# seungjunlee96/lightning-generative-models

Hardware: AMD Instinct MI355X
Metric: training images/sec (DDPM UNet 32x32, bs=128) (higher is better)
Workload: dtype f32; 1 GPU; configs/diffusion/ddpm.json UNet dim=64, 3x32x32 synthetic NCHW fp32, training_step+backward+Adam+EMA; global_batch=128, per_gpu_batch=128, parallelism=dp1, launch=hipGraph replay (1 graph/step)

## Files before the change

include/lgm_hip.h:

```cpp
#ifndef LGM_HIP_H
#define LGM_HIP_H

#include <stdint.h>

#ifdef __cplusplus
extern "C" {
#endif

#define LGM_ABI_VERSION 7
#define LGM_OK 0
#define LGM_ERR_INVALID (-1)
#define LGM_ERR_UNSUPPORTED (-2)

int lgm_abi_version(void);
const char* lgm_last_error(void);
const char* lgm_last_kernel(void);
int lgm_kernel_name_count(void);
const char* lgm_kernel_name(int i);

typedef struct {
  int32_t B, H, W, Cw;
  int32_t Ho, Wo, Nw;
  int32_t KH, KW, stride, pad;
} LgmConvGeom;
// ... 306 lines not shown
                float beta_acc, float* m_out, void* stream);
int lgm_bn_reduce3_coef(int modes, const float* v1, int64_t v1_pitch, const float* v2, int64_t v2_pitch,
                        const float* a, int64_t a_pitch, const float* mean, const float* rstd,
                        const float* gamma, const float* saved_m, int64_t rows, int C, float* coef8,
                        float* ggamma0, float* gbeta0, float beta_acc0, float* m_out, float* ggamma1,
                        float beta_acc1, float* sums3, void* workspace, void* stream);
int lgm_bn_reduce3_coef_tiles(int modes, const float* partial, int tiles, const float* gamma, const float* rstd,
                              const float* saved_m, int64_t rows, int C, float* coef8, float* ggamma0, float* gbeta0,
                              float beta_acc0, float* m_out, float* ggamma1, float beta_acc1, float* sums3, void* stream);
int lgm_bn_affine3x2(const float* v1, int64_t v1_pitch, const float* v2, int64_t v2_pitch, const float* a,
                     int64_t a_pitch, const float* mean, const float* rstd, const float* coef8, float* out0,
                     int64_t out0_pitch, float* out1, int64_t out1_pitch, int64_t rows, int C, void* stream);
int lgm_bn_affine3(const float* v1, int64_t v1_pitch, const float* v2, int64_t v2_pitch,
                   const float* a, int64_t a_pitch, const float* mean, const float* rstd,
                   const float* A1, const float* A2, const float* A3, const float* A4, float* out,
                   int64_t out_pitch, int accumulate, int act, float slope, int64_t rows, int C,
                   void* stream);
int lgm_image_transform(const unsigned char* src, int64_t B, int H, int W, int C, const unsigned char* flip,
                        float* dst, int S, void* stream);
int lgm_lerp_rows(const float* x, const float* y, const float* alpha, float* out, int64_t B,
                  int64_t rowlen, void* stream);
int64_t lgm_gp_penalty_workspace(int64_t npix);
int lgm_gp_penalty(const float* g, int64_t npix, int C, float lambda, const float* gscale,
                   float* loss_out, float* gbar, void* workspace, void* stream);
int lgm_r1_penalty(const float* g, int64_t npix, int64_t B, const float* gscale, float* loss_out,
                   float* gbar, void* workspace, void* stream);
int lgm_mean_col(const float* v, int64_t pitch, int64_t n, float scale, float* out, void* stream);
int lgm_fill_col(float* out, int64_t pitch, int64_t n, int ncols, int col, float scale,
                 const float* vptr, void* stream);
int lgm_wgan_dloss(float* vals4, void* stream);
int lgm_vqvae_loss(const float* recon, const float* out3, float w_recon, float w_vq, float* vals4, void* stream);
int lgm_vqvae_loss_samples(const float* per_sample, int n, const float* out3, float w_recon, float w_vq, float* vals4,
                           void* stream);
int lgm_tanh_mse_fwd(const float* pre, const float* target, int64_t pitch, int B, int C, int HW, int Cpad, float* xh,
                     float* per_sample, void* stream);
int lgm_tanh_mse_bwd(const float* xh, const float* target, int64_t pitch, const float* gloss, float w_recon, float w_vq,
                     int B, int C, int HW, int Cpad, float* gpre, float* g2, void* stream);

int64_t lgm_resstack_fwd_supported(int H, int W, int Cin, int hidden, int Rh, int layers);
int lgm_resstack_fwd(const float* x, int64_t x_pitch, int B, int H, int W, int Cin, int hidden, int Rh, int layers,
                     const float* const* w3, const float* const* w1, float* const* y, float* const* z, void* stream);
int lgm_scale_pair(const float* g, float w0, float w1, float* out2, void* stream);

int64_t lgm_conv3x3_bf16x3_supported(const LgmConvGeom* g, int mode, int64_t a_pitch);
int lgm_split_bf16x3(const float* src, uint16_t* dst, const int32_t* table, int n_slots, int64_t total_chunks,
                     int64_t plane_elems, void* stream);
int lgm_conv3x3_bf16x3(int mode, const LgmConvGeom* g, const float* a, int64_t a_pitch,
                       const uint16_t* w_planes, int64_t plane_elems, const float* bias, const float* res,
                       int64_t res_pitch, float* out, int64_t out_pitch, void* workspace,
                       int64_t workspace_bytes, void* stream);

int64_t lgm_conv3x3_wino_supported(const LgmConvGeom* g, int yx);
int64_t lgm_conv3x3_wino_fits(const LgmConvGeom* g, int64_t a_pitch, int64_t out_pitch, int64_t res_pitch);
int64_t lgm_conv3x3_wino_workspace_partial(const LgmConvGeom* g, int yx);
int64_t lgm_conv3x3_wino_bwd_supported(const LgmConvGeom* g, int64_t gy_pitch, int64_t x_pitch, int64_t gx_pitch,
                                       int64_t res_pitch);
int lgm_conv3x3_wino_bwd_workspaces(const LgmConvGeom* g, int partial, int64_t* out);
int lgm_conv3x3_wino_bwd(const LgmConvGeom* g, const float* gy, int64_t gy_pitch, const float* x, int64_t x_pitch,
                         const float* u_b, const float* res, int64_t res_pitch, float* gx, int64_t gx_pitch,
                         void* dgrad_ws, int64_t dgrad_ws_bytes, int64_t* partial, float* gw, float* gbias, float beta,
                         void* wgrad_ws, int64_t wgrad_ws_bytes, int64_t* desc, void* stream);
int64_t lgm_conv3x3_wino_wgrad2_supported(const LgmConvGeom* ga, const LgmConvGeom* gb);
typedef struct {
  const LgmConvGeom* g;
  const float* y;
  int64_t y_pitch;
  const float* x;
  int64_t x_pitch;
  float* gw;
  float* gbias;
  float beta;
  void* ws;
  int64_t ws_bytes;
  int64_t* desc;
} LgmWgradItem;
int64_t lgm_wgrad1x1_group_supported(int n, const LgmConvGeom* const* geoms);
int lgm_wgrad_queue_enable(int on);
int lgm_wgrad_queue_flush(void);
int lgm_wgrad1x1_group_workspaces(int n, const LgmConvGeom* const* geoms, int64_t* out);
int lgm_wgrad1x1_group(int n, const LgmWgradItem* items, void* stream);
int64_t lgm_conv3x3_wino_wgradn_supported(int n, const LgmConvGeom* const* geoms);
int lgm_conv3x3_wino_wgradn_workspaces(int n, const LgmConvGeom* const* geoms, int64_t* out);
int lgm_conv3x3_wino_wgradn(int n, const LgmWgradItem* items, void* stream);
int lgm_conv3x3_wino_wgrad2_workspaces(const LgmConvGeom* ga, const LgmConvGeom* gb, int64_t* out);
int lgm_conv3x3_wino_wgrad2(const LgmConvGeom* ga, const float* ya, int64_t ya_pitch, const float* xa, int64_t xa_pitch,
                            float* gwa, float* gba, float beta_a, void* wsa, int64_t wsa_bytes, int64_t* desca,
                            const LgmConvGeom* gb, const float* yb, int64_t yb_pitch, const float* xb, int64_t xb_pitch,
                            float* gwb, float* gbb, float beta_b, void* wsb, int64_t wsb_bytes, int64_t* descb,
                            void* stream);
int lgm_conv3x3_wino_partial(int yx, const LgmConvGeom* g, const float* a, int64_t a_pitch, const float* u,
                             const float* bias, float* out, int64_t out_pitch, void* workspace,
                             int64_t workspace_bytes, int64_t* partial, void* stream);
int64_t lgm_conv3x3_wino_workspace(const LgmConvGeom* g, int yx);
int lgm_wino_weights(const float* src, float* dst_f, float* dst_b, const int64_t* table, int n_slots,
                     int64_t total_blocks, void* stream);
int lgm_wino_set_debug_buffer(void* buf, int mode);
int lgm_conv3x3_wino(int yx, const LgmConvGeom* g, const float* a, int64_t a_pitch, const float* u,
                     const float* bias, const float* res, int64_t res_pitch, float* out, int64_t out_pitch,
                     void* workspace, int64_t workspace_bytes, void* stream);

int64_t lgm_conv3x3_wino4_supported(const LgmConvGeom* g, int yx);
int64_t lgm_conv3x3_wino4_workspace(const LgmConvGeom* g, int yx);
int64_t lgm_conv3x3_wino4_preferred(const LgmConvGeom* g, int yx);
int lgm_conv3x3_wino4_partial(int yx, const LgmConvGeom* g, const float* a, int64_t a_pitch, const float* u,
                              const float* bias, float* out, int64_t out_pitch, void* workspace,
                              int64_t workspace_bytes, int64_t* partial, void* stream);
int64_t lgm_conv3x3_wino4_stats_floats(const LgmConvGeom* g, int* parts_per_image);
int lgm_conv3x3_wino4_stats(const LgmConvGeom* g, const float* x, int64_t x_pitch, const float* u, const float* bias,
                            float* y, int64_t y_pitch, float* stats, int64_t stats_floats, void* stream);
int lgm_wino4_weights(const float* src, float* dst_f, float* dst_b, const int64_t* table, int n_slots,
                      int64_t total_blocks, void* stream);
int lgm_wino4_set_debug_buffer(void* buf, int exp);
int lgm_conv3x3_wino4(int yx, const LgmConvGeom* g, const float* a, int64_t a_pitch, const float* u,
                      const float* bias, const float* res, int64_t res_pitch, float* out, int64_t out_pitch,
                      void* workspace, int64_t workspace_bytes, void* stream);

int lgm_wino4_set_light(int mode);

int lgm_set_cu_margin(int margin);
int lgm_cu_margin(void);
int64_t lgm_conv3x3_wino4l_supported(const LgmConvGeom* g, int yx);
int64_t lgm_conv3x3_wino4l_workspace(const LgmConvGeom* g, int yx);
int lgm_conv3x3_wino4l(int yx, const LgmConvGeom* g, const float* a, int64_t a_pitch, const float* u,
                       const float* bias, const float* res, int64_t res_pitch, float* out, int64_t out_pitch,
                       void* workspace, int64_t workspace_bytes, void* stream);

int64_t lgm_conv3x3_wino4_wgrad_supported(const LgmConvGeom* g);
int64_t lgm_conv3x3_wino4_wgrad_workspace(const LgmConvGeom* g);
int lgm_conv3x3_wino4_wgrad(const LgmConvGeom* g, const float* y, int64_t y_pitch, const float* x, int64_t x_pitch,
                            float* gw, float* gbias, float beta, void* workspace, int64_t workspace_bytes,
                            int64_t* desc, void* stream);

int lgm_adam_step(float* p, const float* g, float* m, float* v, int64_t n, float lr, float b1,
                  float b2, float eps, float weight_decay, float step, const float* step_dev,
                  float grad_scale, int decoupled, void* stream);
int lgm_rmsprop_step(float* p, const float* g, float* sq, int64_t n, float lr, float alpha, float eps,
                     float weight_decay, float grad_scale, void* stream);
int lgm_clamp(float* x, int64_t n, float lo, float hi, void* stream);
int lgm_ema_lerp(float* shadow, const float* online, int64_t n, float w, void* stream);
int lgm_add_scalar(float* x, float a, void* stream);
int lgm_fill(float* x, int64_t n, float val, void* stream);

#ifdef __cplusplus
}
#endif
#endif
```

lightning-generative-models_amd/csrc/conv3x3.hip:

```cpp
#include <type_traits>
#include "lgm_common.h"

namespace lgm3x3 {
typedef unsigned int u32x4 __attribute__((ext_vector_type(4)));

constexpr int BN = 64;
constexpr int BK = 32;

enum { MODE_XY = 0, MODE_YX = 1, MODE_YXT = 2 };

struct Args {
  const float* a;
  const float* w;
  const float* bias;
  const float* res;
  float* out;
  long a_pitch, res_pitch, out_pitch;
  int B, H, W;
  int C;
  int N;
  int Wn;
  int TH, TW, NI, lgTW, lgTT;
  int tiles_h, tiles_w, tiles_n, NP;
  int units, per;
  int splits, pps;
  float* ws;
  long ws_stride;
  const unsigned short* wb;
  long w_plane;
};

__global__ __launch_bounds__(256) void splitk_reduce_kernel(const float* __restrict__ ws, long ws_stride, int splits,
                                                            const float* __restrict__ bias,
                                                            const float* __restrict__ res, long res_pitch,
                                                            float* __restrict__ out, long out_pitch, long M, int N) {
  const int n4 = N / 4;
  const long i = (long)blockIdx.x * blockDim.x + threadIdx.x;
  if (i >= M * n4) return;
  const long m = i / n4;
  const int n = (int)(i % n4) * 4;
  f32x4 s = *reinterpret_cast<const f32x4*>(ws + m * N + n);
  for (int k = 1; k < splits; ++k) s += *reinterpret_cast<const f32x4*>(ws + (long)k * ws_stride + m * N + n);
  if (bias) s += *reinterpret_cast<const f32x4*>(bias + n);
  if (res) s += *reinterpret_cast<const f32x4*>(res + m * res_pitch + n);
  *reinterpret_cast<f32x4*>(out + m * out_pitch + n) = s;
}

__device__ __forceinline__ int xcd_swizzle(int bid, int nb) {
  return (nb % 8 == 0) ? (bid % 8) * (nb / 8) + bid / 8 : bid;
}

struct Phase {
  int L, cc, cc_end;
  int tn, split, twi, thi, bg;
  int n0, b0, h0, w0;
  unsigned border;
  long abase;
  bool valid;
};

template <int MODE>
__global__ __launch_bounds__(256, 1) void conv3x3_kernel(const Args p) {
  constexpr int CK = 32;
  constexpr int LDP = CK + 4;
  constexpr int TPP = CK / 4;
  constexpr int PPP = 256 / TPP;
  constexpr int U = 9;
  constexpr int NJ = 288 / PPP;
  static_assert(NJ == U, "one patch position per step");
  constexpr int PBUF = 288 * LDP;
  extern __shared__ __align__(16) float smem[];

  const int tid = threadIdx.x;
  const int lane = tid & 63, wid = tid >> 6;
  const int wm = wid >> 1, wn = wid & 1;
  const int lr = lane & 31, lh = lane >> 5;
  float* Ts = smem + 2 * PBUF + wid * LGM_TS_FLOATS;

  const int Lb = xcd_swizzle(blockIdx.x, gridDim.x);
  const int L0 = Lb * p.per;
  const int L1 = min(p.units, L0 + p.per);
  if (L0 >= L1) return;

  const int PW = p.TW + 2, PP1 = (p.TH + 2) * PW;
  const int ncc_total = p.C / CK;

  auto place = [&](Phase& ph) {
    ph.n0 = ph.tn * BN;
    ph.w0 = ph.twi * p.TW;
    ph.h0 = ph.thi * p.TH;
    ph.b0 = ph.bg * p.NI;
    ph.cc = ph.split * p.pps;
    ph.cc_end = min(ncc_total, ph.cc + p.pps);
    ph.border = 16u | (ph.h0 == 0 ? 1u : 0u) | (ph.h0 + p.TH == p.H ? 2u : 0u) | (ph.w0 == 0 ? 4u : 0u) |
                (ph.w0 + p.TW == p.W ? 8u : 0u);
    ph.abase = ((long)((ph.b0 * p.H + ph.h0) * p.W + ph.w0) * p.a_pitch) * 4;
  };
  auto decode = [&](Phase& ph, int L) {
    ph.L = L;
    ph.tn = L % p.tiles_n;
    int ts = L / p.tiles_n;
    ph.split = ts % p.splits;
    ts /= p.splits;
    ph.twi = ts % p.tiles_w;
    ts /= p.tiles_w;
    ph.thi = ts % p.tiles_h;
    ph.bg = ts / p.tiles_h;
    place(ph);
  };
  auto advance = [&](Phase& ph) {
    if (!ph.valid) return;
    if (ph.cc + 1 < ph.cc_end) {
      ++ph.cc;
    } else if (ph.L + 1 < L1) {
      ++ph.L;
      if (++ph.tn == p.tiles_n) {
        ph.tn = 0;
        if (++ph.split == p.splits) {
          ph.split = 0;
          if (++ph.twi == p.tiles_w) {
            ph.twi = 0;
            if (++ph.thi == p.tiles_h) {
              ph.thi = 0;
              ++ph.bg;
            }
          }
// ... 957 lines not shown
extern "C" int lgm_split_bf16x3(const float* src, uint16_t* dst, const int32_t* table, int n_slots, int64_t total_chunks,
                                int64_t plane_elems, void* stream) {
  LGM_REQUIRE(src && dst && table && n_slots > 0 && total_chunks > 0 && plane_elems % 8 == 0 && lgm_aligned16(src) &&
                  lgm_aligned16(dst),
              "split_bf16x3: bad arguments");
  hipLaunchKernelGGL(lgm3x3::split_bf16x3_kernel, dim3((unsigned)lgm_cdiv(total_chunks, 256)), dim3(256), 0,
                     (hipStream_t)stream, src, dst, table, n_slots, (long)total_chunks, (long)plane_elems);
  LGM_LAUNCH_CHECK();
  return LGM_OK;
}

extern "C" int lgm_conv3x3_bf16x3(int mode, const LgmConvGeom* g, const float* a, int64_t a_pitch,
                                  const uint16_t* w_planes, int64_t plane_elems, const float* bias, const float* res,
                                  int64_t res_pitch, float* out, int64_t out_pitch, void* workspace,
                                  int64_t workspace_bytes, void* stream) {
  using namespace lgm3x3;
  LGM_REQUIRE(g && a && w_planes && out && (mode == 0 || mode == 1), "conv3x3_bf16x3: bad arguments");
  LGM_REQUIRE(lgm_conv3x3_bf16x3_supported(g, mode, a_pitch), "conv3x3_bf16x3: unsupported geometry");
  LGM_REQUIRE(lgm_aligned16(a) && lgm_aligned16(out) && a_pitch % 4 == 0 && out_pitch % 4 == 0 &&
                  (((uintptr_t)w_planes) & 15u) == 0 && plane_elems % 8 == 0 &&
                  (!res || (lgm_aligned16(res) && res_pitch % 4 == 0)) && (!bias || lgm_aligned16(bias)),
              "conv3x3_bf16x3: 16-byte aligned tensors with pitch %% 4 == 0 required");
  hipStream_t s = (hipStream_t)stream;
  Args p{};
  p.a = a; p.w = nullptr; p.wb = w_planes; p.w_plane = plane_elems; p.bias = bias; p.res = res; p.out = out;
  p.a_pitch = a_pitch; p.res_pitch = res_pitch; p.out_pitch = out_pitch;
  p.B = g->B; p.H = g->H; p.W = g->W;
  p.C = mode == 0 ? g->Cw : g->Nw;
  p.N = mode == 0 ? g->Nw : g->Cw;
  p.Wn = g->Cw;
  plan_tile(g->H, g->W, &p.TH, &p.TW, &p.NI);
  p.lgTW = ilog2(p.TW);
  p.lgTT = ilog2(p.TH * p.TW);
  p.tiles_h = g->H / p.TH;
  p.tiles_w = g->W / p.TW;
  p.tiles_n = p.N / BN;
  p.NP = p.NI * (p.TH + 2) * (p.TW + 2);
  const int groups = lgm_cdiv(g->B, p.NI);
  const long M = (long)g->B * g->H * g->W;
  p.splits = lgm_conv3x3_splits(g, p.C, p.N);
  if (p.splits > 1) {
    const long need = (long)p.splits * M * p.N * (long)sizeof(float);
    if (!workspace || workspace_bytes < need || !lgm_aligned16(workspace)) p.splits = 1;
  }
  p.ws = (float*)workspace;
  p.ws_stride = M * p.N;
  p.pps = lgm_cdiv(p.C / 32, p.splits);
  p.splits = lgm_cdiv(p.C / 32, p.pps);
  p.units = (int)((long)groups * p.tiles_h * p.tiles_w * p.tiles_n * p.splits);
  p.per = lgm_cdiv(p.units, lgm_cu_budget());
  const unsigned nblocks = (unsigned)lgm_cdiv(p.units, p.per);
  const size_t smem = (size_t)2 * 288 * 208 + 4 * LGM_TS_FLOATS * sizeof(float);
  if (mode == 0) {
    static bool attr = false;
    if (!attr) {
      hipFuncSetAttribute(reinterpret_cast<const void*>(conv3x3_b3_kernel<false>), hipFuncAttributeMaxDynamicSharedMemorySize,
                          (int)smem);
      attr = true;
    }
    hipLaunchKernelGGL(conv3x3_b3_kernel<false>, dim3(nblocks), dim3(256), smem, s, p);
  } else {
    static bool attr = false;
    if (!attr) {
      hipFuncSetAttribute(reinterpret_cast<const void*>(conv3x3_b3_kernel<true>), hipFuncAttributeMaxDynamicSharedMemorySize,
                          (int)smem);
      attr = true;
    }
    hipLaunchKernelGGL(conv3x3_b3_kernel<true>, dim3(nblocks), dim3(256), smem, s, p);
  }
  if (p.splits > 1) {
    const long items = M * (p.N / 4);
    hipLaunchKernelGGL(splitk_reduce_kernel, dim3((unsigned)lgm_cdiv(items, 256)), dim3(256), 0, s, (const float*)p.ws,
                       p.ws_stride, p.splits, bias, res, res_pitch, out, out_pitch, M, p.N);
  }
  LGM_LAUNCH_CHECK();
  return LGM_OK;
}

int lgm_splitk_reduce_launch(const float* ws, long ws_stride, int splits, const float* bias, const float* res,
                             long res_pitch, float* out, long out_pitch, long M, int N, hipStream_t s) {
  const long items = M * (N / 4);
  hipLaunchKernelGGL(lgm3x3::splitk_reduce_kernel, dim3((unsigned)lgm_cdiv(items, 256)), dim3(256), 0, s, ws, ws_stride,
                     splits, bias, res, res_pitch, out, out_pitch, M, N);
  LGM_LAUNCH_CHECK();
  return LGM_OK;
}

bool lgm_wgrad3x3_supported(const LgmConvGeom* g) {
  using namespace lgm3x3;
  int TH, TW, NI;
  if (!(g->KH == 3 && g->KW == 3 && g->stride == 1 && g->pad == 1)) return false;
  if (g->Cw % 64 != 0 || g->Nw % 64 != 0) return false;
  if (!plan_tile(g->H, g->W, &TH, &TW, &NI)) return false;
  return g->B % NI == 0;
}

void lgm_wgrad3x3_plan(const LgmConvGeom* g, int* splits, int* tps, int* total_ts) {
  using namespace lgm3x3;
  int TH, TW, NI;
  plan_tile(g->H, g->W, &TH, &TW, &NI);
  const int total = lgm_cdiv(g->B, NI) * (g->H / TH) * (g->W / TW);
  const long tiles = (long)(g->Nw / 64) * (g->Cw / 64);
  long s = lgm_cu_budget() / tiles;
  if (s > total) s = total;
  if (s < 1) s = 1;
  const int t = lgm_cdiv(total, s);
  *tps = t;
  const int tsplits = lgm_cdiv(total, t);
  const long wgs = tiles * tsplits;
  static const bool no_gsplit = getenv("LGM_NO_GSPLIT") != nullptr;
  const int gsplit = no_gsplit ? 1 : wgs <= 64 ? 4 : wgs <= 128 ? 2 : 1;
  *splits = tsplits * gsplit;
  *total_ts = total;
}

int lgm_wgrad3x3_launch(const LgmConvGeom* g, const float* y, long y_pitch, const float* x, long x_pitch,
                        float* out, float* bias_out, float beta, long slab, int splits, int tps, int total_ts,
                        hipStream_t s) {
  using namespace lgm3x3;
  WArgs p{};
  int TW;
  p.y = y; p.x = x; p.out = out; p.bias_out = bias_out; p.beta = beta; p.slab = slab;
  p.y_pitch = y_pitch; p.x_pitch = x_pitch;
  p.B = g->B; p.H = g->H; p.W = g->W; p.Nw = g->Nw; p.Cw = g->Cw;
  plan_tile(g->H, g->W, &p.TH, &TW, &p.NI);
  p.lgTH = ilog2(p.TH);
  p.tiles_h = g->H / p.TH; p.tiles_w = g->W / TW;
  p.tiles_n = g->Nw / 64; p.tiles_c = g->Cw / 64;
  p.splits = splits; p.tps = tps; p.total_ts = total_ts;
  p.gsplit = splits / lgm_cdiv(total_ts, tps);
  const int NP = p.NI * (p.TH + 2) * (TW + 2);
  (void)NP;
  const size_t smem = (size_t)(128 * 64 + 288 * 64) * sizeof(float);
  const unsigned nblocks = (unsigned)((long)p.tiles_n * p.tiles_c * splits);
#define LGM_W3_LAUNCH1(TWV, GSV)                                                                       \
  do {                                                                                                 \
    auto kern = wgrad3x3_kernel<TWV, GSV>;                                                             \
    static size_t attr = 0;                                                                            \
    if (smem > attr) {                                                                                 \
      hipFuncSetAttribute(reinterpret_cast<const void*>(kern), hipFuncAttributeMaxDynamicSharedMemorySize, (int)smem); \
      attr = smem;                                                                                     \
    }                                                                                                  \
    lgm_note_kernel(LGM_KNAME("lgm3x3::wgrad3x3_kernel<" #TWV ", " #GSV ">"));                                    \
    hipLaunchKernelGGL(kern, dim3(nblocks), dim3(256), smem, s, p);                                    \
  } while (0)
#define LGM_W3_LAUNCH(TWV)                                                                             \
  do {                                                                                                 \
    if (p.gsplit == 4) LGM_W3_LAUNCH1(TWV, 4);                                                         \
    else if (p.gsplit == 2) LGM_W3_LAUNCH1(TWV, 2);                                                    \
    else LGM_W3_LAUNCH1(TWV, 1);                                                                       \
  } while (0)
  if (p.gsplit != 1 && p.gsplit != 2 && p.gsplit != 4) {
    lgm_set_error("wgrad3x3: unsupported group split %d", p.gsplit);
    return LGM_ERR_UNSUPPORTED;
  }
  switch (TW) {
    case 32: LGM_W3_LAUNCH(32); break;
    case 16: LGM_W3_LAUNCH(16); break;
    case 8: LGM_W3_LAUNCH(8); break;
    case 4: LGM_W3_LAUNCH(4); break;
    default: lgm_set_error("wgrad3x3: unsupported tile width %d", TW); return LGM_ERR_UNSUPPORTED;
  }
#undef LGM_W3_LAUNCH
#undef LGM_W3_LAUNCH1
  LGM_LAUNCH_CHECK();
  return LGM_OK;
// ... 2 lines not shown
```

lightning-generative-models_amd/csrc/lgm_internal.h:

```cpp
#pragma once
#include <hip/hip_runtime.h>
#include <stdint.h>

#include "../../include/lgm_hip.h"

bool lgm_conv3x3_supported(const LgmConvGeom* g, int gather_channels, int out_channels);
int lgm_conv3x3_splits(const LgmConvGeom* g, int gather_channels, int out_channels);
int lgm_conv3x3_launch(int mode, const LgmConvGeom* g, const float* a, long a_pitch, const float* w, const float* bias,
                       const float* res, long res_pitch, float* out, long out_pitch, void* workspace, long workspace_bytes,
                       hipStream_t s);
int lgm_splitk_reduce_launch(const float* ws, long ws_stride, int splits, const float* bias, const float* res,
                             long res_pitch, float* out, long out_pitch, long M, int N, hipStream_t s);
bool lgm_wgrad3x3_supported(const LgmConvGeom* g);
void lgm_wgrad3x3_plan(const LgmConvGeom* g, int* splits, int* tps, int* total_ts);
int lgm_wgrad3x3_launch(const LgmConvGeom* g, const float* y, long y_pitch, const float* x, long x_pitch, float* out,
                        float* bias_out, float beta, long slab, int splits, int tps, int total_ts, hipStream_t s);

int lgm_wgrad_reduce_launch(const float* ws, long slab, float* gw, long n_w, float* gb, long n_b, int splits, float beta,
                            hipStream_t s);

bool lgm_wgrad1x1_supported(const LgmConvGeom* g, long y_pitch, long x_pitch);
void lgm_wgrad1x1_plan(const LgmConvGeom* g, int* splits, int* chunks_per_split);
int lgm_wgrad1x1_launch(const LgmConvGeom* g, const float* y, long y_pitch, const float* x, long x_pitch, float* out,
                        float* bias_out, float beta, long slab, int splits, int chunks_per_split, hipStream_t s);

bool lgm_gemm_stream_supported(long M, int N, int K, long x_pitch, long out_pitch, long res_pitch);
int lgm_gemm_stream_launch(const float* x, long x_pitch, const float* w, const float* bias, const float* res,
                           long res_pitch, float* out, long out_pitch, long M, int N, int K, hipStream_t s);
bool lgm_gemm_rows_supported(long M, int N, int K);
int lgm_gemm_rows_launch(const float* x, long x_pitch, const float* w, const float* bias, const float* res,
                         long res_pitch, float* out, long out_pitch, long M, int N, int K, hipStream_t s);

bool lgm_wino_supported(const LgmConvGeom* g, int gather_channels, int out_channels);
int lgm_wino_splits(const LgmConvGeom* g, int gather_channels, int out_channels, bool fused = false);
int lgm_wino_launch(const LgmConvGeom* g, int yx, const float* a, long a_pitch, const float* u, const float* bias,
                    const float* res, long res_pitch, float* out, long out_pitch, void* workspace, long workspace_bytes,
                    hipStream_t s, int64_t* partial = nullptr);
bool lgm_wino_wgrad_supported(const LgmConvGeom* g);
void lgm_wino_wgrad_plan(const LgmConvGeom* g, int* splits, int* cps, int* total_chunks);
int lgm_wino_wgrad_launch(const LgmConvGeom* g, const float* y, long y_pitch, const float* x, long x_pitch, float* out,
                          int bias, long slab, int splits, int cps, int total_chunks, hipStream_t s);
struct WinoPairPlan {
  int csplits, wsplits, cps, total_chunks;
};
WinoPairPlan lgm_wino_pair_plan(const LgmConvGeom* g, bool fused);
int lgm_wino_pair_launch(const LgmConvGeom* g, const float* gy, long gy_pitch, const float* x, long x_pitch,
                         const float* u_b, const float* res, long res_pitch, float* gx, long gx_pitch, void* dws,
                         long dws_bytes, int64_t* partial, float* slabs, int bias, long slab, hipStream_t s);

bool lgm_wino4_supported(const LgmConvGeom* g, int gather_channels, int out_channels);
int lgm_wino4_pick_splits(long base, long slots, int phases, int smax, int min_pps);
int lgm_wino4_splits(const LgmConvGeom* g, int gather_channels, int out_channels);
int lgm_wino4_launch(const LgmConvGeom* g, int yx, const float* a, long a_pitch, const float* u, const float* bias,
                     const float* res, long res_pitch, float* out, long out_pitch, void* workspace, long workspace_bytes,
                     hipStream_t s, int64_t* partial = nullptr, float* stats = nullptr);
bool lgm_wino4l_supported(const LgmConvGeom* g, int gather_channels, int out_channels);
long lgm_wino4l_units(const LgmConvGeom* g, int out_channels);
int lgm_wino4l_stats_parts(const LgmConvGeom* g);
int lgm_wino4l_class(const LgmConvGeom* g);
int lgm_wino4l_splits(const LgmConvGeom* g, int gather_channels, int out_channels);
int lgm_wino4l_launch(const LgmConvGeom* g, int yx, const float* a, long a_pitch, const float* u, const float* bias,
                      const float* res, long res_pitch, float* out, long out_pitch, void* workspace, long workspace_bytes,
                      hipStream_t s, int64_t* partial, float* stats);

bool lgm_wino4_wgrad_supported(const LgmConvGeom* g);
bool lgm_wino4_wgrad_use(const LgmConvGeom* g);
void lgm_wino4_wgrad_plan(const LgmConvGeom* g, long budget, int* splits, int* gps, int* total_groups);
int lgm_wino4_wgrad_launch(const LgmConvGeom* g, const float* y, long y_pitch, const float* x, long x_pitch, float* out,
                           int bias, long slab, int splits, int gps, int total, hipStream_t s);
int lgm_wino4_wgradn_launch(int n, const LgmConvGeom* const* gs, const float* const* ys, const long* yps,
                            const float* const* xs, const long* xps, float* const* outs, const int* biases,
                            const long* slabs, const int* splits, const int* gpss, const int* totals, hipStream_t s);

int lgm_linattn_ctx_launch(int mode, const float* qkv, long pitch, const float* mem_kv, const float* gout,
                           long gout_pitch, const float* ctx_in, int B, int n, int heads, int M, float scale,
                           float* ctx_out, float* kmax, float* ksum, float* r_out, hipStream_t s,
                           const float* kmax_in = nullptr, const float* ksum_in = nullptr, float* gmem_partial = nullptr);
int lgm_linattn_bwd_launch(const float* qkv, long pitch, const float* mem_kv, const float* gout, long gout_pitch,
                           const float* ctx, const float* gctx, const float* kmax, const float* ksum, const float* rvec,
                           int B, int n, int heads, int M, float scale, float* gqkv, long gq_pitch, float* gmem_partial,
                           hipStream_t s);
int lgm_linattn_bwd_fused_launch(const float* qkv, long pitch, const float* gout, long gout_pitch, const float* ctx,
                                 const float* gctx, const float* kmax, const float* ksum, const float* rvec,
                                 const float* xn, long xn_pitch, const float* wt, int B, int n, float scale, float* gxn,
                                 long gxn_pitch, float* slabs, int* blocks_out, hipStream_t s);
int lgm_linattn_out_fused_launch(const float* qkv, long pitch, const float* ctx, const float* wout, const float* bout,
                                 const float* g, const float* x, long x_pitch, float* ao, long ao_pitch, float* o2,
                                 long o2_pitch, float* y, long y_pitch, int B, int n, int Cout, float scale, hipStream_t s);
int lgm_attn_tiled_fwd_launch(const float* qkv, long pitch, const float* mem_kv, int B, int n, int heads, int M,
                              float scale, float* out, long out_pitch, float* lse, hipStream_t s);
int lgm_attn_tiled_bwd_launch(const float* qkv, long pitch, const float* mem_kv, const float* out, long out_pitch,
                              const float* gout, long gout_pitch, const float* lse, int B, int n, int heads, int M,
                              float scale, float* gqkv, long gq_pitch, float* gmem_partial, hipStream_t s);
```

lightning-generative-models_amd/csrc/wino4_device.h:

```cpp
#pragma once
#include "lgm_common.h"

namespace lgmwino4dev {
typedef unsigned int u32x4 __attribute__((ext_vector_type(4)));
typedef unsigned int u32x2 __attribute__((ext_vector_type(2)));
typedef float f32x2 __attribute__((ext_vector_type(2)));

constexpr int KC = 8;
constexpr int NXI = 36;

__device__ __forceinline__ f32x4 add4(const f32x4 a, const f32x4 b) { return a + b; }
__device__ __forceinline__ f32x4 sub4(const f32x4 a, const f32x4 b) {
  f32x2 lo, hi;
  asm("v_pk_add_f32 %0, %1, %2 neg_lo:[0,1] neg_hi:[0,1]"
      : "=v"(lo)
      : "v"(__builtin_shufflevector(a, a, 0, 1)), "v"(__builtin_shufflevector(b, b, 0, 1)));
  asm("v_pk_add_f32 %0, %1, %2 neg_lo:[0,1] neg_hi:[0,1]"
      : "=v"(hi)
      : "v"(__builtin_shufflevector(a, a, 2, 3)), "v"(__builtin_shufflevector(b, b, 2, 3)));
  return __builtin_shufflevector(lo, hi, 0, 1, 2, 3);
}
__device__ __forceinline__ f32x4 fma4(const float c, const f32x4 a, const f32x4 b) {
  return __builtin_elementwise_fma(f32x4{c, c, c, c}, a, b);
}
__device__ __forceinline__ f32x2 fma2(const float c, const f32x2 a, const f32x2 b) {
  return __builtin_elementwise_fma(f32x2{c, c}, a, b);
}

__device__ __forceinline__ __amdgpu_buffer_rsrc_t wave_buffer_rsrc(const float* ptr, unsigned bytes) {
  const unsigned long long ab = reinterpret_cast<unsigned long long>(ptr);
  const unsigned lo = __builtin_amdgcn_readfirstlane((unsigned)ab);
  const unsigned hi = __builtin_amdgcn_readfirstlane((unsigned)(ab >> 32));
  return __builtin_amdgcn_make_buffer_rsrc(reinterpret_cast<void*>(((unsigned long long)hi << 32) | lo), 0,
                                           __builtin_amdgcn_readfirstlane(bytes), 0x00020000);
}

struct ConvArgs {
  const float* a;
  const float* u;
  const float* bias;
  const float* res;
  float* out;
  long a_pitch, res_pitch, out_pitch;
  int B, H, W;
  int C;
  int N;
  int tb_h, tb_w, tiles_n, nbg;
  int splits, pps, units;
  int tn_slowest;
  int xcd_ranges;
  float* ws;
  long ws_stride;
};

struct ConvUnit {
  int tn, split, twi, thi, bg;
};
__device__ __forceinline__ ConvUnit conv_unit(const ConvArgs& p) {
  int L = (p.xcd_ranges && (gridDim.x & 7) == 0) ? (int)((blockIdx.x & 7) * (gridDim.x >> 3) + (blockIdx.x >> 3)) : (int)blockIdx.x;
  ConvUnit q;
  if (p.tn_slowest) {
    q.twi = L % p.tb_w;
    L /= p.tb_w;
    q.thi = L % p.tb_h;
    L /= p.tb_h;
    q.bg = L % p.nbg;
    L /= p.nbg;
    q.split = L % p.splits;
    q.tn = L / p.splits;
  } else {
    q.tn = L % p.tiles_n;
    L /= p.tiles_n;
    q.split = L % p.splits;
    L /= p.splits;
    q.twi = L % p.tb_w;
    L /= p.tb_w;
    q.thi = L % p.tb_h;
    q.bg = L / p.tb_h;
  }
  return q;
}

}
```

lightning-generative-models_amd/csrc/wino4_host.h:

```cpp
#pragma once
#include "wino4_device.h"

namespace lgmwino4host {
namespace {
using lgmwino4dev::KC;

template <class F>
int unit_class(int H, int W) {
  if (F::NCLS > 3 && H == 4 && W == 4) return 3;
  if (H == 8 && W == 8) return 2;
  if (H == 16 && W == 16) return 1;
  if (H >= F::UH && W >= F::UW && H % F::UH == 0 && W % F::UW == 0) return 0;
  return -1;
}

template <class F>
long unit_count(int cls, int B, int H, int W) {
  return cls == 0 ? (long)B * (H / F::UH) * (W / F::UW) : B / F::NI[cls];
}

template <class F>
bool supported(const LgmConvGeom* g, int gather_channels, int out_channels) {
  if (!(g->KH == 3 && g->KW == 3 && g->stride == 1 && g->pad == 1)) return false;
  if (gather_channels % 32 != 0 || out_channels % 64 != 0) return false;
  const int cls = unit_class<F>(g->H, g->W);
  if (cls < 0) return false;
  const long pix = (long)g->B * g->H * g->W + g->W + 1;
  if (pix * gather_channels >= (1L << 29) || pix * out_channels >= (1L << 29)) return false;
  if ((long)gather_channels * out_channels * 36 >= (1L << 29)) return false;
  return g->B % F::NI[cls] == 0;
}

template <class F>
int stats_parts(const LgmConvGeom* g) {
  return unit_class<F>(g->H, g->W) == 0 ? (g->H / F::UH) * (g->W / F::UW) * 4 : 0;
}

int split_front(long base, long slots, int phases, int forced, int* smax) {
  *smax = phases / 2 < 16 ? phases / 2 : 16;
  if (*smax < 1) *smax = 1;
  if (forced > 0) return forced < *smax ? forced : *smax;
  return base >= slots * 3 / 4 ? 1 : 0;
}

void unit_order(lgmwino4dev::ConvArgs& p, long M) {
  static const bool no_ranges = lgm_env_set("LGM_WINO4_NO_XCD_RANGES");
  p.xcd_ranges = no_ranges ? 0 : 1;
  static const int forced = lgm_env_int("LGM_WINO4_TN_SLOWEST", -1);
  const double in_b = 1.2 * (double)M * p.C * 4.0, u_b = 36.0 * p.C * p.N * 4.0;
  p.tn_slowest = forced >= 0 ? forced : ((in_b + 8.0 * u_b > in_b * p.tiles_n + u_b) ? 1 : 0);
}

template <auto KERN, int THREADS, class A>
void launch_kernel(const A& p, size_t smem, hipStream_t s) {
  static bool attr = false;
  if (!attr) {
    (void)hipFuncSetAttribute(reinterpret_cast<const void*>(KERN), hipFuncAttributeMaxDynamicSharedMemorySize, (int)smem);
    attr = true;
  }
  hipLaunchKernelGGL(KERN, dim3((unsigned)p.units), dim3(THREADS), smem, s, p);
}

template <class F>
int conv_launch(const LgmConvGeom* g, int yx, const float* a, long a_pitch, const float* u, const float* bias,
                const float* res, long res_pitch, float* out, long out_pitch, void* workspace, long workspace_bytes,
                hipStream_t s, int64_t* partial, float* stats) {
  typename F::Args p{};
  p.stats = stats;
  p.a = a; p.u = u; p.bias = bias; p.res = res; p.out = out;
  p.a_pitch = a_pitch; p.res_pitch = res_pitch; p.out_pitch = out_pitch;
  p.B = g->B; p.H = g->H; p.W = g->W;
  p.C = yx ? g->Nw : g->Cw;
  p.N = yx ? g->Cw : g->Nw;
  const int cls = unit_class<F>(g->H, g->W);
  p.tb_h = cls == 0 ? g->H / F::UH : 1;
  p.tb_w = cls == 0 ? g->W / F::UW : 1;
  p.nbg = g->B / F::NI[cls];
  p.tiles_n = p.N / 64;
  const long M = (long)g->B * g->H * g->W;
  p.splits = F::splits(g, p.C, p.N);
  if (p.splits > 1) {
    const long need = (long)p.splits * M * p.N * (long)sizeof(float);
    if (!workspace || workspace_bytes < need || !lgm_aligned16(workspace)) p.splits = 1;
  }
  p.ws = (float*)workspace;
  p.ws_stride = M * p.N;
  p.pps = lgm_cdiv(p.C / KC, p.splits);
  p.splits = lgm_cdiv(p.C / KC, p.pps);
  p.units = (int)((long)p.nbg * p.tb_h * p.tb_w * p.tiles_n * p.splits);
  unit_order(p, M);
  if (const int rc = F::launch(p, cls, res != nullptr, partial != nullptr, stats != nullptr, (size_t)F::MBUF * sizeof(float), s))
    return rc;
  if (partial) {
    partial[0] = p.splits;
    partial[1] = p.ws_stride;
    LGM_LAUNCH_CHECK_AS(F::LAUNCHER);
    return LGM_OK;
  }
  if (p.splits > 1)
    return lgm_splitk_reduce_launch(p.ws, p.ws_stride, p.splits, bias, res, res_pitch, out, out_pitch, M, p.N, s);
  LGM_LAUNCH_CHECK_AS(F::LAUNCHER);
  return LGM_OK;
}

}
}
```

lightning-generative-models_amd/csrc/winograd.hip:

```cpp
#include <stdlib.h>

#include <type_traits>

#include "lgm_common.h"

static void* lgm_wino_debug_buffer = nullptr;
static int lgm_wino_debug_mode = 0;
extern "C" int lgm_wino_set_debug_buffer(void* buf, int mode) {
  lgm_wino_debug_buffer = buf;
  lgm_wino_debug_mode = mode;
  return LGM_OK;
}

#ifndef LGM_STORE_AUX
#define LGM_STORE_AUX 0
#endif

namespace lgmwino {
typedef unsigned int u32x4 __attribute__((ext_vector_type(4)));
typedef float f32x2 __attribute__((ext_vector_type(2)));

__device__ __forceinline__ f32x4 sub4(const f32x4 a, const f32x4 b) {
#ifdef LGM_WINO_NO_ASM
  return a - b;
// ... 1311 lines not shown
  if (n < 2 || n > 8) return false;
  if (n > 4) {
    for (int k = 0; k < n; ++k)
      if (!gs[k]) return false;
    return wgradn_use4(n, gs);
  }
  int G0 = 0;
  long need = 0;
  static const bool alone4 = lgm_env_int("LGM_W4W_ALONE", 1) != 0;
  if (alone4 && !wgradn_use4(n, gs)) {
    bool all4 = true;
    for (int k = 0; k < n; ++k) all4 = all4 && gs[k] && lgm_wino4_wgrad_use(gs[k]);
    if (all4) return false;
  }
  if (wgradn_use4(n, gs))
    for (int k = 0; k < n; ++k)
      if (gs[k]->H == 4 && gs[k]->W == 4) return true;
  for (int k = 0; k < n; ++k) {
    if (!gs[k] || !lgm_wino_wgrad_supported(gs[k])) return false;
    int G, ipc;
    wgrad_class(gs[k]->H, gs[k]->W, &G, &ipc);
    if (k == 0) G0 = G;
    else if (G != G0) return false;
    need += 2L * (gs[k]->Nw / 64) * (gs[k]->Cw / 64);
  }
  return need <= lgm_cu_budget();
}

static void wgradn_budgets(int n, const LgmConvGeom* const* gs, long* budget) {
  double w[4], tot = 0;
  long mn[4], left = lgm_cu_budget();
  for (int k = 0; k < n; ++k) {
    w[k] = (double)gs[k]->B * gs[k]->H * gs[k]->W * gs[k]->Nw * gs[k]->Cw;
    tot += w[k];
    mn[k] = 2L * (gs[k]->Nw / 64) * (gs[k]->Cw / 64);
  }
  for (int k = 0; k < n; ++k) {
    long b = (long)((double)lgm_cu_budget() * w[k] / tot);
    if (b < mn[k]) b = mn[k];
    budget[k] = b;
    left -= b;
  }
  int big = 0;
  for (int k = 1; k < n; ++k)
    if (budget[k] - mn[k] > budget[big] - mn[big]) big = k;
  budget[big] += left;
  if (budget[big] < mn[big]) budget[big] = mn[big];
}

extern "C" int64_t lgm_conv3x3_wino_wgradn_supported(int n, const LgmConvGeom* const* geoms) {
  return (geoms && wgradn_supported(n, geoms)) ? 1 : 0;
}
extern "C" int64_t lgm_conv3x3_wino_wgrad2_supported(const LgmConvGeom* ga, const LgmConvGeom* gb) {
  const LgmConvGeom* gs[2] = {ga, gb};
  return wgradn_supported(2, gs) ? 1 : 0;
}

extern "C" int lgm_conv3x3_wino_wgradn_workspaces(int n, const LgmConvGeom* const* geoms, int64_t* out) {
  LGM_REQUIRE(geoms && out && wgradn_supported(n, geoms), "conv3x3_wino_wgradn_workspaces: unsupported group of layers");
  if (wgradn_use4(n, geoms)) {
    long b4[8];
    wgrad4_budgets(n, geoms, b4);
    for (int k = 0; k < n; ++k) {
      int splits, gps, total;
      lgm_wino4_wgrad_plan(geoms[k], b4[k], &splits, &gps, &total);
      out[k] = (int64_t)splits * ((int64_t)geoms[k]->Nw * 9 * geoms[k]->Cw + geoms[k]->Nw) * (int64_t)sizeof(float);
    }
    return LGM_OK;
  }
  long bud[4];
  wgradn_budgets(n, geoms, bud);
  for (int k = 0; k < n; ++k) {
    int splits, cps, total;
    wino_wgrad_plan_budget(geoms[k], bud[k], &splits, &cps, &total);
    out[k] = (int64_t)splits * ((int64_t)geoms[k]->Nw * 9 * geoms[k]->Cw + geoms[k]->Nw) * (int64_t)sizeof(float);
  }
  return LGM_OK;
}
extern "C" int lgm_conv3x3_wino_wgrad2_workspaces(const LgmConvGeom* ga, const LgmConvGeom* gb, int64_t* out) {
  const LgmConvGeom* gs[2] = {ga, gb};
  return lgm_conv3x3_wino_wgradn_workspaces(2, gs, out);
}

extern "C" int lgm_conv3x3_wino_wgradn(int n, const LgmWgradItem* it, void* stream) {
  using namespace lgmwino;
  LGM_REQUIRE(it && n >= 2 && n <= 8, "conv3x3_wino_wgradn: 2 ... 8 layers expected");
  const LgmConvGeom* gs[8];
  for (int k = 0; k < n; ++k) gs[k] = it[k].g;
  LGM_REQUIRE(wgradn_supported(n, gs), "conv3x3_wino_wgradn: unsupported group of layers");
  for (int k = 0; k < n; ++k)
    LGM_REQUIRE(it[k].desc && it[k].ws && lgm_aligned16(it[k].ws) &&
                wgrad2_operands_ok(it[k].g, it[k].y, it[k].y_pitch, it[k].x, it[k].x_pitch, it[k].gw, it[k].gbias),
                "conv3x3_wino_wgradn: layer %d: 16-byte aligned operands with pitch %% 4 == 0 inside 32-bit offsets expected", k);
  if (wgradn_use4(n, gs)) {
    long b4[8];
    wgrad4_budgets(n, gs, b4);
    const float* ys[8];
    const float* xs[8];
    long yps[8], xps[8], slabs[8];
    float* outs[8];
    int biases[8], splits[8], gpss[8], totals[8];
    for (int k = 0; k < n; ++k) {
      const LgmConvGeom* g = gs[k];
      lgm_wino4_wgrad_plan(g, b4[k], &splits[k], &gpss[k], &totals[k]);
      const long n_w = (long)g->Nw * 9 * g->Cw;
      slabs[k] = n_w + g->Nw;
      LGM_REQUIRE(it[k].ws_bytes >= (int64_t)splits[k] * slabs[k] * (int64_t)sizeof(float),
                  "conv3x3_wino_wgradn: workspace %d too small", k);
      ys[k] = it[k].y; xs[k] = it[k].x; yps[k] = it[k].y_pitch; xps[k] = it[k].x_pitch;
      outs[k] = (float*)it[k].ws; biases[k] = it[k].gbias ? 1 : 0;
      union { float f; int64_t i; } bbits;
      bbits.i = 0;
      bbits.f = it[k].beta;
      int64_t* d = it[k].desc;
      d[0] = (int64_t)(uintptr_t)it[k].ws; d[1] = slabs[k]; d[2] = (int64_t)(uintptr_t)it[k].gw; d[3] = n_w;
      d[4] = (int64_t)(uintptr_t)it[k].gbias; d[5] = it[k].gbias ? g->Nw : 0; d[6] = splits[k]; d[7] = bbits.i;
    }
    return lgm_wino4_wgradn_launch(n, gs, ys, yps, xs, xps, outs, biases, slabs, splits, gpss, totals, (hipStream_t)stream);
  }
  int G, ipc;
  wgrad_class(gs[0]->H, gs[0]->W, &G, &ipc);
  long bud[4];
  wgradn_budgets(n, gs, bud);
  WGArgs pp[4];
  unsigned nb[4] = {0, 0, 0, 0};
  for (int k = 0; k < n; ++k) {
    const LgmConvGeom* g = gs[k];
    int splits, cps, total;
    wino_wgrad_plan_budget(g, bud[k], &splits, &cps, &total);
    const long n_w = (long)g->Nw * 9 * g->Cw, slab = n_w + g->Nw;
    LGM_REQUIRE(it[k].ws_bytes >= (int64_t)splits * slab * (int64_t)sizeof(float), "conv3x3_wino_wgradn: workspace %d too small", k);
    wino_wgrad_prepare(g, it[k].y, it[k].y_pitch, it[k].x, it[k].x_pitch, (float*)it[k].ws, it[k].gbias ? 1 : 0, slab, splits,
                       cps, total, pp[k]);
    nb[k] = (unsigned)((g->Nw / 64) * (g->Cw / 64) * splits);
    union { float f; int64_t i; } bbits;
    bbits.i = 0;
    bbits.f = it[k].beta;
    int64_t* d = it[k].desc;
    d[0] = (int64_t)(uintptr_t)it[k].ws; d[1] = slab; d[2] = (int64_t)(uintptr_t)it[k].gw; d[3] = n_w;
    d[4] = (int64_t)(uintptr_t)it[k].gbias; d[5] = it[k].gbias ? g->Nw : 0; d[6] = splits; d[7] = bbits.i;
  }
  for (int k = n; k < 4; ++k) pp[k] = pp[n - 1];
  const size_t smem = (size_t)3 * WBUF * sizeof(float);
  hipStream_t s = (hipStream_t)stream;
  const int e0 = (int)nb[0], e1 = e0 + (int)nb[1], e2 = e1 + (int)nb[2];
  const unsigned grid = nb[0] + nb[1] + nb[2] + nb[3];
#define LGM_WGN(GG)                                                                                              \
  do {                                                                                                           \
    static bool attr2 = false, attr4 = false;                                                                    \
    if (n == 2) {                                                                                                \
      auto kern = wino_wgrad2_kernel<GG>;                                                                        \
      if (!attr2) {                                                                                              \
        (void)hipFuncSetAttribute(reinterpret_cast<const void*>(kern), hipFuncAttributeMaxDynamicSharedMemorySize, (int)smem); \
        attr2 = true;                                                                                            \
      }                                                                                                          \
      hipLaunchKernelGGL(kern, dim3(grid), dim3(256), smem, s, pp[0], pp[1], e0);                                \
    } else {                                                                                                     \
      auto kern = wino_wgrad4_kernel<GG>;                                                                        \
      if (!attr4) {                                                                                              \
        (void)hipFuncSetAttribute(reinterpret_cast<const void*>(kern), hipFuncAttributeMaxDynamicSharedMemorySize, (int)smem); \
        attr4 = true;                                                                                            \
      }                                                                                                          \
      hipLaunchKernelGGL(kern, dim3(grid), dim3(256), smem, s, pp[0], pp[1], pp[2], pp[3], e0, e1, e2);          \
    }                                                                                                            \
  } while (0)
  if (n == 2)
    lgm_note_kernel(G == 8 ? LGM_KNAME("lgmwino::wino_wgrad2_kernel<8>") : G == 4 ? LGM_KNAME("lgmwino::wino_wgrad2_kernel<4>") : LGM_KNAME("lgmwino::wino_wgrad2_kernel<2>"));
  else
    lgm_note_kernel(G == 8 ? LGM_KNAME("lgmwino::wino_wgrad4_kernel<8>") : G == 4 ? LGM_KNAME("lgmwino::wino_wgrad4_kernel<4>") : LGM_KNAME("lgmwino::wino_wgrad4_kernel<2>"));
  if (G == 8) LGM_WGN(8);
  else if (G == 4) LGM_WGN(4);
  else LGM_WGN(2);
#undef LGM_WGN
  LGM_LAUNCH_CHECK();
  return LGM_OK;
}

extern "C" int lgm_conv3x3_wino_wgrad2(const LgmConvGeom* ga, const float* ya, int64_t ya_pitch, const float* xa,
                                       int64_t xa_pitch, float* gwa, float* gba, float beta_a, void* wsa, int64_t wsa_bytes,
                                       int64_t* desca, const LgmConvGeom* gb, const float* yb, int64_t yb_pitch,
                                       const float* xb, int64_t xb_pitch, float* gwb, float* gbb, float beta_b, void* wsb,
                                       int64_t wsb_bytes, int64_t* descb, void* stream) {
  LgmWgradItem it[2] = {{ga, ya, ya_pitch, xa, xa_pitch, gwa, gba, beta_a, wsa, wsa_bytes, desca},
                        {gb, yb, yb_pitch, xb, xb_pitch, gwb, gbb, beta_b, wsb, wsb_bytes, descb}};
  return lgm_conv3x3_wino_wgradn(2, it, stream);
}

static WinoPairPlan wino_pair_plan_search(const LgmConvGeom* g, bool fused);
WinoPairPlan lgm_wino_pair_plan(const LgmConvGeom* g, bool fused) {
  struct Key {
    int B, H, W, C, N, f;
    bool operator==(const Key& o) const { return B == o.B && H == o.H && W == o.W && C == o.C && N == o.N && f == o.f; }
  };
  thread_local Key keys[64];
  thread_local WinoPairPlan plans[64];
  thread_local int n = 0;
  const Key k{g->B, g->H, g->W, g->Cw, g->Nw, fused ? 1 : 0};
  for (int i = 0; i < n; ++i)
    if (keys[i] == k) return plans[i];
  const WinoPairPlan p = wino_pair_plan_search(g, fused);
  if (n < 64) {
// ... 126 lines not shown
```

lightning-generative-models_amd/csrc/winograd4.hip:

```cpp
#include <atomic>
#include <stdlib.h>

#include <type_traits>

#include "wino4_host.h"

static void* lgm_wino4_debug_buffer = nullptr;
static int lgm_wino4_debug_exp = 0;
static int lgm_wino4_debug_slots = 0;
static int lgm_wino4_debug_next = 0;
extern "C" int lgm_wino4_set_debug_buffer(void* buf, int exp) {
  lgm_wino4_debug_buffer = buf;
  lgm_wino4_debug_exp = exp & 0xffff;
  lgm_wino4_debug_slots = exp >> 16;
  lgm_wino4_debug_next = 0;
  return LGM_OK;
}

#ifndef LGM_WINO4_PFU
#define LGM_WINO4_PFU 1
#endif

namespace lgmwino4 {
using namespace lgmwino4dev;

constexpr int VBUF = NXI * 256;
constexpr int MBUF = NXI * 32 * 32;

template <int CLS>
struct Geo;
template <>
struct Geo<0> {
  static constexpr int NI = 1, TTH = 4, TTW = 8, PH = 18, PW = 34, RS = 34, IMG = PH * RS, PLANE = 641;
};
template <>
struct Geo<1> {
  static constexpr int NI = 2, TTH = 4, TTW = 4, PH = 18, PW = 18, RS = 20, IMG = PH * RS, PLANE = 737;
};
template <>
struct Geo<2> {
  static constexpr int NI = 8, TTH = 2, TTW = 2, PH = 10, PW = 10, RS = 10, IMG = 112, PLANE = 897;
};
template <>
struct Geo<3> {
  static constexpr int NI = 32, TTH = 1, TTW = 1, PH = 4, PW = 4, RS = 4, IMG = 20, PLANE = 641;
};

struct Args : ConvArgs {
  long long* dbg;
  float* stats;
};

template <int CLS, bool DBG = false, int EXP = 0, bool STATS = false>
__global__ __launch_bounds__(512, 2) void wino4_conv_kernel(const Args p) {
  using GE = Geo<CLS>;
  constexpr bool PFU = LGM_WINO4_PFU != 0;
  int nstamp = 0;
  auto stamp = [&]() {
    if (DBG) {
      if (threadIdx.x == 0 && nstamp < 30) p.dbg[blockIdx.x * 32 + 1 + nstamp] = (long long)__builtin_amdgcn_s_memtime();
      ++nstamp;
    }
  };
  stamp();
  const long long rt_entry = DBG ? (long long)__builtin_amdgcn_s_memrealtime() : 0;
  constexpr int NI = GE::NI, PH = GE::PH, PW = GE::PW, RS = GE::RS, IMG = GE::IMG, PLANE = GE::PLANE;
  constexpr int RBUF = 8 * PLANE;
  constexpr int NPIX = NI * PH * PW;
  constexpr int NJ = (2 * NPIX + 511) / 512;
  constexpr int HALO = CLS == 3 ? 0 : 1;
  extern __shared__ __align__(16) float smem[];
  float* const Rb = smem;
  float* const Vb = smem + 2 * RBUF;
  float* const Mb = smem;
  const int tid = threadIdx.x;
  const int lane = tid & 63;
  const int wid = __builtin_amdgcn_readfirstlane(tid >> 6);
  const int lr = lane & 31, lh = lane >> 5;

  const ConvUnit un = conv_unit(p);
  const int tn = un.tn, split = un.split, twi = un.twi, thi = un.thi, bg = un.bg;
  const int n0 = tn * 64;
  const int h0 = thi * (4 * GE::TTH), w0 = twi * (4 * GE::TTW), b0 = bg * NI;
  const int ncc = p.C / KC;
  const int cc0 = split * p.pps;
  const int cc1 = min(ncc, cc0 + p.pps);
  const int nph = cc1 - cc0;

  const unsigned nrec_a = (unsigned)((long)p.B * p.H * p.W * p.a_pitch * 4);
  const __amdgpu_buffer_rsrc_t rsrc_a = wave_buffer_rsrc(p.a, nrec_a);
  unsigned goff[NJ], plds[NJ];
#pragma unroll
  for (int j = 0; j < NJ; ++j) {
    const int s = tid + 512 * j;
    const int pix = s >> 1, q = s & 1;
    unsigned g = nrec_a, l = (unsigned)(q * 4 * PLANE + NI * IMG);
    if (pix < NPIX) {
      const int img = pix / (PH * PW);
      const int rem = pix - img * (PH * PW);
      const int py = rem / PW, px = rem - py * PW;
      const int gy = h0 - HALO + py, gx = w0 - HALO + px;
      l = (unsigned)(q * 4 * PLANE + img * IMG + py * RS + px);
      if (gy >= 0 && gy < p.H && gx >= 0 && gx < p.W)
        g = (unsigned)((((long)(b0 + img) * p.H + gy) * p.W + gx) * p.a_pitch + q * 4) * 4u;
    }
    goff[j] = g;
    plds[j] = l;
  }
  u32x4 rp[NJ];
  auto fetch1 = [&](int j, int ph) -> u32x4 {
    const unsigned soff = (unsigned)((cc0 + ph) * (KC * 4));
    return __builtin_amdgcn_raw_buffer_load_b128(rsrc_a, ph < nph ? goff[j] : nrec_a, soff, 0);
  };
  auto commit_r = [&](float* rbuf, int j, const u32x4 r) {
    float* d = rbuf + plds[j];
    const f32x4 f = __builtin_bit_cast(f32x4, r);
    d[0] = f[0];
    d[PLANE] = f[1];
    d[2 * PLANE] = f[2];
    d[3 * PLANE] = f[3];
  };
  u32x4 rq0[NJ], rq1[NJ];
#pragma unroll
  for (int j = 0; j < NJ; ++j) rq0[j] = fetch1(j, 0);
#pragma unroll
  for (int j = 0; j < NJ; ++j) rq1[j] = fetch1(j, 1);
#pragma unroll
  for (int j = 0; j < NJ; ++j) rp[j] = fetch1(j, 2);

  int t_tile, t_img, t_ty, t_tx;
  const int half = wid >> 2;
  const int tk = (lane & 3) + 4 * (lane >> 5);
  if (CLS == 0) {
    t_img = 0;
    t_ty = wid & 3;
    t_tx = (lane >> 2) & 7;
    t_tile = t_ty * 8 + t_tx;
  } else if (CLS == 1) {
    t_img = (wid >> 1) & 1;
    t_ty = 2 * (wid & 1) + ((lane >> 4) & 1);
    t_tx = (lane >> 2) & 3;
    t_tile = t_img * 16 + t_ty * 4 + t_tx;
  } else if (CLS == 2) {
    t_img = 2 * (wid & 3) + ((lane >> 4) & 1);
    t_ty = (lane >> 3) & 1;
    t_tx = (lane >> 2) & 1;
    t_tile = t_img * 4 + t_ty * 2 + t_tx;
  } else {
    t_img = 8 * (wid & 3) + ((lane >> 2) & 7);
    t_ty = 0;
    t_tx = 0;
    t_tile = t_img;
  }
  const int trd = tk * PLANE + t_img * IMG + 4 * t_ty * RS + 4 * t_tx;
  const int vwr = (tk >> 2) * 128 + t_tile * 4 + (tk & 3) + half * (18 * 256);

  const int xg = wid & 3, ch = wid >> 2;
  const int vrd = xg * (9 * 256) + lh * 128 + lr * 4;
  const __amdgpu_buffer_rsrc_t rsrc_u = wave_buffer_rsrc(p.u, (unsigned)((long)p.N * p.C * NXI * 4));
  const unsigned ulane = (unsigned)((ch * 64 + lane) * 16);
  const unsigned ubase = (unsigned)((tn * ncc + cc0) * NXI + xg * 9) * 2048u;
  unsigned pf = 0;
  if (PFU) {
    const unsigned ubytes = min((unsigned)nph * (NXI * 2048u), 2u << 20);
    const unsigned nx = gridDim.x >> 3;
    const unsigned spatial = (unsigned)(p.nbg * p.tb_h * p.tb_w);
    const unsigned grp = p.tn_slowest ? 1u : (unsigned)(p.tiles_n * p.splits);
    const unsigned share = p.tn_slowest ? ((unsigned)blockIdx.x >> 3) % spatial : ((unsigned)blockIdx.x >> 3) / grp;
    const unsigned nshare = p.tn_slowest ? min(nx, spatial) : nx / grp;
    const unsigned off = (share * 512u + (unsigned)tid) * 128u;
    if (p.xcd_ranges && (gridDim.x & 7) == 0 && off < ubytes && nshare * 512u * 128u >= ubytes)
      pf = __builtin_amdgcn_raw_buffer_load_b32(rsrc_u, off, (unsigned)((tn * ncc + cc0) * NXI) * 2048u, 0);
  }
  auto load_u = [&](int ph, int e) -> f32x4 {
    const unsigned soff = ubase + (unsigned)(ph * NXI + e) * 2048u;
    u32x4 v = __builtin_amdgcn_raw_buffer_load_b128(rsrc_u, ulane, soff, 0);
    return __builtin_bit_cast(f32x4, v);
  };

  auto body = [&](auto half_c) {
    constexpr int HALF = decltype(half_c)::value;
    f32x16 acc[9];
#pragma unroll
    for (int e = 0; e < 9; ++e)
#pragma unroll
      for (int r = 0; r < 16; ++r) acc[e][r] = 0.f;
    f32x2 T[3][3];
// ... 69 lines not shown
    };

    stamp();
    f32x4 uq[3];
#pragma unroll
    for (int e = 0; e < 3; ++e) uq[e] = load_u(0, e);
    if (DBG) __builtin_amdgcn_sched_barrier(0);
    stamp();
#pragma unroll
    for (int j = 0; j < NJ; ++j) commit_r(Rb, j, rq0[j]);
#pragma unroll
    for (int j = 0; j < NJ; ++j) commit_r(Rb + RBUF, j, rq1[j]);
    if (DBG) __builtin_amdgcn_sched_barrier(0);
    stamp();
    __syncthreads();
    if (PFU) asm volatile("" ::"v"(pf));
    stamp();
#pragma unroll
    for (int cp = 0; cp < 3; ++cp) stage1(0, cp);
#pragma unroll
    for (int i = 0; i < 3; ++i) {
      stage2(Vb, i, 0);
      stage2(Vb, i, 1);
    }
    if (DBG) __builtin_amdgcn_sched_barrier(0);
    stamp();
    __syncthreads();
    stamp();

    auto phase = [&](int ph, auto cur_c) {
      constexpr int cur = decltype(cur_c)::value;
      float* const rcur = Rb + cur * RBUF;
      float* const vcur = Vb + cur * VBUF;
      float* const vnxt = Vb + (cur ^ 1) * VBUF;
      f32x4 vf = *reinterpret_cast<const f32x4*>(vcur + vrd);
#pragma unroll
      for (int e = 0; e < 9; ++e) {
        f32x4 vfn = vf;
        if (e < 8 && !(EXP & 8)) vfn = *reinterpret_cast<const f32x4*>(vcur + vrd + (e + 1) * 256);
        const f32x4 uf = uq[e % 3];
#pragma unroll
        for (int s = 0; s < 4; ++s) acc[e] = __builtin_amdgcn_mfma_f32_32x32x2f32(uf[s], vf[s], acc[e], 0, 0, 0);
        if (!(EXP & 4)) uq[e % 3] = (e + 3 < 9) ? load_u(ph, e + 3) : load_u(ph + 1, e + 3 - 9);
        if (!(EXP & 1)) {
          if (e < 3) stage1(cur ^ 1, e);
          else stage2(vnxt, (e - 3) >> 1, (e - 3) & 1);
        }
        if (e >= 9 - NJ && !(EXP & 2)) {
          commit_r(rcur, e - (9 - NJ), rp[e - (9 - NJ)]);
          rp[e - (9 - NJ)] = fetch1(e - (9 - NJ), ph + 3);
        }
        vf = vfn;
        __builtin_amdgcn_sched_barrier(0);
      }
      static_assert(NJ >= 1 && NJ <= 4, "the commit is dealt out over the last NJ steps");
      __syncthreads();
      stamp();
    };
    for (int ph = 0; ph < nph; ph += 2) {
      phase(ph, std::integral_constant<int, 0>{});
      if (ph + 1 < nph) phase(ph + 1, std::integral_constant<int, 1>{});
    }

    const int th = tid & 255;
    const int eq = th & 3, et = (th >> 2) & 31, rpair = __builtin_amdgcn_readfirstlane(th >> 7);
    int e_img, e_ty, e_tx;
    if (CLS == 0) {
      e_img = 0;
      e_ty = et >> 3;
      e_tx = et & 7;
    } else if (CLS == 1) {
      e_img = et >> 4;
      e_ty = (et >> 2) & 3;
      e_tx = et & 3;
    } else if (CLS == 2) {
      e_img = et >> 2;
      e_ty = (et >> 1) & 1;
      e_tx = et & 1;
    } else {
      e_img = et;
      e_ty = 0;
      e_tx = 0;
    }
    const long opix = ((long)(b0 + e_img) * p.H + h0 + 4 * e_ty) * p.W + w0 + 4 * e_tx;
    const bool partial = p.splits > 1;
    const int ncol0 = n0 + HALF * 16 + eq * 4;
    float* const obase = partial ? p.ws + (long)split * p.ws_stride + opix * p.N + ncol0 : p.out + opix * p.out_pitch + ncol0;
    const long opitch = partial ? (long)p.N : p.out_pitch;
    const bool has_res = !partial && p.res != nullptr;
    const float* const rbase = p.res + opix * p.res_pitch + ncol0;
    float* const Mh = Mb + HALF * (MBUF / 2);
    const int mrd = (et * 4 + (eq ^ ((et >> 1) & 3))) * 4;
    const int mwr = (lr * 4) * 4;
#pragma unroll
    for (int rd = 0; rd < 2; ++rd) {
      if (rd == 1) __syncthreads();
#pragma unroll
      for (int e = 0; e < 9; ++e)
#pragma unroll
        for (int gg = 0; gg < 2; ++gg) {
          const int g = 2 * rd + gg;
          const f32x4 v = {acc[e][4 * g], acc[e][4 * g + 1], acc[e][4 * g + 2], acc[e][4 * g + 3]};
          *reinterpret_cast<f32x4*>(Mh + (xg * 9 + e) * 512 + mwr + (((2 * gg + lh) ^ ((lr >> 1) & 3)) * 4)) = v;
        }
      __syncthreads();
      f32x4 X[2][6];
#pragma unroll
      for (int j = 0; j < 6; ++j) {
        auto m = [&](int i) -> f32x4 { return *reinterpret_cast<const f32x4*>(Mh + (i * 6 + j) * 512 + mrd); };
        const f32x4 m1 = m(1), m2 = m(2), m3 = m(3), m4 = m(4);
        if (rpair == 0) {
          const f32x4 s1 = add4(m1, m2), s2 = add4(m3, m4);
          X[0][j] = add4(add4(m(0), s1), s2);
          X[1][j] = fma4(4.f, s2, s1);
        } else {
          const f32x4 d1 = sub4(m1, m2), d2 = sub4(m3, m4);
          X[0][j] = fma4(2.f, d2, d1);
          X[1][j] = add4(fma4(8.f, d2, d1), m(5));
        }
      }
      f32x4 bv = {0.f, 0.f, 0.f, 0.f};
      if (!partial && p.bias) bv = *reinterpret_cast<const f32x4*>(p.bias + ncol0 + rd * 32);
      f32x4 st1 = {0.f, 0.f, 0.f, 0.f}, st2 = {0.f, 0.f, 0.f, 0.f};
#pragma unroll
      for (int rr = 0; rr < 2; ++rr) {
        const long orow = (long)(2 * rr + rpair) * p.W;
        const f32x4 s1 = add4(X[rr][1], X[rr][2]), d1 = sub4(X[rr][1], X[rr][2]);
        const f32x4 s2 = add4(X[rr][3], X[rr][4]), d2 = sub4(X[rr][3], X[rr][4]);
        f32x4 y[4];
        y[0] = add4(add4(X[rr][0], s1), s2);
        y[1] = fma4(2.f, d2, d1);
        y[2] = fma4(4.f, s2, s1);
        y[3] = add4(fma4(8.f, d2, d1), X[rr][5]);
        if (STATS) {
#pragma unroll
          for (int oj = 0; oj < 4; ++oj) {
            st1 = add4(st1, y[oj]);
            st2 = __builtin_elementwise_fma(y[oj], y[oj], st2);
          }
        }
        if (has_res) {
#pragma unroll
          for (int oj = 0; oj < 4; ++oj)
            y[oj] = add4(y[oj], *reinterpret_cast<const f32x4*>(rbase + (orow + oj) * p.res_pitch + rd * 32));
        }
#pragma unroll
        for (int oj = 0; oj < 4; ++oj) *reinterpret_cast<f32x4*>(obase + (orow + oj) * opitch + rd * 32) = add4(y[oj], bv);
      }
      if (STATS) {
#pragma unroll
        for (int m = 4; m < 64; m <<= 1) {
#pragma unroll
          for (int k = 0; k < 4; ++k) {
            st1[k] += __shfl_xor(st1[k], m, 64);
            st2[k] += __shfl_xor(st2[k], m, 64);
          }
        }
        if ((lane >> 2) == 0) {
          const int ublk = (bg * p.tb_h + thi) * p.tb_w + twi;
          const int part = (tid >> 6) & 3;
          float* sp = p.stats + ((long)(ublk * 4 + part) * 2) * p.N + ncol0 + rd * 32;
          *reinterpret_cast<f32x4*>(sp) = st1;
          *reinterpret_cast<f32x4*>(sp + p.N) = st2;
        }
      }
      stamp();
    }
    if (DBG && threadIdx.x == 0) {
      p.dbg[blockIdx.x * 32] = nstamp;
      p.dbg[blockIdx.x * 32 + 31] = (long long)__builtin_amdgcn_s_memrealtime();
      if (nstamp <= 29) p.dbg[blockIdx.x * 32 + 30] = rt_entry;
      if (blockIdx.x == 0) {
        long long* m = p.dbg + 4095 * 32;
        m[0] = p.C; m[1] = p.N; m[2] = p.H; m[3] = p.W; m[4] = p.B; m[5] = p.splits; m[6] = CLS; m[7] = gridDim.x;
        m[8] = p.res != nullptr; m[9] = p.tn_slowest;
      }
    }
  };
  if (half == 0) body(std::integral_constant<int, 0>{});
  else body(std::integral_constant<int, 1>{});
}

__device__ __forceinline__ void ggt36(const float (&g)[9], float (&u)[36]) {
  constexpr float k6 = 1.f / 6.f, k12 = 1.f / 12.f, k24 = 1.f / 24.f;
  float t[6][3];
#pragma unroll
  for (int b = 0; b < 3; ++b) {
    const float g0 = g[b], g1 = g[3 + b], g2 = g[6 + b];
    const float s02 = g0 + g2, e = __builtin_fmaf(g0, k24, g2 * k6);
    t[0][b] = g0 * 0.25f;
    t[1][b] = -(s02 + g1) * k6;
    t[2][b] = -(s02 - g1) * k6;
    t[3][b] = __builtin_fmaf(g1, k12, e);
    t[4][b] = __builtin_fmaf(g1, -k12, e);
    t[5][b] = g2;
  }
#pragma unroll
  for (int i = 0; i < 6; ++i) {
    const float g0 = t[i][0], g1 = t[i][1], g2 = t[i][2];
    const float s02 = g0 + g2, e = __builtin_fmaf(g0, k24, g2 * k6);
    u[i * 6 + 0] = g0 * 0.25f;
    u[i * 6 + 1] = -(s02 + g1) * k6;
    u[i * 6 + 2] = -(s02 - g1) * k6;
    u[i * 6 + 3] = __builtin_fmaf(g1, k12, e);
    u[i * 6 + 4] = __builtin_fmaf(g1, -k12, e);
    u[i * 6 + 5] = g2;
  }
}

__global__ __launch_bounds__(256) void wino4_weights_kernel(const float* __restrict__ src, float* __restrict__ dst_f,
                                                            float* __restrict__ dst_b, const long* __restrict__ table,
                                                            int n_slots) {
  __shared__ float wt[32 * 9 * 36];
  int lo = 0, hi = n_slots - 1;
  const long bid = blockIdx.x;
  while (lo < hi) {
    const int mid = (lo + hi + 1) >> 1;
    if (table[mid * 6 + 5] <= bid) lo = mid;
    else hi = mid - 1;
  }
  const long* row = table + lo * 6;
  const long soff = row[0];
  const int Np = (int)row[1], Cp = (int)row[2];
  const long lb = bid - row[5];
  const int cblocks = Cp / 32;
  const int nb = (int)(lb / cblocks), cb = (int)(lb % cblocks);
  const float* w = src + soff + ((long)nb * 32 * 9) * Cp + cb * 32;
  const int tid = threadIdx.x;
  for (int i = tid; i < 288 * 8; i += 256) {
    const int r = i >> 3, c4 = (i & 7) * 4;
    *reinterpret_cast<f32x4*>(wt + r * 36 + c4) = *reinterpret_cast<const f32x4*>(w + (long)r * Cp + c4);
  }
  __syncthreads();
  if (dst_f) {
    const int n = tid & 31, cq = tid >> 5;
    f32x4 uu[36];
#pragma unroll
    for (int s = 0; s < 4; ++s) {
      float g[9], u[36];
#pragma unroll
      for (int t = 0; t < 9; ++t) g[t] = wt[(n * 9 + t) * 36 + cq * 4 + s];
      ggt36(g, u);
#pragma unroll
      for (int x = 0; x < 36; ++x) uu[x][s] = u[x];
    }
    float* d = dst_f + row[3] + (((long)(nb >> 1) * (Cp / 8) + cb * 4 + (cq >> 1)) * NXI) * 512 +
               (((n >> 4) * 2 + (cq & 1)) * 32 + 16 * (nb & 1) + (n & 15)) * 4;
#pragma unroll
    for (int x = 0; x < 36; ++x) *reinterpret_cast<f32x4*>(d + x * 512) = uu[x];
  }
  if (dst_b) {
    const int c = tid & 31, nq = tid >> 5;
    f32x4 uu[36];
#pragma unroll
    for (int s = 0; s < 4; ++s) {
      float g[9], u[36];
#pragma unroll
      for (int t = 0; t < 9; ++t) g[8 - t] = wt[((nq * 4 + s) * 9 + t) * 36 + c];
      ggt36(g, u);
#pragma unroll
      for (int x = 0; x < 36; ++x) uu[x][s] = u[x];
    }
    float* d = dst_b + row[4] + (((long)(cb >> 1) * (Np / 8) + nb * 4 + (nq >> 1)) * NXI) * 512 +
               (((c >> 4) * 2 + (nq & 1)) * 32 + 16 * (cb & 1) + (c & 15)) * 4;
#pragma unroll
    for (int x = 0; x < 36; ++x) *reinterpret_cast<f32x4*>(d + x * 512) = uu[x];
  }
}

namespace {
struct Form {
  using Args = lgmwino4::Args;
  static constexpr int THREADS = 512, MBUF = lgmwino4::MBUF;
  static constexpr int UH = 16, UW = 32;
  static constexpr int NCLS = 4;
  static constexpr int NI[NCLS] = {1, 2, 8, 32};
  static constexpr const char* LAUNCHER = "lgm_wino4_launch";
  static int splits(const LgmConvGeom* g, int gather_channels, int out_channels);
  static int launch(Args& p, int cls, bool res, bool partial, bool stats, size_t smem, hipStream_t s);
  template <int CLS, bool DBG = false, int EXP = 0, bool STATS = false>
  static void go(const Args& p, size_t smem, hipStream_t s) {
    lgmwino4host::launch_kernel<wino4_conv_kernel<CLS, DBG, EXP, STATS>, THREADS>(p, smem, s);
  }
};

int Form::launch(Args& p, int cls, bool res, bool partial, bool stats, size_t smem, hipStream_t s) {
  p.dbg = (long long*)lgm_wino4_debug_buffer;
  if (p.dbg && lgm_wino4_debug_slots > 0) {
    if (lgm_wino4_debug_next >= lgm_wino4_debug_slots || p.units > 4095) p.dbg = nullptr;
    else p.dbg += (long)(lgm_wino4_debug_next++) * 4096 * 32;
  }
  lgm_note_kernel(cls == 0 ? LGM_KNAME("lgmwino4::wino4_conv_kernel<0, false, 0, false>") : cls == 1 ? LGM_KNAME("lgmwino4::wino4_conv_kernel<1, false, 0, false>")
                  : cls == 2 ? LGM_KNAME("lgmwino4::wino4_conv_kernel<2, false, 0, false>") : LGM_KNAME("lgmwino4::wino4_conv_kernel<3, false, 0, false>"));
  if (p.dbg) {
    const int e = lgm_wino4_debug_exp;
    if (cls == 1) go<1, true>(p, smem, s);
    else if (cls == 2) go<2, true>(p, smem, s);
    else if (cls == 3) go<3, true>(p, smem, s);
    else if (e == 0) go<0, true, 0>(p, smem, s);
    else if (e == 1) go<0, true, 1>(p, smem, s);
    else if (e == 2) go<0, true, 2>(p, smem, s);
    else if (e == 3) go<0, true, 3>(p, smem, s);
    else if (e == 4) go<0, true, 4>(p, smem, s);
    else if (e == 7) go<0, true, 7>(p, smem, s);
    else if (e == 8) go<0, true, 8>(p, smem, s);
    else go<0, true, 15>(p, smem, s);
  } else if (stats) {
    if (cls != 0 || p.splits != 1 || res || partial) {
      lgm_set_error("wino4 (stats): class-0 maps, an unsplit reduction and no residual expected");
      return LGM_ERR_UNSUPPORTED;
    }
    lgm_note_kernel(LGM_KNAME("lgmwino4::wino4_conv_kernel<0, false, 0, true>"));
    go<0, false, 0, true>(p, smem, s);
  } else if (cls == 0) go<0>(p, smem, s);
  else if (cls == 1) go<1>(p, smem, s);
  else if (cls == 2) go<2>(p, smem, s);
  else go<3>(p, smem, s);
  return LGM_OK;
}
}

}

using lgmwino4::Form;
namespace w4h = lgmwino4host;

static std::atomic<int> lgm_wino4_light_override{-1};
extern "C" int lgm_wino4_set_light(int mode) {
  lgm_wino4_light_override.store(mode, std::memory_order_relaxed);
  return LGM_OK;
}
struct Wino4LightAsk {
  bool given;
  int mode;
};
static Wino4LightAsk wino4_light_ask() {
  static const bool env_given = lgm_env_set("LGM_WINO4_LIGHT");
  static const int env_mode = lgm_env_int("LGM_WINO4_LIGHT", 0);
  const int ov = lgm_wino4_light_override.load(std::memory_order_relaxed);
  return {env_given || ov >= 0, ov >= 0 ? ov : env_mode};
}
static bool wino4_use_light(const LgmConvGeom* g, int gather_channels, int out_channels) {
  if (!lgm_wino4l_supported(g, gather_channels, out_channels)) return false;
  const Wino4LightAsk ask = wino4_light_ask();
  if (ask.mode != 0) return true;
  if (ask.given) return false;
  static long below[3] = {-1, 0, 0};
  if (below[0] < 0) {
    long b0 = 200, b1 = 128, b2 = 64;
    if (const char* e = getenv("LGM_WINO4_LIGHT_BELOW")) {
      b1 = b2 = -1;
      sscanf(e, "%ld,%ld,%ld", &b0, &b1, &b2);
      if (b1 < 0) b1 = b0;
      if (b2 < 0) b2 = b1;
    }
    below[1] = b1, below[2] = b2, below[0] = b0 < 0 ? 0 : b0;
  }
  const int cls = lgm_wino4l_class(g);
  return cls >= 0 && lgm_wino4l_units(g, out_channels) / 2 < below[cls];
}

bool lgm_wino4_supported(const LgmConvGeom* g, int gather_channels, int out_channels) {
  return wino4_use_light(g, gather_channels, out_channels) || w4h::supported<Form>(g, gather_channels, out_channels);
}

int lgm_wino4_pick_splits(long base, long slots, int phases, int smax, int min_pps) {
  int s0 = (int)((slots + base - 1) / base);
  if (s0 > smax) s0 = smax;
  while (s0 > 1 && phases / s0 < min_pps) --s0;
  if (base * s0 <= slots) return s0;
  int best = s0;
  double best_cost = 1e30;
  for (int s = 1; s <= smax; ++s) {
    if (s > 1 && phases / s < min_pps) break;
    const long rounds = (base * s + slots - 1) / slots;
    const double pps = (double)((phases + s - 1) / s);
    const double cost = (double)rounds * (5.5 + pps) + (s > 1 ? 2.0 + 0.5 * s : 0.0);
    if (cost < best_cost - 1e-9) {
      best_cost = cost;
      best = s;
    }
  }
  return best;
}

int Form::splits(const LgmConvGeom* g, int gather_channels, int out_channels) {
  const int cls = w4h::unit_class<Form>(g->H, g->W);
  if (cls < 0) return 1;
  const long base = w4h::unit_count<Form>(cls, g->B, g->H, g->W) * (out_channels / 64);
  static const int forced = lgm_env_int("LGM_WINO4_SPLITS", 0);
  const long slots = lgm_cu_budget();
  const int phases = gather_channels / lgmwino4dev::KC;
  int smax;
  if (const int s = w4h::split_front(base, slots, phases, forced, &smax)) return s;
  static const int min_pps = lgm_env_int("LGM_WINO4_MIN_PPS", 4);
  static const bool old_rule = lgm_env_set("LGM_WINO4_SPLITS_CEIL");
  if (old_rule) {
    int s = (int)((slots + base - 1) / base);
    if (s > smax) s = smax;
    while (s > 1 && phases / s < min_pps) --s;
    return s;
  }
  return lgm_wino4_pick_splits(base, slots, phases, smax, min_pps);
}

int lgm_wino4_splits(const LgmConvGeom* g, int gather_channels, int out_channels) {
  return wino4_use_light(g, gather_channels, out_channels) ? lgm_wino4l_splits(g, gather_channels, out_channels)
                                                           : Form::splits(g, gather_channels, out_channels);
}

int lgm_wino4_launch(const LgmConvGeom* g, int yx, const float* a, long a_pitch, const float* u, const float* bias,
                     const float* res, long res_pitch, float* out, long out_pitch, void* workspace, long workspace_bytes,
                     hipStream_t s, int64_t* partial, float* stats) {
  if (wino4_use_light(g, yx ? g->Nw : g->Cw, yx ? g->Cw : g->Nw))
    return lgm_wino4l_launch(g, yx, a, a_pitch, u, bias, res, res_pitch, out, out_pitch, workspace, workspace_bytes, s, partial,
                             stats);
  return w4h::conv_launch<Form>(g, yx, a, a_pitch, u, bias, res, res_pitch, out, out_pitch, workspace, workspace_bytes, s,
                                partial, stats);
}

extern "C" int64_t lgm_conv3x3_wino4_supported(const LgmConvGeom* g, int yx) {
  if (!g) return 0;
  return lgm_wino4_supported(g, yx ? g->Nw : g->Cw, yx ? g->Cw : g->Nw) ? 1 : 0;
}

extern "C" int64_t lgm_conv3x3_wino4_stats_floats(const LgmConvGeom* g, int* parts_per_image) {
  if (parts_per_image) *parts_per_image = 0;
  if (!g || !lgm_wino4_supported(g, g->Cw, g->Nw)) return 0;
  const int per = wino4_use_light(g, g->Cw, g->Nw) ? lgm_wino4l_stats_parts(g) : w4h::stats_parts<Form>(g);
  if (per == 0) return 0;
  if (lgm_wino4_splits(g, g->Cw, g->Nw) != 1) return 0;
  static const bool off = lgm_env_set("LGM_NO_GN_EPI_STATS");
  if (off) return 0;
  if (parts_per_image) *parts_per_image = per;
  return (int64_t)g->B * per * 2 * g->Nw;
}

extern "C" int64_t lgm_conv3x3_wino4_workspace(const LgmConvGeom* g, int yx) {
  if (!g) return -1;
  const int gc = yx ? g->Nw : g->Cw, oc = yx ? g->Cw : g->Nw;
  if (!lgm_wino4_supported(g, gc, oc)) return 0;
  return lgm_splitk_workspace(g, oc, lgm_wino4_splits(g, gc, oc));
}

extern "C" int64_t lgm_conv3x3_wino4_preferred(const LgmConvGeom* g, int yx) {
  if (!g) return 0;
  const int gc = yx ? g->Nw : g->Cw, oc = yx ? g->Cw : g->Nw;
  if (!lgm_wino4_supported(g, gc, oc)) return 0;
  static const int force = lgm_env_int("LGM_WINO4_FORCE", 0);
  if (force) return 1;
  const bool light = wino4_use_light(g, gc, oc);
  const int cls = light ? lgm_wino4l_class(g) : w4h::unit_class<Form>(g->H, g->W);
  static const long min_units0_env = lgm_env_long("LGM_WINO4_MIN_UNITS", -1);
  static const long min_units1_env = lgm_env_long("LGM_WINO4_MIN_UNITS1", -1);
  const long min_units0 = min_units0_env >= 0 ? min_units0_env : (light ? 32 : 128);
  const long min_units1 = min_units1_env >= 0 ? min_units1_env : (light ? 32 : 128);
  if (cls == 3) {
    static const bool no4 = lgm_env_set("LGM_WINO4_NO4");
    const int narrow = gc < oc ? gc : oc;
    const long units = w4h::unit_count<Form>(3, g->B, g->H, g->W) * (narrow / 64);
    return (!no4 && wino4_light_ask().mode == 0 && narrow >= 256 && units >= 32) ? 1 : 0;
  }
  const long base = light ? lgm_wino4l_units(g, oc) / 2 : w4h::unit_count<Form>(cls, g->B, g->H, g->W) * (oc / 64);
  static const int fwd_all = lgm_env_int("LGM_WINO4_FWD_ALL", 0);
  if (light && yx == 0 && fwd_all) return 1;
  static const int bwd_all = lgm_env_int("LGM_WINO4_BWD_ALL", 0);
  if (light && yx == 1 && bwd_all) return 1;
  static const bool no8 = lgm_env_set("LGM_WINO4_NO8");
  static const bool noyx8 = lgm_env_set("LGM_WINO4_NOYX8");
  static const int c2_minc = lgm_env_int("LGM_WINO4_C2_MINC", 256);
  if (cls == 2) return (!no8 && (yx == 0 || !noyx8) && base >= 32 && gc >= c2_minc) ? 1 : 0;
  static const int c1_minc = lgm_env_int("LGM_WINO4_C1_MINC", 0);
  if (cls == 1 && gc < c1_minc) return 0;
  static const long min_units1w_env = lgm_env_long("LGM_WINO4_MIN_UNITS1W", -1);
  const long min_units1w = min_units1w_env >= 0 ? min_units1w_env : (light ? 32 : 64);
  if (cls == 1 && gc >= 128 && base >= min_units1w) return 1;
  return base >= (cls == 1 ? min_units1 : min_units0) ? 1 : 0;
}

extern "C" int lgm_wino4_weights(const float* src, float* dst_f, float* dst_b, const int64_t* table, int n_slots,
                                 int64_t total_blocks, void* stream) {
  LGM_REQUIRE(src && table && n_slots > 0 && total_blocks > 0 && (dst_f || dst_b), "wino4_weights: bad arguments");
  hipLaunchKernelGGL(lgmwino4::wino4_weights_kernel, dim3((unsigned)total_blocks), dim3(256), 0, (hipStream_t)stream,
                     src, dst_f, dst_b, (const long*)table, n_slots);
  LGM_LAUNCH_CHECK();
  return LGM_OK;
}

extern "C" int lgm_conv3x3_wino4(int yx, const LgmConvGeom* g, const float* a, int64_t a_pitch, const float* u,
                                 const float* bias, const float* res, int64_t res_pitch, float* out, int64_t out_pitch,
                                 void* workspace, int64_t workspace_bytes, void* stream) {
  LGM_REQUIRE(g && a && u && out, "conv3x3_wino4: null pointer");
  const int gc = yx ? g->Nw : g->Cw, oc = yx ? g->Cw : g->Nw;
  LGM_REQUIRE(lgm_wino4_supported(g, gc, oc), "conv3x3_wino4: unsupported geometry (3x3/s1/p1, maps 16x16 or H %% 16 == 0 "
              "and W %% 32 == 0, reduction channels %% 32, produced channels %% 64)");
  if (const int rc = lgm_conv_operands_check("conv3x3_wino4", g, gc, oc, a, a_pitch,
                                             u, bias, res, res_pitch, out, out_pitch))
    return rc;
  return lgm_wino4_launch(g, yx, a, a_pitch, u, bias, res, res_pitch, out, out_pitch, workspace, workspace_bytes,
                          (hipStream_t)stream);
}

extern "C" int lgm_conv3x3_wino4_stats(const LgmConvGeom* g, const float* x, int64_t x_pitch, const float* u,
// ... 28 lines not shown
```

lightning-generative-models_amd/csrc/winograd4_wgrad.hip:

```cpp
#include <stdlib.h>

#include <type_traits>

#include "wino4_device.h"

#ifndef W4W_EXP
#define W4W_EXP 0
#endif

namespace lgmwino4w {
using namespace lgmwino4dev;

constexpr int YB = NXI * 256;
constexpr int XB = NXI * 128;
constexpr int OPB = YB + XB;
constexpr int MH = NXI * 512;

struct WArgs {
  const float* y;
  const float* x;
  float* out;
  long y_pitch, x_pitch, slab;
  int bias;
  int B, H, W, Nw, Cw;
  int tiles_c;
  int splits, gps, total_groups;
  int grow;
  int trows;
  int xcd_order;
  int sq;
};

__device__ __forceinline__ void wino4_wgrad_body(const WArgs& p, const int bidx) {
  extern __shared__ __align__(16) float smem[];
  const int tid = threadIdx.x;
  const int lane = tid & 63;
  const int wid = __builtin_amdgcn_readfirstlane(tid >> 6);
  const int lr = lane & 31, lh = lane >> 5;

  int L = bidx;
  const int inner = p.tiles_c * (p.Nw >> 6);
  if (p.xcd_order) {
    const int nblk = inner * p.splits, v = bidx & 7, r = nblk & 7;
    L = v * (nblk >> 3) + (v < r ? v : r) + (bidx >> 3);
  }
  const int split = p.xcd_order ? L / inner : L % p.splits;
  const int bid = p.xcd_order ? L % inner : L / p.splits;
  const int tc = bid % p.tiles_c, tn = bid / p.tiles_c;
  const int n0 = tn * 64, c0 = tc * 32;
  const int g_begin = split * p.gps;
  const int g_end = min(p.total_groups, g_begin + p.gps);
  const int nph = g_end - g_begin;

  const int xg = wid & 3, nh = wid >> 2;
  const int ard = xg * (9 * 256) + lh * 128 + (nh * 32 + lr) * 2;
  const int brd = YB + xg * (9 * 128) + lh * 64 + lr * 2;

  const unsigned nrec_y = (unsigned)((long)p.B * p.H * p.W * p.y_pitch * 4);
  const unsigned nrec_x = (unsigned)(((long)p.B * p.H * p.W + p.W + 1) * p.x_pitch * 4);
  const __amdgpu_buffer_rsrc_t rsrc_y = wave_buffer_rsrc(p.y, nrec_y);
  const __amdgpu_buffer_rsrc_t rsrc_x = wave_buffer_rsrc(p.x - (long)(p.W + 1) * p.x_pitch, nrec_x);

  struct GPos {
    int gx, ty, b;
  };
  auto gdecode = [&](int g) {
    GPos q;
    q.gx = g % p.grow;
    const int r = g / p.grow;
    q.ty = r % p.trows;
    q.b = r / p.trows;
    return q;
  };
  auto gnext = [&](GPos& q) {
    if (++q.gx == p.grow) {
      q.gx = 0;
      if (++q.ty == p.trows) {
        q.ty = 0;
        ++q.b;
      }
    }
  };
  const int gh = p.sq == 1 ? 8 : 4, gw = p.sq == 1 ? 8 : p.sq == 2 ? 4 : 16;
  auto gpix = [&](const GPos& q) -> long {
    return ((long)(p.sq == 2 ? 4 * q.b : q.b) * p.H + gh * q.ty) * p.W + gw * q.gx;
  };
  auto tile_row = [&](int tl) { return p.sq == 1 ? (tl >> 1) : 0; };
  auto tile_col = [&](int tl) { return p.sq == 1 ? (tl & 1) : p.sq == 2 ? 0 : tl; };
  auto tile_img = [&](int tl) { return p.sq == 2 ? tl : 0; };

  f32x16 acc[9];
#pragma unroll
  for (int e = 0; e < 9; ++e)
#pragma unroll
    for (int r = 0; r < 16; ++r) acc[e][r] = 0.f;

  auto mfma_step = [&](const float* buf, int e, f32x2& af, f32x2& bf) {
    f32x2 an = af, bn = bf;
    if (e < 8 && !(W4W_EXP & 8)) {
      an = *reinterpret_cast<const f32x2*>(buf + ard + (e + 1) * 256);
      bn = *reinterpret_cast<const f32x2*>(buf + brd + (e + 1) * 128);
    }
    acc[e] = __builtin_amdgcn_mfma_f32_32x32x2f32(af[0], bf[0], acc[e], 0, 0, 0);
    acc[e] = __builtin_amdgcn_mfma_f32_32x32x2f32(af[1], bf[1], acc[e], 0, 0, 0);
    af = an;
    bf = bn;
  };

  float bsum = 0.f;

  auto body_y = [&]() {
    const int tl = wid;
    const unsigned ylane =
        (unsigned)(((((long)tile_img(tl) * p.H + 4 * tile_row(tl)) * p.W + 4 * tile_col(tl)) * p.y_pitch + n0 + lane) * 4);
    const int ywr = (tl >> 1) * 128 + lane * 2 + (tl & 1);
    float dA[4][4], dB[4][4];
    GPos gq = gdecode(g_begin);
    auto load = [&](float (&d)[4][4], int ph) {
      const unsigned ok = ph < nph ? 0u : nrec_y;
      const unsigned ybase = (unsigned)(gpix(gq) * p.y_pitch * 4);
#pragma unroll
      for (int r = 0; r < 4; ++r)
#pragma unroll
        for (int c = 0; c < 4; ++c)
          d[r][c] = __builtin_bit_cast(float, __builtin_amdgcn_raw_buffer_load_b32(
              rsrc_y, ylane + ok, ybase + (unsigned)(((long)r * p.W + c) * p.y_pitch * 4), 0));
      if (ph + 1 < nph) gnext(gq);
    };
    float T[6][4];
    auto vertical2 = [&](const float (&d)[4][4], int cp) {
      const f32x2 d0 = {d[0][2 * cp], d[0][2 * cp + 1]}, d1 = {d[1][2 * cp], d[1][2 * cp + 1]};
      const f32x2 d2 = {d[2][2 * cp], d[2][2 * cp + 1]}, d3 = {d[3][2 * cp], d[3][2 * cp + 1]};
      const f32x2 s02 = d0 + d2, s13 = d1 + d3;
      const f32x2 e = fma2(4.f, d2, d0), f = fma2(4.f, d3, d1);
      const f32x2 t1 = s02 + s13, t2 = s02 - s13, t3 = fma2(2.f, f, e), t4 = fma2(-2.f, f, e);
#pragma unroll
      for (int k = 0; k < 2; ++k) {
        const int c = 2 * cp + k;
        T[0][c] = d0[k];
        T[1][c] = t1[k];
        T[2][c] = t2[k];
        T[3][c] = t3[k];
        T[4][c] = t4[k];
        T[5][c] = d3[k];
      }
      bsum += t1[0] + t1[1];
    };
    auto horizontal = [&](float* ybuf, int i) {
      float* v = ybuf + ywr + i * (6 * 256);
      const float t0 = T[i][0], t1 = T[i][1], t2 = T[i][2], t3 = T[i][3];
      const float s02 = t0 + t2, s13 = t1 + t3;
      const float e = __builtin_fmaf(4.f, t2, t0), f = __builtin_fmaf(4.f, t3, t1);
      v[0 * 256] = t0;
      v[1 * 256] = s02 + s13;
      v[2 * 256] = s02 - s13;
      v[3 * 256] = __builtin_fmaf(2.f, f, e);
      v[4 * 256] = __builtin_fmaf(-2.f, f, e);
      v[5 * 256] = t3;
    };
    load(dA, 0);
    load(dB, 1);
    vertical2(dA, 0);
    vertical2(dA, 1);
#pragma unroll
    for (int i = 0; i < 6; ++i) horizontal(smem, i);
    __syncthreads();
    auto phase = [&](int ph, auto cur_c) {
      constexpr int cur = decltype(cur_c)::value;
      const float* const ocur = smem + cur * OPB;
      float* const onxt = smem + (cur ^ 1) * OPB;
      f32x2 af = *reinterpret_cast<const f32x2*>(ocur + ard);
      f32x2 bf = *reinterpret_cast<const f32x2*>(ocur + brd);
#pragma unroll
      for (int e = 0; e < 9; ++e) {
        mfma_step(ocur, e, af, bf);
        if (e == 0 && !(W4W_EXP & 4)) {
          if (cur == 0) load(dA, ph + 2);
          else load(dB, ph + 2);
        }
        if (e < 2) {
          if (!(W4W_EXP & 1)) {
            if (cur == 0) vertical2(dB, e);
            else vertical2(dA, e);
          }
        } else if (e < 8) {
          if (!(W4W_EXP & 1)) horizontal(onxt, e - 2);
        }
        __builtin_amdgcn_sched_barrier(0);
      }
      __syncthreads();
    };
    for (int ph = 0; ph < nph; ph += 2) {
      phase(ph, std::integral_constant<int, 0>{});
      if (ph + 1 < nph) phase(ph + 1, std::integral_constant<int, 1>{});
    }
  };

  auto body_x = [&](auto half_c) {
    constexpr int HALF = decltype(half_c)::value;
    const int tl = 2 * ((wid >> 1) & 1) + lh;
    const int c = lr;
    const int trow = tile_row(tl), tcol = tile_col(tl);
    const int tlast = p.sq == 1 ? 1 : p.sq == 2 ? 0 : 3;
    const unsigned xlane =
        (unsigned)(((((long)tile_img(tl) * p.H + 4 * trow) * p.W + 4 * tcol) * p.x_pitch + c0 + c) * 4);
    const int xwr = YB + (tl >> 1) * 64 + c * 2 + (tl & 1) + HALF * (18 * 128);
    constexpr int R0 = HALF ? 1 : 0;
    float d[5][6];
    GPos gq = gdecode(g_begin);
    auto load_rows = [&](int ph, int r_lo, int r_hi) {
      const GPos q = gq;
      const unsigned xbase = (unsigned)(gpix(q) * p.x_pitch * 4);
      const bool live = ph < nph;
#pragma unroll
      for (int r = 0; r < 5; ++r) {
        if (r < r_lo || r >= r_hi) continue;
        const int yy = gh * q.ty + 4 * trow - 1 + R0 + r;
        const bool rok = live && yy >= 0 && yy < p.H;
        const unsigned soff = rok ? xbase + (unsigned)((long)(R0 + r) * p.W * p.x_pitch * 4) : nrec_x;
#pragma unroll
        for (int cc = 0; cc < 6; ++cc) {
          unsigned vo = xlane + (unsigned)((long)cc * p.x_pitch * 4);
          if (cc == 0) vo = (q.gx == 0 && tcol == 0) ? nrec_x : vo;
          if (cc == 5) vo = (q.gx == p.grow - 1 && tcol == tlast) ? nrec_x : vo;
          d[r][cc] = __builtin_bit_cast(float, __builtin_amdgcn_raw_buffer_load_b32(rsrc_x, vo, soff, 0));
        }
      }
      if (r_hi == 5 && ph + 1 < nph) gnext(gq);
    };
    f32x2 T[3][3];
    auto stage1 = [&](int cp) {
      auto D = [&](int rr) { return f32x2{d[rr - R0][2 * cp], d[rr - R0][2 * cp + 1]}; };
      if (HALF == 0) {
        T[0][cp] = fma2(4.f, D(0), fma2(-5.f, D(2), D(4)));
        const f32x2 a = fma2(-4.f, D(2), D(4)), b = fma2(-4.f, D(1), D(3));
        T[1][cp] = a + b;
        T[2][cp] = a - b;
      } else {
        const f32x2 cd = D(4) - D(2), f = D(3) - D(1);
        T[0][cp] = fma2(2.f, f, cd);
        T[1][cp] = fma2(-2.f, f, cd);
        T[2][cp] = fma2(4.f, D(1), fma2(-5.f, D(3), D(5)));
      }
    };
    auto stage2 = [&](float* obuf, int i, int part) {
      float* v = obuf + xwr + i * (6 * 128);
      const float t0 = T[i][0][0], t1 = T[i][0][1], t2 = T[i][1][0], t3 = T[i][1][1], t4 = T[i][2][0], t5 = T[i][2][1];
      if (part == 0) {
        const float a = __builtin_fmaf(-4.f, t2, t4), b = __builtin_fmaf(-4.f, t1, t3);
        v[0 * 128] = __builtin_fmaf(4.f, t0, __builtin_fmaf(-5.f, t2, t4));
        v[1 * 128] = a + b;
        v[2 * 128] = a - b;
      } else {
        const float cd = t4 - t2, f = t3 - t1;
        v[3 * 128] = __builtin_fmaf(2.f, f, cd);
        v[4 * 128] = __builtin_fmaf(-2.f, f, cd);
        v[5 * 128] = __builtin_fmaf(4.f, t1, __builtin_fmaf(-5.f, t3, t5));
      }
    };
    load_rows(0, 0, 5);
#pragma unroll
    for (int cp = 0; cp < 3; ++cp) stage1(cp);
#pragma unroll
    for (int i = 0; i < 3; ++i) {
      stage2(smem, i, 0);
      stage2(smem, i, 1);
    }
    load_rows(1, 0, 5);
    __syncthreads();
    auto phase = [&](int ph, auto cur_c) {
      constexpr int cur = decltype(cur_c)::value;
      const float* const ocur = smem + cur * OPB;
      float* const onxt = smem + (cur ^ 1) * OPB;
      f32x2 af = *reinterpret_cast<const f32x2*>(ocur + ard);
      f32x2 bf = *reinterpret_cast<const f32x2*>(ocur + brd);
#pragma unroll
      for (int e = 0; e < 9; ++e) {
        mfma_step(ocur, e, af, bf);
        if (!(W4W_EXP & 2)) {
          if (e < 3) stage1(e);
          else stage2(onxt, (e - 3) >> 1, (e - 3) & 1);
        }
        if (e == 3 && !(W4W_EXP & 4)) load_rows(ph + 2, 0, 3);
        if (e == 4 && !(W4W_EXP & 4)) load_rows(ph + 2, 3, 5);
        __builtin_amdgcn_sched_barrier(0);
      }
      __syncthreads();
    };
    for (int ph = 0; ph < nph; ph += 2) {
      phase(ph, std::integral_constant<int, 0>{});
      if (ph + 1 < nph) phase(ph + 1, std::integral_constant<int, 1>{});
    }
  };

  if (wid < 4) body_y();
  else if (wid & 1) body_x(std::integral_constant<int, 1>{});
  else body_x(std::integral_constant<int, 0>{});

  float* const Bs = smem + 2 * MH;
  if (p.bias && wid < 4) Bs[wid * 64 + lane] = bsum;
  const long n_w = (long)p.Nw * 9 * p.Cw;
  float* const slab = p.out + (long)split * p.slab;
  float* const Mh = smem + nh * MH;
  const int th = tid & 255;
  const int ec = th & 31, eg = (th >> 5) & 3, erow = __builtin_amdgcn_readfirstlane(th >> 7);
// ... 39 lines not shown
      }
      finish(0, X0);
      finish(1, X1);
    } else {
      f32x4 X2[6];
#pragma unroll
      for (int j = 0; j < 6; ++j) {
        const f32x4 s12 = add4(m(1, j), m(2, j)), s34 = add4(m(3, j), m(4, j));
        X2[j] = add4(fma4(k6, s34, s12 * (-k6)), m(5, j));
      }
      finish(2, X2);
    }
  }
}

__global__ __launch_bounds__(512, 2) void wino4_wgrad_kernel(const WArgs p) { wino4_wgrad_body(p, (int)blockIdx.x); }

__global__ __launch_bounds__(512, 2) void wino4_wgrad2_kernel(const WArgs pa, const WArgs pb, const int na) {
  if ((int)blockIdx.x < na) wino4_wgrad_body(pa, (int)blockIdx.x);
  else wino4_wgrad_body(pb, (int)blockIdx.x - na);
}

__global__ __launch_bounds__(512, 2) void wino4_wgrad4_kernel(const WArgs p0, const WArgs p1, const WArgs p2, const WArgs p3,
                                                               const int e0, const int e1, const int e2) {
  const int b = (int)blockIdx.x;
  if (b < e0) wino4_wgrad_body(p0, b);
  else if (b < e1) wino4_wgrad_body(p1, b - e0);
  else if (b < e2) wino4_wgrad_body(p2, b - e1);
  else wino4_wgrad_body(p3, b - e2);
}

struct WArgs8 {
  WArgs p[8];
  int e[7];
};
__global__ __launch_bounds__(512, 2) void wino4_wgrad8_kernel(const WArgs8 a) {
  const int b = (int)blockIdx.x;
  int k = 0;
#pragma unroll
  for (int i = 0; i < 7; ++i) k += b >= a.e[i] ? 1 : 0;
  const int base = k == 0 ? 0 : a.e[k - 1];
  wino4_wgrad_body(a.p[k], b - base);
}

}

bool lgm_wino4_wgrad_supported(const LgmConvGeom* g) {
  if (!(g->KH == 3 && g->KW == 3 && g->stride == 1 && g->pad == 1)) return false;
  if (g->Nw % 64 != 0 || g->Cw % 32 != 0) return false;
  const bool row_groups = g->W % 16 == 0 && g->H % 4 == 0, square_groups = g->W % 8 == 0 && g->H % 8 == 0;
  const bool image_groups = g->H == 4 && g->W == 4 && g->B % 4 == 0;
  if (!row_groups && !square_groups && !image_groups) return false;
  const long groups = (long)g->B * g->H * g->W / 64;
  return groups >= 4;
}

bool lgm_wino4_wgrad_use(const LgmConvGeom* g) {
  static const bool off = lgm_env_set("LGM_NO_WINO4_WGRAD") || lgm_env_set("LGM_NO_WINO4");
  return !off && lgm_wino4_wgrad_supported(g) && lgm_conv3x3_wino4_preferred(g, 1) != 0;
}

void lgm_wino4_wgrad_plan(const LgmConvGeom* g, long budget, int* splits, int* gps, int* total_groups) {
  const long groups = (long)g->B * g->H * g->W / 64;
  const long blocks = (long)(g->Nw / 64) * (g->Cw / 32);
  long smax = groups / 2 < budget ? groups / 2 : budget;
  if (smax < 2) smax = 2;
  long s = 2, best = -1;
  for (long c = 2; c <= smax; ++c) {
    const long rounds = (blocks * c + budget - 1) / budget;
    const long cost = rounds * ((groups + c - 1) / c + 6);
    if (best < 0 || cost < best) {
      best = cost;
      s = c;
    }
  }
  long per = (groups + s - 1) / s;
  s = (groups + per - 1) / per;
  *splits = (int)s;
  *gps = (int)per;
  *total_groups = (int)groups;
}

static void wino4_wgrad_prepare(const LgmConvGeom* g, const float* y, long y_pitch, const float* x, long x_pitch, float* out,
                                int bias, long slab, int splits, int gps, int total, lgmwino4w::WArgs& p) {
  p = lgmwino4w::WArgs{};
  p.y = y; p.x = x; p.out = out; p.bias = bias; p.slab = slab; p.y_pitch = y_pitch; p.x_pitch = x_pitch;
  p.B = g->B; p.H = g->H; p.W = g->W; p.Nw = g->Nw; p.Cw = g->Cw;
  p.tiles_c = g->Cw / 32;
  p.splits = splits; p.gps = gps; p.total_groups = total;
  p.sq = (g->H == 4 && g->W == 4) ? 2 : (g->W % 16 != 0) ? 1 : 0;
  static const int xcd_order = lgm_env_int("LGM_W4W_XCD", 1);
  p.xcd_order = xcd_order;
  p.grow = p.sq == 2 ? 1 : p.sq ? g->W / 8 : g->W / 16;
  p.trows = p.sq == 2 ? 1 : p.sq ? g->H / 8 : g->H / 4;
}

static constexpr size_t kW4Smem = (size_t)(2 * lgmwino4w::MH + 256) * sizeof(float);

int lgm_wino4_wgrad_launch(const LgmConvGeom* g, const float* y, long y_pitch, const float* x, long x_pitch, float* out,
                           int bias, long slab, int splits, int gps, int total, hipStream_t s) {
  using namespace lgmwino4w;
  WArgs p;
  wino4_wgrad_prepare(g, y, y_pitch, x, x_pitch, out, bias, slab, splits, gps, total, p);
  const unsigned nblocks = (unsigned)((g->Nw / 64) * (g->Cw / 32) * splits);
  static bool attr = false;
  if (!attr) {
    (void)hipFuncSetAttribute(reinterpret_cast<const void*>(wino4_wgrad_kernel), hipFuncAttributeMaxDynamicSharedMemorySize,
                              (int)kW4Smem);
    attr = true;
  }
  lgm_note_kernel(LGM_KNAME("lgmwino4w::wino4_wgrad_kernel"));
  hipLaunchKernelGGL(wino4_wgrad_kernel, dim3(nblocks), dim3(512), kW4Smem, s, p);
  LGM_LAUNCH_CHECK();
  return LGM_OK;
}

int lgm_wino4_wgradn_launch(int n, const LgmConvGeom* const* gs, const float* const* ys, const long* yps,
                            const float* const* xs, const long* xps, float* const* outs, const int* biases, const long* slabs,
                            const int* splits, const int* gpss, const int* totals, hipStream_t s) {
  using namespace lgmwino4w;
  WArgs pp[8];
  unsigned nb[8] = {0, 0, 0, 0, 0, 0, 0, 0};
  for (int k = 0; k < n; ++k) {
    wino4_wgrad_prepare(gs[k], ys[k], yps[k], xs[k], xps[k], outs[k], biases[k], slabs[k], splits[k], gpss[k], totals[k], pp[k]);
    nb[k] = (unsigned)((gs[k]->Nw / 64) * (gs[k]->Cw / 32) * splits[k]);
  }
  for (int k = n; k < 8; ++k) pp[k] = pp[n - 1];
  if (n > 4) {
    static bool attr = false;
    if (!attr) {
      (void)hipFuncSetAttribute(reinterpret_cast<const void*>(wino4_wgrad8_kernel), hipFuncAttributeMaxDynamicSharedMemorySize,
                                (int)kW4Smem);
      attr = true;
    }
    WArgs8 a8;
    unsigned tot = 0;
    for (int k = 0; k < 8; ++k) {
      a8.p[k] = pp[k];
      tot += nb[k];
      if (k < 7) a8.e[k] = (int)tot;
    }
    lgm_note_kernel(LGM_KNAME("lgmwino4w::wino4_wgrad8_kernel"));
    hipLaunchKernelGGL(wino4_wgrad8_kernel, dim3(tot), dim3(512), kW4Smem, s, a8);
  } else if (n == 2) {
    static bool attr = false;
    if (!attr) {
      (void)hipFuncSetAttribute(reinterpret_cast<const void*>(wino4_wgrad2_kernel), hipFuncAttributeMaxDynamicSharedMemorySize,
                                (int)kW4Smem);
      attr = true;
    }
    lgm_note_kernel(LGM_KNAME("lgmwino4w::wino4_wgrad2_kernel"));
    hipLaunchKernelGGL(wino4_wgrad2_kernel, dim3(nb[0] + nb[1]), dim3(512), kW4Smem, s, pp[0], pp[1], (int)nb[0]);
  } else {
    static bool attr = false;
    if (!attr) {
      (void)hipFuncSetAttribute(reinterpret_cast<const void*>(wino4_wgrad4_kernel), hipFuncAttributeMaxDynamicSharedMemorySize,
                                (int)kW4Smem);
      attr = true;
    }
    const int e0 = (int)nb[0], e1 = e0 + (int)nb[1], e2 = e1 + (int)nb[2];
    lgm_note_kernel(LGM_KNAME("lgmwino4w::wino4_wgrad4_kernel"));
    hipLaunchKernelGGL(wino4_wgrad4_kernel, dim3(nb[0] + nb[1] + nb[2] + nb[3]), dim3(512), kW4Smem, s, pp[0], pp[1], pp[2],
                       pp[3], e0, e1, e2);
  }
  LGM_LAUNCH_CHECK();
  return LGM_OK;
}

extern "C" int64_t lgm_conv3x3_wino4_wgrad_supported(const LgmConvGeom* g) {
  return (g && lgm_wino4_wgrad_supported(g)) ? 1 : 0;
}

extern "C" int64_t lgm_conv3x3_wino4_wgrad_workspace(const LgmConvGeom* g) {
  if (!g || !lgm_wino4_wgrad_supported(g)) return 0;
  int splits, gps, total;
  lgm_wino4_wgrad_plan(g, lgm_cu_budget(), &splits, &gps, &total);
  return (int64_t)splits * ((int64_t)g->Nw * 9 * g->Cw + g->Nw) * (int64_t)sizeof(float);
}

extern "C" int lgm_conv3x3_wino4_wgrad(const LgmConvGeom* g, const float* y, int64_t y_pitch, const float* x, int64_t x_pitch,
                                       float* gw, float* gbias, float beta, void* workspace, int64_t workspace_bytes,
                                       int64_t* desc, void* stream) {
  LGM_REQUIRE(g && y && x && gw && workspace && desc, "conv3x3_wino4_wgrad: null pointer");
  LGM_REQUIRE(lgm_wino4_wgrad_supported(g), "conv3x3_wino4_wgrad: unsupported geometry");
  LGM_REQUIRE(y_pitch % 4 == 0 && x_pitch % 4 == 0 && y_pitch >= g->Nw && x_pitch >= g->Cw && lgm_aligned16(y) && lgm_aligned16(x) &&
              lgm_aligned16(gw) && lgm_aligned16(workspace) && (!gbias || lgm_aligned16(gbias)) &&
              ((long)g->B * g->H * g->W + g->W + 1) * x_pitch < (1L << 29) && (long)g->B * g->H * g->W * y_pitch < (1L << 29),
              "conv3x3_wino4_wgrad: 16-byte aligned operands with pitch %% 4 == 0 inside 32-bit offsets expected");
  int splits, gps, total;
  lgm_wino4_wgrad_plan(g, lgm_cu_budget(), &splits, &gps, &total);
  const long n_w = (long)g->Nw * 9 * g->Cw, slab = n_w + g->Nw;
  LGM_REQUIRE(workspace_bytes >= (int64_t)splits * slab * (int64_t)sizeof(float), "conv3x3_wino4_wgrad: workspace too small");
  if (int rc = lgm_wino4_wgrad_launch(g, y, y_pitch, x, x_pitch, (float*)workspace, gbias ? 1 : 0, slab, splits, gps, total,
                                      (hipStream_t)stream))
    return rc;
  union { float f; int64_t i; } bb;
  bb.i = 0;
  bb.f = beta;
  desc[0] = (int64_t)(uintptr_t)workspace; desc[1] = slab; desc[2] = (int64_t)(uintptr_t)gw; desc[3] = n_w;
  desc[4] = (int64_t)(uintptr_t)gbias; desc[5] = gbias ? g->Nw : 0; desc[6] = splits; desc[7] = bb.i;
  return LGM_OK;
}
```

lightning-generative-models_amd/csrc/winograd4l.hip:

```cpp
#include <stdlib.h>

#include <type_traits>

#include "wino4_host.h"

namespace lgmwino4l {
using namespace lgmwino4dev;

constexpr int NT = 16;
constexpr int VBUF = NXI * 128;
constexpr int MBUF = NXI * NT * 32;

template <int CLS>
struct Geo;
template <>
struct Geo<0> {
  static constexpr int NI = 1, TTH = 2, TTW = 8, PH = 10, PW = 34, RS = 34, IMG = PH * RS, PLANE = 353;
};
template <>
struct Geo<1> {
  static constexpr int NI = 1, TTH = 4, TTW = 4, PH = 18, PW = 18, RS = 20, IMG = PH * RS, PLANE = 385;
};
template <>
struct Geo<2> {
  static constexpr int NI = 4, TTH = 2, TTW = 2, PH = 10, PW = 10, RS = 10, IMG = 112, PLANE = 449;
};

struct Args : ConvArgs {
  float* stats;
};

template <int CLS, bool STATS = false>
__global__ __launch_bounds__(256, 2) void wino4l_conv_kernel(const Args p) {
  using GE = Geo<CLS>;
  constexpr int NI = GE::NI, PH = GE::PH, PW = GE::PW, RS = GE::RS, IMG = GE::IMG, PLANE = GE::PLANE;
  constexpr int RBUF = 8 * PLANE;
  constexpr int NPIX = NI * PH * PW;
  constexpr int NJ = (2 * NPIX + 255) / 256;
  static_assert(NJ >= 1 && NJ <= 4, "the commit is dealt out over the last NJ steps");
  static_assert(2 * RBUF + 2 * VBUF <= MBUF, "the epilogue exchange sets the LDS size");
  extern __shared__ __align__(16) float smem[];
  float* const Rb = smem;
  float* const Vb = smem + 2 * RBUF;
  float* const Mb = smem;
  const int tid = threadIdx.x;
  const int lane = tid & 63;
  const int wid = __builtin_amdgcn_readfirstlane(tid >> 6);

  const ConvUnit un = conv_unit(p);
  const int tn = un.tn, split = un.split, twi = un.twi, thi = un.thi, bg = un.bg;
  const int n0 = tn * 64;
  const int h0 = thi * (4 * GE::TTH), w0 = twi * (4 * GE::TTW), b0 = bg * NI;
  const int ncc = p.C / KC;
  const int cc0 = split * p.pps;
  const int cc1 = min(ncc, cc0 + p.pps);
  const int nph = cc1 - cc0;

  const unsigned nrec_a = (unsigned)((long)p.B * p.H * p.W * p.a_pitch * 4);
  const __amdgpu_buffer_rsrc_t rsrc_a = wave_buffer_rsrc(p.a, nrec_a);
  unsigned goff[NJ], plds[NJ];
#pragma unroll
  for (int j = 0; j < NJ; ++j) {
    const int s = tid + 256 * j;
    const int pix = s >> 1, q = s & 1;
    unsigned g = nrec_a, l = (unsigned)(q * 4 * PLANE + NI * IMG);
    if (pix < NPIX) {
      const int img = pix / (PH * PW);
      const int rem = pix - img * (PH * PW);
      const int py = rem / PW, px = rem - py * PW;
      const int gy = h0 - 1 + py, gx = w0 - 1 + px;
      l = (unsigned)(q * 4 * PLANE + img * IMG + py * RS + px);
      if (gy >= 0 && gy < p.H && gx >= 0 && gx < p.W)
        g = (unsigned)((((long)(b0 + img) * p.H + gy) * p.W + gx) * p.a_pitch + q * 4) * 4u;
    }
    goff[j] = g;
    plds[j] = l;
  }
  u32x4 rp[NJ];
  auto fetch1 = [&](int j, int ph) -> u32x4 {
    const unsigned soff = (unsigned)((cc0 + ph) * (KC * 4));
    return __builtin_amdgcn_raw_buffer_load_b128(rsrc_a, ph < nph ? goff[j] : nrec_a, soff, 0);
  };
  auto commit_r = [&](float* rbuf, int j, const u32x4 r) {
    float* d = rbuf + plds[j];
    const f32x4 f = __builtin_bit_cast(f32x4, r);
    d[0] = f[0];
    d[PLANE] = f[1];
    d[2 * PLANE] = f[2];
    d[3 * PLANE] = f[3];
  };
  u32x4 rq0[NJ], rq1[NJ];
#pragma unroll
  for (int j = 0; j < NJ; ++j) rq0[j] = fetch1(j, 0);
#pragma unroll
  for (int j = 0; j < NJ; ++j) rq1[j] = fetch1(j, 1);
#pragma unroll
  for (int j = 0; j < NJ; ++j) rp[j] = fetch1(j, 2);

  const int half = wid >> 1;
  const int tk = (lane & 3) + 4 * (lane >> 5);
  const int t_tile = 8 * (wid & 1) + ((lane >> 2) & 7);
  int t_img, t_ty, t_tx;
  if (CLS == 0) {
    t_img = 0;
    t_ty = t_tile >> 3;
    t_tx = t_tile & 7;
  } else if (CLS == 1) {
    t_img = 0;
    t_ty = t_tile >> 2;
    t_tx = t_tile & 3;
  } else {
    t_img = t_tile >> 2;
    t_ty = (t_tile >> 1) & 1;
    t_tx = t_tile & 1;
  }
  const int trd = tk * PLANE + t_img * IMG + 4 * t_ty * RS + 4 * t_tx;
  const int vwr = (tk >> 2) * 64 + t_tile * 4 + (tk & 3) + half * (18 * 128);

  const int xg = wid;
  const int mt = lane & 15, kk = lane >> 4;
  const int vrd = xg * (9 * 128) + (kk >> 1) * 64 + mt * 4 + 2 * (kk & 1);
  const __amdgpu_buffer_rsrc_t rsrc_u = wave_buffer_rsrc(p.u, (unsigned)((long)p.N * p.C * NXI * 4));
  const unsigned ulane = (unsigned)((((kk >> 1) * 32 + mt) * 4 + 2 * (kk & 1)) * 4);
  const unsigned ubase = (unsigned)((tn * ncc + cc0) * NXI + xg * 9) * 2048u;
  unsigned pf = 0;
  {
    const unsigned ubytes = min((unsigned)nph * (NXI * 2048u), 2u << 20);
    const unsigned nx = gridDim.x >> 3;
    const unsigned spatial = (unsigned)(p.nbg * p.tb_h * p.tb_w);
    const unsigned grp = p.tn_slowest ? 1u : (unsigned)(p.tiles_n * p.splits);
    const unsigned share = p.tn_slowest ? ((unsigned)blockIdx.x >> 3) % spatial : ((unsigned)blockIdx.x >> 3) / grp;
    const unsigned nshare = p.tn_slowest ? min(nx, spatial) : nx / grp;
    const unsigned off = (share * 256u + (unsigned)tid) * 128u;
    if (p.xcd_ranges && (gridDim.x & 7) == 0 && off < ubytes && nshare * 256u * 128u >= ubytes)
      pf = __builtin_amdgcn_raw_buffer_load_b32(rsrc_u, off, (unsigned)((tn * ncc + cc0) * NXI) * 2048u, 0);
  }
  struct UF {
    f32x2 c[4];
  };
  auto load_u = [&](int ph, int e) -> UF {
    const unsigned soff = ubase + (unsigned)(ph * NXI + e) * 2048u;
    UF r;
#pragma unroll
    for (int cb = 0; cb < 4; ++cb) {
      const u32x2 v = __builtin_amdgcn_raw_buffer_load_b64(rsrc_u, ulane + (unsigned)(((cb & 1) * 64 + (cb >> 1) * 16) * 16), soff, 0);
      r.c[cb] = __builtin_bit_cast(f32x2, v);
    }
    return r;
  };

  auto body = [&](auto half_c) {
    constexpr int HALF = decltype(half_c)::value;
    f32x4 acc[9][4];
#pragma unroll
    for (int e = 0; e < 9; ++e)
#pragma unroll
// ... 289 lines not shown
```

lightning-generative-models_amd/lgm_hip/nn.py:

```python
from __future__ import annotations

import math
from typing import Optional

import torch
from torch import nn

from . import ops
from .flat import FlatParams, _r4


def _flat(p: nn.Parameter) -> FlatParams:
    fp = getattr(p, "_lgm_flat", None)
    if fp is None:
        raise RuntimeError("parameter is not bound to flat HIP storage; call prepare() on the network first")
    return fp


class GradCtx:

    def __init__(self, flat: FlatParams, transposed: bool = True, defer: bool = False):
        self.flat = flat
        self.beta0 = flat.begin_backward()
        self.written = set()
        self.deferred = [] if defer else None
        self._pending = []
        self._pending1 = []
        self._keep = []
        if defer:
            ops.lib().lgm_wgrad_queue_enable(-1)
        if transposed:
            flat.refresh_transposed()

    def flush(self):
        self.finish_pending()
        if self.deferred:
            ops.wgrad_reduce_batch(self.deferred, self.flat.device)

    def queue_wgrad(self, g, gy, x, gw_ptr: int, beta: float, gb_ptr):
        new = (g, gy, x, gw_ptr, beta, gb_ptr)
        if self._pending and not ops.wgrad_group_supported([e[0] for e in self._pending] + [g]):
            self._finish_pending3x3()
        self._pending.append(new)
        if len(self._pending) == ops.WGRAD_GROUP:
            self._finish_pending3x3()

    def _finish_pending3x3(self):
        pend, self._pending = self._pending, []
        if len(pend) == 1:
            e = pend[0]
            ops.conv_wgrad(e[0], e[1], e[2], e[3], e[4], e[5], defer=self.deferred)
        elif pend:
            ops.conv_wgrad_group(pend, self.deferred)

    def finish_pending(self):
        self._finish_pending3x3()
        self.finish_pending1x1()
        if self._keep:
            ops.wgrad_queue_flush()
            self._keep.clear()

    def queue_wgrad1x1(self, g, gy, x, gw_ptr: int, beta: float, gb_ptr):
        new = (g, gy, x, gw_ptr, beta, gb_ptr)
        for q in self._pending1:
            if ops.wgrad1x1_group_supported([e[0] for e in q] + [g]):
                q.append(new)
                if len(q) == 4:
                    self._pending1.remove(q)
                    ops.conv_wgrad1x1_group(q, self.deferred)
                return
        self._pending1.append([new])

    def finish_pending1x1(self):
        queues, self._pending1 = self._pending1, []
        for pend in queues:
            if len(pend) == 1:
                e = pend[0]
                ops.conv_wgrad(e[0], e[1], e[2], e[3], e[4], e[5], defer=self.deferred)
            else:
                ops.conv_wgrad1x1_group(pend, self.deferred)

    def defer_for(self, p: nn.Parameter):
        return self.deferred if id(p) not in self.written else None

    def beta(self, p: nn.Parameter) -> float:
        k = id(p)
        if k in self.written:
            return 1.0
        self.written.add(k)
        return self.beta0


class Conv2d(nn.Module):

    transposed = False

    def __init__(self, cin, cout, k, stride=1, padding=0, bias=True):
        super().__init__()
        self.cin, self.cout, self.k, self.stride, self.padding = cin, cout, k, stride, padding
        self.weight = nn.Parameter(torch.empty(cout, cin, k, k))
        nn.init.kaiming_uniform_(self.weight, a=math.sqrt(5))
        if bias:
            bound = 1 / math.sqrt(cin * k * k)
            self.bias = nn.Parameter(torch.empty(cout).uniform_(-bound, bound))
        else:
            self.register_parameter("bias", None)
        self._geoms = {}

    def geom(self, B, H, W):
        key = (B, H, W)
        g = self._geoms.get(key)
        if g is None:
            g = ops.make_geom(B, H, W, _r4(self.cin), _r4(self.cout), self.k, self.k, self.stride, self.padding)
            self._geoms[key] = g
        return g

    def out_shape(self, x):
        B, H, W, _ = x.shape
        g = self.geom(B, H, W)
        return (B, g.Ho, g.Wo, _r4(self.cout))

    def fwd_planes(self, x, groups: int):
        B, H, W, C = x.shape
        assert C == _r4(self.cin), f"conv expects {_r4(self.cin)} (padded) channels, got {C}"
        g = self.geom(B, H, W)
        fp = _flat(self.weight)
        y = ops.new((B, g.Ho, g.Wo, _r4(self.cout)), x)
        if self.k == 3 and self.stride == 1:
            st = ops.conv_xy_stats(g, x, fp.ptr(self.weight), fp.ptr(self.bias) if self.bias is not None else None, y,
                                   groups)
            if st is not None:
                return y, st
        ok = self.k == 3 and ops.gn_planes_ok(B, g.Ho * g.Wo, _r4(self.cout), groups)
        pl = ops.conv_xy(g, x, fp.ptr(self.weight), fp.ptr(self.bias) if self.bias is not None else None, None, y,
                         partial=ok)
        return y, pl

    def fwd(self, x, out=None, res=None, stats=False, act=0, slope=0.0):
        B, H, W, C = x.shape
        assert C == _r4(self.cin), f"conv expects {_r4(self.cin)} (padded) channels, got {C}"
        g = self.geom(B, H, W)
        fp = _flat(self.weight)
        y = out if out is not None else ops.new((B, g.Ho, g.Wo, _r4(self.cout)), x)
        if stats and self.bias is None and res is None:
            return y, ops.conv_stats(0, g, x, fp.ptr(self.weight), y)
        ops.conv_xy(g, x, fp.ptr(self.weight), fp.ptr(self.bias) if self.bias is not None else None, res, y,
                    post=ops.make_post(act, slope))
        return (y, (None, 0)) if stats else y

    def bwd(self, gc: GradCtx, x, gy, gx=None, accumulate=False, need_gx=True, res=None, planes_for_groups=0,
            mask=None, mask_slope=0.0, bn_sums=None):
        B, H, W, _ = x.shape
        g = self.geom(B, H, W)
        fp = gc.flat
        dfr = gc.defer_for(self.weight)
        bw = gc.beta(self.weight)
        gb = None
        if self.bias is not None:
            bb = gc.beta(self.bias)
            if bb == bw:
                gb = fp.gptr(self.bias)
            else:
                ops.colsum(gy, fp.gptr(self.bias), bb)
        if need_gx:
            if gx is None:
                gx = ops.new(x.shape, x)
                accumulate = False
            assert not (accumulate and res is not None)
            if accumulate:
                res = gx
        if need_gx and self.k == 3 and mask is None and bn_sums is None:
            ok_pl = bool(planes_for_groups) and res is None and ops.gn_planes_ok(B, H * W, x.shape[-1], planes_for_groups)
            r = ops.conv_bwd_pair(g, gy, x, fp.ptr(self.weight), fp.gptr(self.weight), bw, gb, dfr, res, gx, partial=ok_pl)
            if r is not False:
                return (gx, r) if planes_for_groups else gx
        if (need_gx and self.k == 1 and mask is None and bn_sums is None and not planes_for_groups and dfr is not None
                and ops.wgrad1x1_queueable(g, gy, x)):
            gc.queue_wgrad1x1(g, gy, x, fp.gptr(self.weight), bw, gb)
            ops.conv_yx(g, gy, fp.ptr(self.weight), None, res, gx, fp.tptr(self.weight))
            return gx
        if need_gx and (self.k != 3 or mask is not None or bn_sums is not None) and not planes_for_groups and not ops.B3:
            if ops._weng_take(g, fp.ptr(self.weight), res, False) is not None:
                ops.conv_wgrad(g, gy, x, fp.gptr(self.weight), bw, gb, defer=dfr)
                ops.conv_yx(g, gy, fp.ptr(self.weight), None, None, gx, fp.tptr(self.weight),
                            post=ops.make_post(0, 0.0, mask, mask_slope, bn=bn_sums), post_mask=mask)
                return gx
            if dfr is not None:
                gc._keep.append((gy, x))
            ops.conv_bwd_generic(g, gy, x, fp.ptr(self.weight), fp.tptr(self.weight), fp.gptr(self.weight), bw, gb, dfr,
                                 res, gx, post=ops.make_post(0, 0.0, mask, mask_slope, bn=bn_sums),
                                 post_mask=mask, queue=dfr is not None)
            return gx
        if dfr is not None and self.k == 3 and ops.wgrad_queueable(g, gy, x):
            gc.queue_wgrad(g, gy, x, fp.gptr(self.weight), bw, gb)
        else:
            if dfr is not None:
                gc._keep.append((gy, x))
            ops.conv_wgrad(g, gy, x, fp.gptr(self.weight), bw, gb, defer=dfr, queue=dfr is not None)
        if not need_gx:
            return None
        if planes_for_groups:
            ok = self.k == 3 and res is None and ops.gn_planes_ok(B, H * W, x.shape[-1], planes_for_groups)
            return gx, ops.conv_yx(g, gy, fp.ptr(self.weight), None, res, gx, fp.tptr(self.weight), partial=ok)
        ops.conv_yx(g, gy, fp.ptr(self.weight), None, res, gx, fp.tptr(self.weight),
                    post=ops.make_post(0, 0.0, mask, mask_slope, bn=bn_sums), post_mask=mask)
        return gx


def _conv_linear(self, x, out=None):
    B, H, W, _ = x.shape
    g = self.geom(B, H, W)
    fp = _flat(self.weight)
    y = out if out is not None else ops.new((B, g.Ho, g.Wo, _r4(self.cout)), x)
    ops.conv_xy(g, x, fp.ptr(self.weight), None, None, y)
    return y


def _conv_dgrad(self, gy, in_shape, gx=None, accumulate=False, mask=None, mask_slope=0.0, bn_sums=None):
    B, H, W, _ = in_shape
    g = self.geom(B, H, W)
    fp = _flat(self.weight)
    if gx is None:
        gx = ops.new(tuple(in_shape), gy)
        accumulate = False
    ops.conv_yx(g, gy, fp.ptr(self.weight), None, gx if accumulate else None, gx,
                post=ops.make_post(0, 0.0, mask, mask_slope, bn=bn_sums), post_mask=mask)
    return gx


def _conv_wgrad(self, gc: GradCtx, y, x):
    B, H, W, _ = x.shape
    ops.conv_wgrad(self.geom(B, H, W), y, x, gc.flat.gptr(self.weight), gc.beta(self.weight), None)


Conv2d.linear = _conv_linear
Conv2d.dgrad = _conv_dgrad
Conv2d.wgrad = _conv_wgrad


class ConvTranspose2d(nn.Module):

    def __init__(self, cin, cout, k, stride=1, padding=0, bias=True):
        super().__init__()
        self.cin, self.cout, self.k, self.stride, self.padding = cin, cout, k, stride, padding
        self.weight = nn.Parameter(torch.empty(cin, cout, k, k))
        nn.init.kaiming_uniform_(self.weight, a=math.sqrt(5))
        if bias:
            bound = 1 / math.sqrt(cout * k * k)
            self.bias = nn.Parameter(torch.empty(cout).uniform_(-bound, bound))
        else:
            self.register_parameter("bias", None)
        self._geoms = {}

    def geom(self, B, Hin, Win):
        key = (B, Hin, Win)
        g = self._geoms.get(key)
        if g is None:
            H = (Hin - 1) * self.stride - 2 * self.padding + self.k
            W = (Win - 1) * self.stride - 2 * self.padding + self.k
            g = ops.make_geom(B, H, W, _r4(self.cout), _r4(self.cin), self.k, self.k, self.stride, self.padding)
            assert g.Ho == Hin and g.Wo == Win
            self._geoms[key] = g
        return g

    def fwd(self, x, out=None, res=None, stats=False, act=0, slope=0.0):
        B, H, W, C = x.shape
        assert C == _r4(self.cin)
        g = self.geom(B, H, W)
        fp = _flat(self.weight)
        y = out if out is not None else ops.new((B, g.H, g.W, _r4(self.cout)), x)
        if stats and self.bias is None and res is None:
            return y, ops.conv_stats(1, g, x, fp.ptr(self.weight), y)
        ops.conv_yx(g, x, fp.ptr(self.weight), fp.ptr(self.bias) if self.bias is not None else None, res, y,
                    post=ops.make_post(act, slope))
        return (y, (None, 0)) if stats else y

    def bwd(self, gc: GradCtx, x, gy, gx=None, accumulate=False, need_gx=True, res=None, mask=None, mask_slope=0.0,
            bn_sums=None):
        B, H, W, _ = x.shape
        g = self.geom(B, H, W)
        fp = gc.flat
        dfr = gc.defer_for(self.weight)
        ops.conv_wgrad(g, x, gy, fp.gptr(self.weight), gc.beta(self.weight), defer=dfr)
        if self.bias is not None:
            dfb = gc.defer_for(self.bias)
            ops.colsum(gy, fp.gptr(self.bias), gc.beta(self.bias), defer=dfb)
        if not need_gx:
            return None
        if gx is None:
            gx = ops.new(x.shape, x)
            accumulate = False
        if accumulate:
            assert res is None
            res = gx
        ops.conv_xy(g, gy, fp.ptr(self.weight), None, res, gx, post=ops.make_post(0, 0.0, mask, mask_slope, bn=bn_sums),
                    post_mask=mask)
        return gx


class Linear(nn.Module):

    def __init__(self, cin, cout, bias=True):
        super().__init__()
        self.cin, self.cout = cin, cout
        self.weight = nn.Parameter(torch.empty(cout, cin))
        nn.init.kaiming_uniform_(self.weight, a=math.sqrt(5))
        bound = 1 / math.sqrt(cin)
        if bias:
            self.bias = nn.Parameter(torch.empty(cout).uniform_(-bound, bound))
        else:
            self.register_parameter("bias", None)
        self._geoms = {}

    def geom(self, B):
        g = self._geoms.get(B)
        if g is None:
            g = ops.make_geom(B, 1, 1, _r4(self.cin), _r4(self.cout), 1, 1, 1, 0)
# ... 60 lines not shown
```

lightning-generative-models_amd/lgm_hip/ops.py:

```python
from __future__ import annotations

import ctypes
from typing import Optional

import torch

from ._lib import ConvGeom, lib

ACT_NONE, ACT_SILU, ACT_GELU, ACT_RELU, ACT_LRELU, ACT_TANH = 0, 1, 2, 3, 4, 5


def stream() -> int:
    return torch.cuda.current_stream().cuda_stream


def _p(t: Optional[torch.Tensor]) -> Optional[int]:
    return None if t is None else t.data_ptr()


def pitch(t: torch.Tensor) -> int:
    assert t.stride(-1) == 1 or t.shape[-1] == 1, "last dim must be dense"
    if t.dim() == 1:
        return t.shape[0]
    pt = t.stride(-2)
# ... 160 lines not shown
            return (addr, fp.pstride) if addr % 16 == 0 else None
    return None


def _b3_supported(g: ConvGeom, mode: int, a_pitch: int) -> bool:
    key = (g.B, g.H, g.W, g.Cw, g.Nw, g.KH, g.stride, g.pad, mode, a_pitch)
    return _memo(_B3_OK, key, lambda: bool(g.KH == 3 and g.KW == 3 and
                                           lib().lgm_conv3x3_bf16x3_supported(ctypes.byref(g), mode, a_pitch)))


WINO = _os.environ.get("LGM_NO_WINO", "0") != "1"
_WINO_FLATS = []
_WINO_OK = _plan_cache()
_WINO_WS = _plan_cache()
_WINO_FITS = _plan_cache()


def register_wino_flat(fp):
    import weakref as _wr
    _WINO_FLATS[:] = [r for r in _WINO_FLATS if r() is not None]
    _WINO_FLATS.append(_wr.ref(fp))


def _wino_u(w_ptr: Optional[int], backward: bool, f4: bool = False):
    if w_ptr is None:
        return None
    for ref in _WINO_FLATS:
        fp = ref()
        if fp is None:
            continue
        off = w_ptr - fp.data.data_ptr()
        if 0 <= off < 4 * fp.total:
            return (fp.wino4_u if f4 else fp.wino_u)(off // 4, backward) if off % 4 == 0 else None
    return None


def _wino_supported(g: ConvGeom, yx: int) -> bool:
    key = (g.B, g.H, g.W, g.Cw, g.Nw, g.KH, g.KW, g.stride, g.pad, yx)
    return _memo(_WINO_OK, key, lambda: bool(g.KH == 3 and g.KW == 3 and
                                             lib().lgm_conv3x3_wino_supported(ctypes.byref(g), yx)))


WINO4 = _os.environ.get("LGM_NO_WINO4", "0") != "1"
_WINO4_OK = _plan_cache()


def _wino4_preferred(g: ConvGeom, yx: int) -> bool:
    key = (g.B, g.H, g.W, g.Cw, g.Nw, g.KH, g.KW, g.stride, g.pad, yx)
    return _memo(_WINO4_OK, key, lambda: bool(WINO4 and g.KH == 3 and g.KW == 3 and
                                              lib().lgm_conv3x3_wino4_preferred(ctypes.byref(g), yx)))


def _wino_fits(g: ConvGeom, a, out, res, bias_ptr) -> bool:
    if a.data_ptr() % 16 or out.data_ptr() % 16 or pitch(a) % 4 or pitch(out) % 4 or (bias_ptr or 0) % 16:
        return False
    if res is not None and (res.data_ptr() % 16 or pitch(res) % 4):
        return False
    key = (g.B, g.H, g.W, pitch(a), pitch(out), pitch(res) if res is not None else 0)
    return _memo(_WINO_FITS, key, lambda: bool(lib().lgm_conv3x3_wino_fits(ctypes.byref(g), *key[3:])))


_F22 = ("lgm_conv3x3_wino", "lgm_conv3x3_wino_workspace", "lgm_conv3x3_wino_workspace_partial")
_F44 = ("lgm_conv3x3_wino4", "lgm_conv3x3_wino4_workspace", "lgm_conv3x3_wino4_workspace")


def _wino_call(kind, yx: int, g: ConvGeom, a, u_ptr: int, bias_ptr, res, out, partial: bool = False):
    if not _wino_fits(g, a, out, res, bias_ptr):
        return False
    L = lib()
    launch, ws_query, ws_query_partial = kind
    n = _memo(_WINO_WS, (g.B, g.H, g.W, g.Cw, g.Nw, yx, launch, partial),
              lambda: getattr(L, ws_query_partial if partial else ws_query)(ctypes.byref(g), yx))
    ws = workspace(n, a.device) if n > 0 else None
    wsa = (None, 0) if ws is None else (ws.data_ptr(), ws.numel() * 4)
    if partial:
        assert res is None
        part = (ctypes.c_int64 * 2)()
        getattr(L, launch + "_partial")(yx, ctypes.byref(g), a.data_ptr(), pitch(a), u_ptr, bias_ptr, out.data_ptr(),
                                        pitch(out), *wsa, ctypes.addressof(part), stream())
        return (ws.data_ptr(), int(part[1]), int(part[0])) if part[0] > 1 else True
    getattr(L, launch)(yx, ctypes.byref(g), a.data_ptr(), pitch(a), u_ptr, bias_ptr, _p(res),
                       pitch(res) if res is not None else 0, out.data_ptr(), pitch(out), *wsa, stream())
    return True


_EPI_STATS = _plan_cache()


def conv_xy_stats(g: ConvGeom, x, w_ptr: Optional[int], bias_ptr, y, groups: int):
    if not (WINO and WINO4 and _WINO_FLATS and not B3) or g.KH != 3 or g.KW != 3 or w_ptr is None:
        return None

    def plan():
        n, per = 0, ctypes.c_int(0)
        C = g.Nw
        if (_wino4_preferred(g, 0) and C % groups == 0 and 64 % (C // groups) == 0
                and not lib().lgm_gn_fwd_fused_supported(g.B, g.H * g.W, C, groups)):
            n = int(lib().lgm_conv3x3_wino4_stats_floats(ctypes.byref(g), ctypes.addressof(per)))
        return (n, int(per.value))
    n, per = _memo(_EPI_STATS, (g.B, g.H, g.W, g.Cw, g.Nw, groups), plan)
    if n <= 0 or not _wino_fits(g, x, y, None, bias_ptr):
        return None
    u = _wino_u(w_ptr, False, f4=True)
    if u is None:
        return None
    st = torch.empty(n, dtype=torch.float32, device=x.device)
    with _timed("igemm_xy", g):
        lib().lgm_conv3x3_wino4_stats(ctypes.byref(g), x.data_ptr(), pitch(x), u, bias_ptr, y.data_ptr(), pitch(y),
                                      st.data_ptr(), n, stream())
    return ("stats", st, per, bias_ptr)


def _conv_ws(g: ConvGeom, yx: int, device):
    key = (g.B, g.H, g.W, g.Cw, g.Nw, g.KH, g.stride, g.pad, yx)
    n = _memo(_CONV_WS_BYTES, key, lambda: lib().lgm_conv_workspace(ctypes.byref(g), yx))
    return workspace(n, device) if n > 0 else None


PLANES = _os.environ.get("LGM_NO_PLANES", "0") != "1"
POSTOPS = _os.environ.get("LGM_NO_POSTOP", "0") != "1"


class PostOp(ctypes.Structure):
    _fields_ = [("act", ctypes.c_int32), ("slope", ctypes.c_float), ("mask", ctypes.c_void_p),
                ("mask_pitch", ctypes.c_int64), ("mask_slope", ctypes.c_float),
                ("bn_a", ctypes.c_void_p), ("bn_a_pitch", ctypes.c_int64), ("bn_mean", ctypes.c_void_p),
                ("bn_rstd", ctypes.c_void_p), ("bn_partial", ctypes.c_void_p), ("bn_partial_floats", ctypes.c_int64),
                ("bn_tiles", ctypes.c_void_p)]


BN_EPI = _os.environ.get("LGM_NO_BN_EPI", "0") != "1"


class BnSums:
    __slots__ = ("a", "mean", "rstd", "partial", "_tiles")

    def __init__(self, a, mean, rstd):
        self.a, self.mean, self.rstd = a, mean, rstd
        r, C = rows(a), a.shape[-1]
        self.partial = torch.empty((r + 63) // 64 * 3 * C, dtype=torch.float32, device=a.device)
        self._tiles = ctypes.c_int32(0)

    @property
    def tiles(self) -> int:
        return int(self._tiles.value)


def make_post(act: int = 0, slope: float = 0.0, mask: Optional[torch.Tensor] = None, mask_slope: float = 0.0,
              bn: Optional[BnSums] = None):
    if bn is not None and not BN_EPI:
        bn = None
    if act == 0 and mask is None and bn is None:
        return None
    assert act in (0, ACT_RELU, ACT_LRELU)
    po = PostOp(act, slope, None if mask is None else mask.data_ptr(), 0 if mask is None else pitch(mask), mask_slope)
    if bn is not None:
        po.bn_a, po.bn_a_pitch = bn.a.data_ptr(), pitch(bn.a)
        po.bn_mean, po.bn_rstd = bn.mean.data_ptr(), bn.rstd.data_ptr()
        po.bn_partial, po.bn_partial_floats = bn.partial.data_ptr(), bn.partial.numel()
        po.bn_tiles = ctypes.addressof(bn._tiles)
    return po


def _apply_post_separately(post: PostOp, out, mask):
    if post.act:
        act_fwd(out, None, None, out, post.act, post.slope)
# ... 164 lines not shown

_PAIR_SLABS = {}


WGRAD_QUEUE = _os.environ.get("LGM_NO_WGRAD_QUEUE", "0") != "1"


def wgrad_queue_flush():
    with _timed("wgrad"):
        lib().lgm_wgrad_queue_flush()


def conv_wgrad(g: ConvGeom, y, x, gw_ptr: int, beta: float, gbias_ptr: Optional[int] = None, defer=None, queue: bool = False):
    L = lib()
    queue = queue and defer is not None and WGRAD_QUEUE
    nbytes = L.lgm_conv_wgrad_workspace(ctypes.byref(g))
    with _timed("wgrad", g):
        if defer is None:
            ws = workspace(nbytes, y.device)
            L.lgm_conv_wgrad(ctypes.byref(g), y.data_ptr(), pitch(y), x.data_ptr(), pitch(x), gw_ptr, gbias_ptr, beta,
                             ws.data_ptr(), ws.numel() * 4, stream())
            return
        ws = _persistent((gw_ptr, nbytes), nbytes, y.device)
        desc = (ctypes.c_int64 * 8)()
        if queue:
            L.lgm_wgrad_queue_enable(1)
        try:
            L.lgm_conv_wgrad_deferred(ctypes.byref(g), y.data_ptr(), pitch(y), x.data_ptr(), pitch(x), gw_ptr, gbias_ptr,
                                      beta, ws.data_ptr(), ws.numel() * 4, ctypes.addressof(desc), stream())
        finally:
            if queue:
                L.lgm_wgrad_queue_enable(0)
        if desc[6] > 1:
            defer.append(tuple(desc))


_PAIR_OK = _plan_cache()


WGRAD2 = _os.environ.get("LGM_NO_WGRAD2", "0") != "1"
WGRAD_GROUP = max(2, min(8, int(_os.environ.get("LGM_WGRAD_GROUP", "4"))))
_WG2_OK = _plan_cache()
_WG2_WS = _plan_cache()

WGRAD1X1_GROUP = _os.environ.get("LGM_NO_WGRAD1X1_GROUP", "0") != "1"
_W1G_OK = _plan_cache()
_W1G_WS = _plan_cache()

_WGRAD3X3 = ("lgm_conv3x3_wino_wgradn", _WG2_OK, _WG2_WS)
_WGRAD1X1 = ("lgm_wgrad1x1_group", _W1G_OK, _W1G_WS)


class WgradItem(ctypes.Structure):
    _fields_ = [("g", ctypes.c_void_p), ("y", ctypes.c_void_p), ("y_pitch", ctypes.c_int64), ("x", ctypes.c_void_p),
                ("x_pitch", ctypes.c_int64), ("gw", ctypes.c_void_p), ("gbias", ctypes.c_void_p), ("beta", ctypes.c_float),
                ("ws", ctypes.c_void_p), ("ws_bytes", ctypes.c_int64), ("desc", ctypes.c_void_p)]


def _gkey(g: ConvGeom):
    return (g.B, g.H, g.W, g.Cw, g.Nw, g.KH, g.KW, g.stride, g.pad)


def _geom_array(geoms):
    arr = (ctypes.c_void_p * len(geoms))()
    for i, g in enumerate(geoms):
        arr[i] = ctypes.addressof(g)
    return arr


def _group_supported(kind, geoms) -> bool:
    launch, ok, _ = kind

    def ask():
        arr = _geom_array(geoms)
        return bool(getattr(lib(), launch + "_supported")(len(geoms), ctypes.addressof(arr)))
    return _memo(ok, tuple(_gkey(g) for g in geoms), ask)


def _wgrad_group(kind, entries, defer):
    L = lib()
    launch, _, sizes = kind
    n = len(entries)
    geoms = [e[0] for e in entries]

    def plan():
        out = (ctypes.c_int64 * n)()
        arr = _geom_array(geoms)
        getattr(L, launch + "_workspaces")(n, ctypes.addressof(arr), ctypes.addressof(out))
        return tuple(max(int(out[k]), int(L.lgm_conv_wgrad_workspace(ctypes.byref(g)))) for k, g in enumerate(geoms))
    need = _memo(sizes, tuple(_gkey(g) for g in geoms), plan)
    items = (WgradItem * n)()
    descs = []
    for k, (g, gy, x, gw_ptr, beta, gb_ptr) in enumerate(entries):
        ws = _persistent((gw_ptr, need[k]), need[k], gy.device)
        desc = (ctypes.c_int64 * 8)()
        descs.append(desc)
        items[k] = WgradItem(ctypes.addressof(g), gy.data_ptr(), pitch(gy), x.data_ptr(), pitch(x), gw_ptr, gb_ptr, beta,
                             ws.data_ptr(), ws.numel() * 4, ctypes.addressof(desc))
    with _timed("wgrad", geoms):
        getattr(L, launch)(n, ctypes.addressof(items), stream())
    for desc in descs:
        if desc[6] > 1:
            defer.append(tuple(desc))


def wgrad_group_supported(geoms) -> bool:
    return _group_supported(_WGRAD3X3, geoms)


def wgrad1x1_group_supported(geoms) -> bool:
    return _group_supported(_WGRAD1X1, geoms)


def conv_wgrad_group(entries, defer):
    _wgrad_group(_WGRAD3X3, entries, defer)


def conv_wgrad1x1_group(entries, defer):
    _wgrad_group(_WGRAD1X1, entries, defer)


def wgrad2_supported(ga: ConvGeom, gb: ConvGeom) -> bool:
    return wgrad_group_supported([ga, gb])


def conv_wgrad2(a, b, defer):
    conv_wgrad_group([a, b], defer)


def wgrad_queueable(g: ConvGeom, gy, x) -> bool:
    if not (WGRAD2 and WINO and _WINO_FLATS and not B3 and _wino4_preferred(g, 1)):
        return False
    if gy.data_ptr() % 16 or x.data_ptr() % 16 or pitch(gy) % 4 or pitch(x) % 4:
        return False
    return wgrad_group_supported([g, g])


def wgrad1x1_queueable(g: ConvGeom, gy, x) -> bool:
    if not WGRAD1X1_GROUP or B3 or g.KH != 1 or g.KW != 1 or g.stride != 1 or g.pad != 0:
        return False
    if gy.data_ptr() % 16 or x.data_ptr() % 16 or pitch(gy) % 4 or pitch(x) % 4:
        return False
    return wgrad1x1_group_supported([g, g])


def conv_bwd_pair(g: ConvGeom, gy, x, w_ptr: int, gw_ptr: int, beta: float, gbias_ptr: Optional[int], defer, res, gx,
                  partial: bool = False):
    if not (WINO and _WINO_FLATS and not B3) or g.KH != 3 or g.KW != 3:
        return False
    if _wino4_preferred(g, 1) and _wino_u(w_ptr, True, f4=True) is not None:
        return False
    u = _wino_u(w_ptr, True)
    if u is None:
        return False
    if gy.data_ptr() % 16 or x.data_ptr() % 16 or gx.data_ptr() % 16 or (gbias_ptr or 0) % 16 or gw_ptr % 16:
        return False
    if res is not None and res.data_ptr() % 16:
        return False
    key = (g.B, g.H, g.W, g.Cw, g.Nw, pitch(gy), pitch(x), pitch(gx), pitch(res) if res is not None else 0)
    if not _memo(_PAIR_OK, key, lambda: bool(lib().lgm_conv3x3_wino_bwd_supported(ctypes.byref(g), *key[5:]))):
        return False
    L = lib()
    partial = bool(partial and PLANES and res is None)

    def plan():
        two = (ctypes.c_int64 * 2)()
        L.lgm_conv3x3_wino_bwd_workspaces(ctypes.byref(g), 1 if partial else 0, ctypes.addressof(two))
        return (int(two[0]), int(two[1]))
    n, nbytes = _memo(_WINO_WS, (g.B, g.H, g.W, g.Cw, g.Nw, "pair", partial), plan)
    dws = workspace(n, gy.device) if n > 0 else None
    with _timed("bwd_pair", g, 2.0):
        wws, desc = _slabs(gw_ptr, nbytes, defer, gy.device)
        part = (ctypes.c_int64 * 2)() if partial else None
        L.lgm_conv3x3_wino_bwd(ctypes.byref(g), gy.data_ptr(), pitch(gy), x.data_ptr(), pitch(x), u, _p(res),
                               pitch(res) if res is not None else 0, gx.data_ptr(), pitch(gx),
                               None if dws is None else dws.data_ptr(), 0 if dws is None else dws.numel() * 4,
                               None if part is None else ctypes.addressof(part), gw_ptr, gbias_ptr, beta, wws.data_ptr(),
                               wws.numel() * 4, None if desc is None else ctypes.addressof(desc), stream())
    if desc is not None and desc[6] > 1:
        defer.append(tuple(desc))
    if part is not None and part[0] > 1:
        return (dws.data_ptr(), int(part[1]), int(part[0]), None)
    return None
# ... 517 lines not shown
```

lightning-generative-models_amd/models/generative/diffusion/ddpm.py:

```python
from __future__ import annotations

import math
import os
import random
from collections import namedtuple
from typing import List, Optional, Tuple

import torch
from torch import nn

from lgm_hip import ops
from lgm_hip.flat import FlatParams, _r4
from lgm_hip.lightning import LightningModule, multi_rank
from lgm_hip.nn import Conv2d, GradCtx, GroupNorm, Linear, RMSNorm, param_kind
from lgm_hip.optim import EMA, FusedAdam


ModelPrediction = namedtuple("ModelPrediction", ["pred_noise", "pred_x_start"])


_NO_RES_FOLD = os.environ.get("LGM_NO_RES_FOLD") is not None


def _chan(t: torch.Tensor, lo: int, hi: int) -> torch.Tensor:
# ... 116 lines not shown
        hidden = heads * dim_head
        self.norm = RMSNorm(dim)
        self.mem_kv = nn.Parameter(torch.randn(2, heads, num_mem_kv, dim_head))
        self.to_qkv = Conv2d(dim, hidden * 3, 1, bias=False)
        self.to_out = Conv2d(hidden, dim, 1)

    def fwd(self, x, out, save: bool):
        B, H, W, C = x.shape
        fp = self.mem_kv._lgm_flat
        r = ops.rms_qkv_fused(x, fp.ptr(self.norm.g), fp.ptr(self.to_qkv.weight), 3 * self.heads * self.dim_head)
        if r is not None:
            xn, qkv = r
        else:
            xn = self.norm.fwd(x)
            qkv = self.to_qkv.fwd(xn)
        ao = ops.new((B, H, W, self.heads * self.dim_head), x)
        lse = ops.attn_fwd(qkv, fp.ptr(self.mem_kv), self.heads, self.dim_head, self.M, ao)
        self.to_out.fwd(ao, out=out, res=x)
        return (x, xn, qkv, ao, lse) if save else None

    def bwd(self, gc: GradCtx, saved, gy, gx, accumulate: bool):
        x, xn, qkv, ao, lse = saved
        fp = gc.flat
        gao = self.to_out.bwd(gc, ao, gy)
        gqkv = ops.new(qkv.shape, qkv)
        dm = gc.defer_for(self.mem_kv)
        ops.attn_bwd(qkv, fp.ptr(self.mem_kv), ao, gao, lse, self.heads, self.dim_head, self.M, gqkv,
                     fp.gptr(self.mem_kv), gc.beta(self.mem_kv), defer=dm)
        gxn = self.to_qkv.bwd(gc, xn, gqkv)
        del gqkv, gao
        self.norm.bwd(gc, x, gxn, gx, accumulate, res=gy)
        return gx


class _DownConv(Conv2d):

    def __init__(self, dim, dim_out):
        super().__init__(dim, dim_out, 2, stride=2, padding=0)

    @property
    def ref_shape(self):
        return (self.cout, 4 * self.cin, 1, 1)

    def _save_to_state_dict(self, destination, prefix, keep_vars):
        super()._save_to_state_dict(destination, prefix, keep_vars)
        k = prefix + "weight"
        destination[k] = destination[k].reshape(self.ref_shape)

    def _load_from_state_dict(self, state_dict, prefix, local_metadata, strict, missing_keys, unexpected_keys, error_msgs):
        k = prefix + "weight"
        w = state_dict.get(k)
        if w is not None and tuple(w.shape) == self.ref_shape:
            state_dict = {kk: v for kk, v in state_dict.items() if kk.startswith(prefix)}
            state_dict[k] = w.reshape(self.weight.shape)
        super()._load_from_state_dict(state_dict, prefix, local_metadata, strict, missing_keys, unexpected_keys, error_msgs)


class _Down(nn.Module):

    def __init__(self, dim, dim_out):
        super().__init__()
        self.add_module("0", nn.Identity())
        self.add_module("1", _DownConv(dim, dim_out))

    def fwd(self, x, out, save):
        self._modules["1"].fwd(x, out=out)
        return (x,) if save else None

    def bwd(self, gc, saved, gy, gx, accumulate):
        (x,) = saved
        self._modules["1"].bwd(gc, x, gy, gx, accumulate)
        return gx


class _Up(nn.Module):

    def __init__(self, dim, dim_out):
        super().__init__()
        self.add_module("0", nn.Identity())
        self.add_module("1", Conv2d(dim, dim_out, 3, padding=1))

    def fwd(self, x, out, save):
        B, H, W, C = x.shape
        hi = ops.new((B, 2 * H, 2 * W, C), x)
        ops.upsample2x_fwd(x, hi)
        self._modules["1"].fwd(hi, out=out)
        return (hi,) if save else None

    def bwd(self, gc, saved, gy, gx, accumulate):
        (hi,) = saved
        ghi = self._modules["1"].bwd(gc, hi, gy)
        ops.upsample2x_bwd(ghi, gx, accumulate)
        return gx


class _PlainConv(Conv2d):

    def fwd_s(self, x, out, save):
        self.fwd(x, out=out)
        return (x,) if save else None

    def bwd_s(self, gc, saved, gy, gx, accumulate):
        (x,) = saved
        self.bwd(gc, x, gy, gx, accumulate)
        return gx


class Unet(nn.Module):
    def __init__(self, dim, init_dim=None, out_dim=None, dim_mults=(1, 2, 4, 8), channels=3,
                 self_condition=False, resnet_block_groups=8, learned_variance=False,
                 learned_sinusoidal_cond=False, random_fourier_features=False,
                 learned_sinusoidal_dim=16, sinusoidal_pos_emb_theta=10000, attn_dim_head=32,
                 attn_heads=4, full_attn=None, flash_attn=False, num_classes=None):
        super().__init__()
        if num_classes is not None and int(num_classes) < 1:
            raise ValueError(f"num_classes must be a positive number of classes, got {num_classes!r}")
        if learned_variance or learned_sinusoidal_cond or random_fourier_features:
            raise NotImplementedError("HIP UNet covers the configuration the reference DDPM constructs "
                                      "(ddpm.py:984-987) and self-conditioning: no learned variance / fourier features")
        if init_dim not in (None, dim):
            raise NotImplementedError("init_dim != dim")
        self.dim, self.channels = dim, channels
        self.self_condition = bool(self_condition)
        self.random_or_learned_sinusoidal_cond = False
        self.theta = float(sinusoidal_pos_emb_theta)
        self.in_channels = channels * (2 if self.self_condition else 1)
        self.in_pitch = _r4(self.in_channels)
        self.x_off, self.sc_off = (channels, 0) if self.self_condition else (0, -1)
        self.init_conv = Conv2d(self.in_channels, dim, 7, padding=3)
        dims = [dim, *[dim * m for m in dim_mults]]
        in_out = list(zip(dims[:-1], dims[1:]))
        self.in_out = in_out
        time_dim = dim * 4
        self.time_dim = time_dim
        self.time_mlp = nn.Sequential(nn.Identity(), Linear(dim, time_dim), nn.Identity(), Linear(time_dim, time_dim))
        self.num_classes = None if num_classes is None else int(num_classes)
        if self.num_classes is not None:
            self.label_emb = nn.Embedding(self.num_classes + 1, time_dim)
        self._null_labels = {}
        n = len(in_out)
        if not full_attn:
            full_attn = (*((False,) * (n - 1)), True)
        heads = attn_heads if isinstance(attn_heads, tuple) else (attn_heads,) * n
        dheads = attn_dim_head if isinstance(attn_dim_head, tuple) else (attn_dim_head,) * n
        rb = lambda a, b: ResnetBlock(a, b, time_emb_dim=time_dim, groups=resnet_block_groups)
        self.downs = nn.ModuleList([])
        self.ups = nn.ModuleList([])
        for i, ((ci, co), fa, h, dh) in enumerate(zip(in_out, full_attn, heads, dheads)):
            last = i >= n - 1
            att = Attention(ci, heads=h, dim_head=dh) if fa else LinearAttention(ci, heads=h, dim_head=dh)
            self.downs.append(nn.ModuleList([rb(ci, ci), rb(ci, ci), att,
                                             _Down(ci, co) if not last else _PlainConv(ci, co, 3, padding=1)]))
        mid = dims[-1]
        self.mid_block1 = rb(mid, mid)
        self.mid_attn = Attention(mid, heads=heads[-1], dim_head=dheads[-1])
        self.mid_block2 = rb(mid, mid)
        for i, ((ci, co), fa, h, dh) in enumerate(zip(*map(reversed, (in_out, full_attn, heads, dheads)))):
            last = i == n - 1
            att = Attention(co, heads=h, dim_head=dh) if fa else LinearAttention(co, heads=h, dim_head=dh)
            self.ups.append(nn.ModuleList([rb(co + ci, co), rb(co + ci, co), att,
                                           _Up(co, ci) if not last else _PlainConv(co, ci, 3, padding=1)]))
        self.out_dim = out_dim if out_dim is not None else channels
        self.final_res_block = rb(dim * 2, dim)
        self.final_conv = Conv2d(dim, self.out_dim, 1)
        self._flat: Optional[FlatParams] = None

    def resblocks(self) -> List[ResnetBlock]:
        out = []
        for b1, b2, _, _ in self.downs:
            out += [b1, b2]
        out += [self.mid_block1, self.mid_block2]
        for b1, b2, _, _ in self.ups:
            out += [b1, b2]
        out.append(self.final_res_block)
# ... 876 lines not shown
```

Before: 13560 images/s.

## Fold nearest 2x upsample into Winograd F(4x4) conv forward, dgrad and wgrad

The Up block's nearest-neighbour 2x upsample is folded into the Winograd F(4x4) 3x3 conv kernels. The forward pass reads the low-res input at halved coordinates, and the data-grad pass sums each 2x2 output block into the low-res gradient, either in the epilogue or in a new split-K reduce kernel. The weight-grad pass reads the low-res activation through a half-resolution flag. This avoids materialising, writing and re-reading the high-res upsampled tensor and drops the separate upsample forward and backward kernels. The cost is extra kernel template variants, an extra LDS exchange with syncthreads in the fold epilogue, and fallbacks that re-materialise the upsample when a grouped or single wgrad cannot take the half-resolution path.

Result: no change. 13660 images/s, median of 6 (+0.7%).

```diff
diff --git a/include/lgm_hip.h b/include/lgm_hip.h
--- a/include/lgm_hip.h
+++ b/include/lgm_hip.h
@@ -412,6 +412,16 @@
 int64_t lgm_conv3x3_wino_wgradn_supported(int n, const LgmConvGeom* const* geoms);
 int lgm_conv3x3_wino_wgradn_workspaces(int n, const LgmConvGeom* const* geoms, int64_t* out);
 int lgm_conv3x3_wino_wgradn(int n, const LgmWgradItem* items, void* stream);
+int64_t lgm_conv3x3_wino4_up2_supported(const LgmConvGeom* g);
+int64_t lgm_conv3x3_wino4_up2_splits(const LgmConvGeom* g, int yx);
+int lgm_conv3x3_wino4_up2(int yx, const LgmConvGeom* g, const float* a, int64_t a_pitch, const float* u, const float* bias,
+                          const float* res, int64_t res_pitch, float* out, int64_t out_pitch, void* workspace,
+                          int64_t workspace_bytes, void* stream);
+int lgm_conv3x3_wino4_wgrad_up2(const LgmConvGeom* g, const float* y, int64_t y_pitch, const float* x, int64_t x_pitch,
+                                float* gw, float* gbias, float beta, void* workspace, int64_t workspace_bytes, int64_t* desc,
+                                void* stream);
+int64_t lgm_conv3x3_wino_wgradn_up2_supported(int n, const LgmConvGeom* const* geoms);
+int lgm_conv3x3_wino_wgradn_up2(int n, const LgmWgradItem* items, const int* x_half, void* stream);
 int lgm_conv3x3_wino_wgrad2_workspaces(const LgmConvGeom* ga, const LgmConvGeom* gb, int64_t* out);
 int lgm_conv3x3_wino_wgrad2(const LgmConvGeom* ga, const float* ya, int64_t ya_pitch, const float* xa, int64_t xa_pitch,
                             float* gwa, float* gba, float beta_a, void* wsa, int64_t wsa_bytes, int64_t* desca,
diff --git a/lightning-generative-models_amd/csrc/conv3x3.hip b/lightning-generative-models_amd/csrc/conv3x3.hip
--- a/lightning-generative-models_amd/csrc/conv3x3.hip
+++ b/lightning-generative-models_amd/csrc/conv3x3.hip
@@ -42,6 +42,32 @@
   f32x4 s = *reinterpret_cast<const f32x4*>(ws + m * N + n);
   for (int k = 1; k < splits; ++k) s += *reinterpret_cast<const f32x4*>(ws + (long)k * ws_stride + m * N + n);
   if (bias) s += *reinterpret_cast<const f32x4*>(bias + n);
+  if (res) s += *reinterpret_cast<const f32x4*>(res + m * res_pitch + n);
+  *reinterpret_cast<f32x4*>(out + m * out_pitch + n) = s;
+}
+
+__global__ __launch_bounds__(256) void splitk_reduce_up2_kernel(const float* __restrict__ ws, long ws_stride, int splits,
+                                                                const float* __restrict__ res, long res_pitch,
+                                                                float* __restrict__ out, long out_pitch, int B, int H, int W,
+                                                                int N) {
+  const int n4 = N / 4;
+  const long i = (long)blockIdx.x * blockDim.x + threadIdx.x;
+  if (i >= (long)B * H * W * n4) return;
+  const int n = (int)(i % n4) * 4;
+  long pix = i / n4;
+  const int w = (int)(pix % W);
+  pix /= W;
+  const int h = (int)(pix % H);
+  const int b = (int)(pix / H);
+  const long base = (((long)b * 2 * H + 2 * h) * 2 * W + 2 * w) * N + n;
+  const long rowp = (long)2 * W * N;
+  auto child = [&](long off) {
+    f32x4 s = *reinterpret_cast<const f32x4*>(ws + base + off);
+    for (int k = 1; k < splits; ++k) s += *reinterpret_cast<const f32x4*>(ws + (long)k * ws_stride + base + off);
+    return s;
+  };
+  f32x4 s = (child(0) + child(N)) + (child(rowp) + child(rowp + N));
+  const long m = ((long)b * H + h) * W + w;
   if (res) s += *reinterpret_cast<const f32x4*>(res + m * res_pitch + n);
   *reinterpret_cast<f32x4*>(out + m * out_pitch + n) = s;
 }
@@ -1165,6 +1191,15 @@
   const long items = M * (N / 4);
   hipLaunchKernelGGL(lgm3x3::splitk_reduce_kernel, dim3((unsigned)lgm_cdiv(items, 256)), dim3(256), 0, s, ws, ws_stride,
                      splits, bias, res, res_pitch, out, out_pitch, M, N);
+  LGM_LAUNCH_CHECK();
+  return LGM_OK;
+}
+
+int lgm_splitk_reduce_up2_launch(const float* ws, long ws_stride, int splits, const float* res, long res_pitch, float* out,
+                                 long out_pitch, int B, int H, int W, int N, hipStream_t s) {
+  const long items = (long)B * H * W * (N / 4);
+  hipLaunchKernelGGL(lgm3x3::splitk_reduce_up2_kernel, dim3((unsigned)lgm_cdiv(items, 256)), dim3(256), 0, s, ws, ws_stride,
+                     splits, res, res_pitch, out, out_pitch, B, H, W, N);
   LGM_LAUNCH_CHECK();
   return LGM_OK;
 }
diff --git a/lightning-generative-models_amd/csrc/lgm_internal.h b/lightning-generative-models_amd/csrc/lgm_internal.h
--- a/lightning-generative-models_amd/csrc/lgm_internal.h
+++ b/lightning-generative-models_amd/csrc/lgm_internal.h
@@ -11,6 +11,8 @@
                        hipStream_t s);
 int lgm_splitk_reduce_launch(const float* ws, long ws_stride, int splits, const float* bias, const float* res,
                              long res_pitch, float* out, long out_pitch, long M, int N, hipStream_t s);
+int lgm_splitk_reduce_up2_launch(const float* ws, long ws_stride, int splits, const float* res, long res_pitch, float* out,
+                                 long out_pitch, int B, int H, int W, int N, hipStream_t s);
 bool lgm_wgrad3x3_supported(const LgmConvGeom* g);
 void lgm_wgrad3x3_plan(const LgmConvGeom* g, int* splits, int* tps, int* total_ts);
 int lgm_wgrad3x3_launch(const LgmConvGeom* g, const float* y, long y_pitch, const float* x, long x_pitch, float* out,
@@ -54,6 +56,10 @@
 int lgm_wino4_launch(const LgmConvGeom* g, int yx, const float* a, long a_pitch, const float* u, const float* bias,
                      const float* res, long res_pitch, float* out, long out_pitch, void* workspace, long workspace_bytes,
                      hipStream_t s, int64_t* partial = nullptr, float* stats = nullptr);
+bool lgm_wino4_up2_supported(const LgmConvGeom* g);
+int lgm_wino4_up2_launch(const LgmConvGeom* g, int yx, const float* a, long a_pitch, const float* u, const float* bias,
+                         const float* res, long res_pitch, float* out, long out_pitch, void* workspace, long workspace_bytes,
+                         hipStream_t s);
 bool lgm_wino4l_supported(const LgmConvGeom* g, int gather_channels, int out_channels);
 long lgm_wino4l_units(const LgmConvGeom* g, int out_channels);
 int lgm_wino4l_stats_parts(const LgmConvGeom* g);
@@ -67,10 +73,11 @@
 bool lgm_wino4_wgrad_use(const LgmConvGeom* g);
 void lgm_wino4_wgrad_plan(const LgmConvGeom* g, long budget, int* splits, int* gps, int* total_groups);
 int lgm_wino4_wgrad_launch(const LgmConvGeom* g, const float* y, long y_pitch, const float* x, long x_pitch, float* out,
-                           int bias, long slab, int splits, int gps, int total, hipStream_t s);
+                           int bias, long slab, int splits, int gps, int total, hipStream_t s, int x_half = 0);
 int lgm_wino4_wgradn_launch(int n, const LgmConvGeom* const* gs, const float* const* ys, const long* yps,
                             const float* const* xs, const long* xps, float* const* outs, const int* biases,
-                            const long* slabs, const int* splits, const int* gpss, const int* totals, hipStream_t s);
+                            const long* slabs, const int* splits, const int* gpss, const int* totals, hipStream_t s,
+                            const int* x_half = nullptr);
 
 int lgm_linattn_ctx_launch(int mode, const float* qkv, long pitch, const float* mem_kv, const float* gout,
                            long gout_pitch, const float* ctx_in, int B, int n, int heads, int M, float scale,
diff --git a/lightning-generative-models_amd/csrc/wino4_device.h b/lightning-generative-models_amd/csrc/wino4_device.h
--- a/lightning-generative-models_amd/csrc/wino4_device.h
+++ b/lightning-generative-models_amd/csrc/wino4_device.h
@@ -51,7 +51,16 @@
   int xcd_ranges;
   float* ws;
   long ws_stride;
+  int a_half;
+  int out_half;
 };
+
+template <bool HALF>
+__device__ __forceinline__ unsigned patch_offset(const ConvArgs& p, int b, int gy, int gx, int q, unsigned none) {
+  if (!(gy >= 0 && gy < p.H && gx >= 0 && gx < p.W)) return none;
+  const int sh = HALF ? 1 : 0;
+  return (unsigned)((((long)b * (p.H >> sh) + (gy >> sh)) * (p.W >> sh) + (gx >> sh)) * p.a_pitch + q * 4) * 4u;
+}
 
 struct ConvUnit {
   int tn, split, twi, thi, bg;
diff --git a/lightning-generative-models_amd/csrc/wino4_host.h b/lightning-generative-models_amd/csrc/wino4_host.h
--- a/lightning-generative-models_amd/csrc/wino4_host.h
+++ b/lightning-generative-models_amd/csrc/wino4_host.h
@@ -64,8 +64,10 @@
 template <class F>
 int conv_launch(const LgmConvGeom* g, int yx, const float* a, long a_pitch, const float* u, const float* bias,
                 const float* res, long res_pitch, float* out, long out_pitch, void* workspace, long workspace_bytes,
-                hipStream_t s, int64_t* partial, float* stats) {
+                hipStream_t s, int64_t* partial, float* stats, int up2 = 0) {
   typename F::Args p{};
+  p.a_half = up2 == 1;
+  p.out_half = up2 == 2;
   p.stats = stats;
   p.a = a; p.u = u; p.bias = bias; p.res = res; p.out = out;
   p.a_pitch = a_pitch; p.res_pitch = res_pitch; p.out_pitch = out_pitch;
@@ -97,6 +99,9 @@
     LGM_LAUNCH_CHECK_AS(F::LAUNCHER);
     return LGM_OK;
   }
+  if (p.splits > 1 && p.out_half)
+    return lgm_splitk_reduce_up2_launch(p.ws, p.ws_stride, p.splits, res, res_pitch, out, out_pitch, g->B, g->H / 2, g->W / 2,
+                                        p.N, s);
   if (p.splits > 1)
     return lgm_splitk_reduce_launch(p.ws, p.ws_stride, p.splits, bias, res, res_pitch, out, out_pitch, M, p.N, s);
   LGM_LAUNCH_CHECK_AS(F::LAUNCHER);
diff --git a/lightning-generative-models_amd/csrc/winograd.hip b/lightning-generative-models_amd/csrc/winograd.hip
--- a/lightning-generative-models_amd/csrc/winograd.hip
+++ b/lightning-generative-models_amd/csrc/winograd.hip
@@ -1417,12 +1417,29 @@
   return lgm_conv3x3_wino_wgradn_workspaces(2, gs, out);
 }
 
-extern "C" int lgm_conv3x3_wino_wgradn(int n, const LgmWgradItem* it, void* stream) {
+extern "C" int64_t lgm_conv3x3_wino_wgradn_up2_supported(int n, const LgmConvGeom* const* geoms) {
+  return (geoms && wgradn_supported(n, geoms) && wgradn_use4(n, geoms)) ? 1 : 0;
+}
+
+static int wgradn_impl(int n, const LgmWgradItem* it, const int* x_half, void* stream);
+extern "C" int lgm_conv3x3_wino_wgradn(int n, const LgmWgradItem* it, void* stream) { return wgradn_impl(n, it, nullptr, stream); }
+extern "C" int lgm_conv3x3_wino_wgradn_up2(int n, const LgmWgradItem* it, const int* x_half, void* stream) {
+  LGM_REQUIRE(x_half, "conv3x3_wino_wgradn_up2: null pointer");
+  return wgradn_impl(n, it, x_half, stream);
+}
+
+static int wgradn_impl(int n, const LgmWgradItem* it, const int* x_half, void* stream) {
   using namespace lgmwino;
   LGM_REQUIRE(it && n >= 2 && n <= 8, "conv3x3_wino_wgradn: 2 ... 8 layers expected");
   const LgmConvGeom* gs[8];
   for (int k = 0; k < n; ++k) gs[k] = it[k].g;
   LGM_REQUIRE(wgradn_supported(n, gs), "conv3x3_wino_wgradn: unsupported group of layers");
+  if (x_half) {
+    for (int k = 0; k < n; ++k)
+      LGM_REQUIRE(!x_half[k] || (gs[k]->H % 2 == 0 && gs[k]->W % 2 == 0), "conv3x3_wino_wgradn_up2: layer %d: odd map", k);
+    LGM_REQUIRE(wgradn_use4(n, gs), "conv3x3_wino_wgradn_up2: this group does not run the F(4x4) kernel (ask "
+                "lgm_conv3x3_wino_wgradn_up2_supported)");
+  }
   for (int k = 0; k < n; ++k)
     LGM_REQUIRE(it[k].desc && it[k].ws && lgm_aligned16(it[k].ws) &&
                 wgrad2_operands_ok(it[k].g, it[k].y, it[k].y_pitch, it[k].x, it[k].x_pitch, it[k].gw, it[k].gbias),
@@ -1451,7 +1468,8 @@
       d[0] = (int64_t)(uintptr_t)it[k].ws; d[1] = slabs[k]; d[2] = (int64_t)(uintptr_t)it[k].gw; d[3] = n_w;
       d[4] = (int64_t)(uintptr_t)it[k].gbias; d[5] = it[k].gbias ? g->Nw : 0; d[6] = splits[k]; d[7] = bbits.i;
     }
-    return lgm_wino4_wgradn_launch(n, gs, ys, yps, xs, xps, outs, biases, slabs, splits, gpss, totals, (hipStream_t)stream);
+    return lgm_wino4_wgradn_launch(n, gs, ys, yps, xs, xps, outs, biases, slabs, splits, gpss, totals, (hipStream_t)stream,
+                                   x_half);
   }
   int G, ipc;
   wgrad_class(gs[0]->H, gs[0]->W, &G, &ipc);
diff --git a/lightning-generative-models_amd/csrc/winograd4.hip b/lightning-generative-models_amd/csrc/winograd4.hip
--- a/lightning-generative-models_amd/csrc/winograd4.hip
+++ b/lightning-generative-models_amd/csrc/winograd4.hip
@@ -51,8 +51,8 @@
   float* stats;
 };
 
-template <int CLS, bool DBG = false, int EXP = 0, bool STATS = false>
-__global__ __launch_bounds__(512, 2) void wino4_conv_kernel(const Args p) {
+template <int CLS, bool DBG, int EXP, bool STATS, int UPS>
+__device__ __forceinline__ void wino4_conv_body(const Args& p) {
   using GE = Geo<CLS>;
   constexpr bool PFU = LGM_WINO4_PFU != 0;
   int nstamp = 0;
@@ -87,7 +87,8 @@
   const int cc1 = min(ncc, cc0 + p.pps);
   const int nph = cc1 - cc0;
 
-  const unsigned nrec_a = (unsigned)((long)p.B * p.H * p.W * p.a_pitch * 4);
+  static_assert(UPS == 0 || (CLS < 3 && !DBG && !STATS), "upsample folds: classes 0-2 of the plain build");
+  const unsigned nrec_a = (unsigned)((long)p.B * (p.H >> (UPS == 1)) * (p.W >> (UPS == 1)) * p.a_pitch * 4);
   const __amdgpu_buffer_rsrc_t rsrc_a = wave_buffer_rsrc(p.a, nrec_a);
   unsigned goff[NJ], plds[NJ];
 #pragma unroll
@@ -101,8 +102,7 @@
       const int py = rem / PW, px = rem - py * PW;
       const int gy = h0 - HALO + py, gx = w0 - HALO + px;
       l = (unsigned)(q * 4 * PLANE + img * IMG + py * RS + px);
-      if (gy >= 0 && gy < p.H && gx >= 0 && gx < p.W)
-        g = (unsigned)((((long)(b0 + img) * p.H + gy) * p.W + gx) * p.a_pitch + q * 4) * 4u;
+      g = patch_offset<UPS == 1>(p, b0 + img, gy, gx, q, nrec_a);
     }
     goff[j] = g;
     plds[j] = l;
@@ -338,8 +338,10 @@
       e_ty = 0;
       e_tx = 0;
     }
-    const long opix = ((long)(b0 + e_img) * p.H + h0 + 4 * e_ty) * p.W + w0 + 4 * e_tx;
     const bool partial = p.splits > 1;
+    const bool fold = UPS == 2 && !partial;
+    const long opix = fold ? ((long)(b0 + e_img) * (p.H >> 1) + ((h0 + 4 * e_ty) >> 1)) * (p.W >> 1) + ((w0 + 4 * e_tx) >> 1)
+                           : ((long)(b0 + e_img) * p.H + h0 + 4 * e_ty) * p.W + w0 + 4 * e_tx;
     const int ncol0 = n0 + HALF * 16 + eq * 4;
     float* const obase = partial ? p.ws + (long)split * p.ws_stride + opix * p.N + ncol0 : p.out + opix * p.out_pitch + ncol0;
     const long opitch = partial ? (long)p.N : p.out_pitch;
@@ -378,6 +380,39 @@
       f32x4 bv = {0.f, 0.f, 0.f, 0.f};
       if (!partial && p.bias) bv = *reinterpret_cast<const f32x4*>(p.bias + ncol0 + rd * 32);
       f32x4 st1 = {0.f, 0.f, 0.f, 0.f}, st2 = {0.f, 0.f, 0.f, 0.f};
+      if constexpr (UPS == 2) {
+        if (fold) {
+          __syncthreads();
+          float* const hx = Mh + (et * 4 + eq) * 16;
+          f32x4 hh[2][2];
+#pragma unroll
+          for (int rr = 0; rr < 2; ++rr) {
+            const f32x4 s1 = add4(X[rr][1], X[rr][2]), d1 = sub4(X[rr][1], X[rr][2]);
+            const f32x4 s2 = add4(X[rr][3], X[rr][4]), d2 = sub4(X[rr][3], X[rr][4]);
+            const f32x4 y0 = add4(add4(add4(X[rr][0], s1), s2), bv), y1 = add4(fma4(2.f, d2, d1), bv);
+            const f32x4 y2 = add4(fma4(4.f, s2, s1), bv), y3 = add4(add4(fma4(8.f, d2, d1), X[rr][5]), bv);
+            hh[rr][0] = add4(y0, y1);
+            hh[rr][1] = add4(y2, y3);
+            if (rpair == 1) {
+              *reinterpret_cast<f32x4*>(hx + rr * 8) = hh[rr][0];
+              *reinterpret_cast<f32x4*>(hx + rr * 8 + 4) = hh[rr][1];
+            }
+          }
+          __syncthreads();
+          if (rpair == 0) {
+#pragma unroll
+            for (int rr = 0; rr < 2; ++rr)
+#pragma unroll
+              for (int k = 0; k < 2; ++k) {
+                const long o = (long)rr * (p.W >> 1) + k;
+                f32x4 v = add4(hh[rr][k], *reinterpret_cast<const f32x4*>(hx + rr * 8 + k * 4));
+                if (has_res) v = add4(v, *reinterpret_cast<const f32x4*>(rbase + o * p.res_pitch + rd * 32));
+                *reinterpret_cast<f32x4*>(obase + o * opitch + rd * 32) = v;
+              }
+          }
+          continue;
+        }
+      }
 #pragma unroll
       for (int rr = 0; rr < 2; ++rr) {
         const long orow = (long)(2 * rr + rpair) * p.W;
@@ -435,6 +470,15 @@
   };
   if (half == 0) body(std::integral_constant<int, 0>{});
   else body(std::integral_constant<int, 1>{});
+}
+
+template <int CLS, bool DBG = false, int EXP = 0, bool STATS = false>
+__global__ __launch_bounds__(512, 2) void wino4_conv_kernel(const Args p) {
+  wino4_conv_body<CLS, DBG, EXP, STATS, 0>(p);
+}
+template <int CLS, int UPS>
+__global__ __launch_bounds__(512, 2) void wino4_conv_up2_kernel(const Args p) {
+  wino4_conv_body<CLS, false, 0, false, UPS>(p);
 }
 
 __device__ __forceinline__ void ggt36(const float (&g)[9], float (&u)[36]) {
@@ -538,9 +582,34 @@
   static void go(const Args& p, size_t smem, hipStream_t s) {
     lgmwino4host::launch_kernel<wino4_conv_kernel<CLS, DBG, EXP, STATS>, THREADS>(p, smem, s);
   }
+  template <int CLS, int UPS>
+  static void go_up2(const Args& p, size_t smem, hipStream_t s) {
+    lgmwino4host::launch_kernel<wino4_conv_up2_kernel<CLS, UPS>, THREADS>(p, smem, s);
+  }
 };
 
 int Form::launch(Args& p, int cls, bool res, bool partial, bool stats, size_t smem, hipStream_t s) {
+  if (p.a_half || p.out_half) {
+    if (cls > 2 || stats || partial || (p.a_half && p.out_half)) {
+      lgm_set_error("wino4 (upsample fold): map classes 0-2, no statistics and no planes for the consumer expected");
+      return LGM_ERR_UNSUPPORTED;
+    }
+    p.dbg = nullptr;
+    if (p.a_half) {
+      lgm_note_kernel(cls == 0 ? LGM_KNAME("lgmwino4::wino4_conv_up2_kernel<0, 1>") : cls == 1 ? LGM_KNAME("lgmwino4::wino4_conv_up2_kernel<1, 1>")
+                               : LGM_KNAME("lgmwino4::wino4_conv_up2_kernel<2, 1>"));
+      if (cls == 0) go_up2<0, 1>(p, smem, s);
+      else if (cls == 1) go_up2<1, 1>(p, smem, s);
+      else go_up2<2, 1>(p, smem, s);
+    } else {
+      lgm_note_kernel(cls == 0 ? LGM_KNAME("lgmwino4::wino4_conv_up2_kernel<0, 2>") : cls == 1 ? LGM_KNAME("lgmwino4::wino4_conv_up2_kernel<1, 2>")
+                               : LGM_KNAME("lgmwino4::wino4_conv_up2_kernel<2, 2>"));
+      if (cls == 0) go_up2<0, 2>(p, smem, s);
+      else if (cls == 1) go_up2<1, 2>(p, smem, s);
+      else go_up2<2, 2>(p, smem, s);
+    }
+    return LGM_OK;
+  }
   p.dbg = (long long*)lgm_wino4_debug_buffer;
   if (p.dbg && lgm_wino4_debug_slots > 0) {
     if (lgm_wino4_debug_next >= lgm_wino4_debug_slots || p.units > 4095) p.dbg = nullptr;
@@ -675,6 +744,49 @@
                                 partial, stats);
 }
 
+bool lgm_wino4_up2_supported(const LgmConvGeom* g) {
+  if (g->H % 2 || g->W % 2) return false;
+  if (!w4h::supported<Form>(g, g->Cw, g->Nw) || !w4h::supported<Form>(g, g->Nw, g->Cw)) return false;
+  if (w4h::unit_class<Form>(g->H, g->W) > 2) return false;
+  if (wino4_use_light(g, g->Cw, g->Nw) || wino4_use_light(g, g->Nw, g->Cw)) return false;
+  return lgm_wino4_wgrad_supported(g);
+}
+
+int lgm_wino4_up2_launch(const LgmConvGeom* g, int yx, const float* a, long a_pitch, const float* u, const float* bias,
+                         const float* res, long res_pitch, float* out, long out_pitch, void* workspace, long workspace_bytes,
+                         hipStream_t s) {
+  return w4h::conv_launch<Form>(g, yx, a, a_pitch, u, bias, res, res_pitch, out, out_pitch, workspace, workspace_bytes, s,
+                                nullptr, nullptr, yx ? 2 : 1);
+}
+
+extern "C" int64_t lgm_conv3x3_wino4_up2_supported(const LgmConvGeom* g) {
+  return (g && lgm_wino4_up2_supported(g)) ? 1 : 0;
+}
+
+extern "C" int64_t lgm_conv3x3_wino4_up2_splits(const LgmConvGeom* g, int yx) {
+  if (!g || !lgm_wino4_up2_supported(g)) return 0;
+  return Form::splits(g, yx ? g->Nw : g->Cw, yx ? g->Cw : g->Nw);
+}
+
+extern "C" int lgm_conv3x3_wino4_up2(int yx, const LgmConvGeom* g, const float* a, int64_t a_pitch, const float* u,
+                                     const float* bias, const float* res, int64_t res_pitch, float* out, int64_t out_pitch,
+                                     void* workspace, int64_t workspace_bytes, void* stream) {
+  LGM_REQUIRE(g && a && u && out, "conv3x3_wino4_up2: null pointer");
+  LGM_REQUIRE(lgm_wino4_up2_supported(g), "conv3x3_wino4_up2: this layer keeps the materialised upsample (ask "
+              "lgm_conv3x3_wino4_up2_supported)");
+  const int gc = yx ? g->Nw : g->Cw, oc = yx ? g->Cw : g->Nw;
+  LGM_REQUIRE(!(yx && bias), "conv3x3_wino4_up2: the input gradient takes no bias");
+  LGM_REQUIRE(a_pitch % 4 == 0 && out_pitch % 4 == 0 && a_pitch >= gc && out_pitch >= oc && lgm_aligned16(a) && lgm_aligned16(u) &&
+              lgm_aligned16(out) && (!bias || lgm_aligned16(bias)) &&
+              (!res || (lgm_aligned16(res) && res_pitch % 4 == 0 && res_pitch >= oc)),
+              "conv3x3_wino4_up2: 16-byte aligned operands with pitch %% 4 == 0 expected");
+  const long pix = (long)g->B * g->H * g->W + g->W + 1;
+  LGM_REQUIRE(pix * a_pitch < (1L << 29) && pix * out_pitch < (1L << 29) && (!res || pix * res_pitch < (1L << 29)),
+              "conv3x3_wino4_up2: operands outside 32-bit offsets");
+  return lgm_wino4_up2_launch(g, yx, a, a_pitch, u, bias, res, res_pitch, out, out_pitch, workspace, workspace_bytes,
+                              (hipStream_t)stream);
+}
+
 extern "C" int64_t lgm_conv3x3_wino4_supported(const LgmConvGeom* g, int yx) {
   if (!g) return 0;
   return lgm_wino4_supported(g, yx ? g->Nw : g->Cw, yx ? g->Cw : g->Nw) ? 1 : 0;
diff --git a/lightning-generative-models_amd/csrc/winograd4_wgrad.hip b/lightning-generative-models_amd/csrc/winograd4_wgrad.hip
--- a/lightning-generative-models_amd/csrc/winograd4_wgrad.hip
+++ b/lightning-generative-models_amd/csrc/winograd4_wgrad.hip
@@ -29,6 +29,7 @@
   int trows;
   int xcd_order;
   int sq;
+  int x_half;
 };
 
 __device__ __forceinline__ void wino4_wgrad_body(const WArgs& p, const int bidx) {
@@ -57,9 +58,11 @@
   const int brd = YB + xg * (9 * 128) + lh * 64 + lr * 2;
 
   const unsigned nrec_y = (unsigned)((long)p.B * p.H * p.W * p.y_pitch * 4);
-  const unsigned nrec_x = (unsigned)(((long)p.B * p.H * p.W + p.W + 1) * p.x_pitch * 4);
+  const int xh = p.x_half;
+  const int Hx = p.H >> xh, Wx = p.W >> xh;
+  const unsigned nrec_x = (unsigned)(((long)p.B * Hx * Wx + Wx + 1) * p.x_pitch * 4);
   const __amdgpu_buffer_rsrc_t rsrc_y = wave_buffer_rsrc(p.y, nrec_y);
-  const __amdgpu_buffer_rsrc_t rsrc_x = wave_buffer_rsrc(p.x - (long)(p.W + 1) * p.x_pitch, nrec_x);
+  const __amdgpu_buffer_rsrc_t rsrc_x = wave_buffer_rsrc(p.x - (long)(Wx + 1) * p.x_pitch, nrec_x);
 
   struct GPos {
     int gx, ty, b;
@@ -84,6 +87,9 @@
   const int gh = p.sq == 1 ? 8 : 4, gw = p.sq == 1 ? 8 : p.sq == 2 ? 4 : 16;
   auto gpix = [&](const GPos& q) -> long {
     return ((long)(p.sq == 2 ? 4 * q.b : q.b) * p.H + gh * q.ty) * p.W + gw * q.gx;
+  };
+  auto gpix_x = [&](const GPos& q) -> long {
+    return ((long)(p.sq == 2 ? 4 * q.b : q.b) * Hx + ((gh * q.ty) >> xh)) * Wx + ((gw * q.gx) >> xh);
   };
   auto tile_row = [&](int tl) { return p.sq == 1 ? (tl >> 1) : 0; };
   auto tile_col = [&](int tl) { return p.sq == 1 ? (tl & 1) : p.sq == 2 ? 0 : tl; };
@@ -203,24 +209,24 @@
     const int trow = tile_row(tl), tcol = tile_col(tl);
     const int tlast = p.sq == 1 ? 1 : p.sq == 2 ? 0 : 3;
     const unsigned xlane =
-        (unsigned)(((((long)tile_img(tl) * p.H + 4 * trow) * p.W + 4 * tcol) * p.x_pitch + c0 + c) * 4);
+        (unsigned)(((((long)tile_img(tl) * Hx + ((4 * trow) >> xh)) * Wx + ((4 * tcol) >> xh)) * p.x_pitch + c0 + c) * 4);
     const int xwr = YB + (tl >> 1) * 64 + c * 2 + (tl & 1) + HALF * (18 * 128);
     constexpr int R0 = HALF ? 1 : 0;
     float d[5][6];
     GPos gq = gdecode(g_begin);
     auto load_rows = [&](int ph, int r_lo, int r_hi) {
       const GPos q = gq;
-      const unsigned xbase = (unsigned)(gpix(q) * p.x_pitch * 4);
+      const unsigned xbase = (unsigned)(gpix_x(q) * p.x_pitch * 4);
       const bool live = ph < nph;
 #pragma unroll
       for (int r = 0; r < 5; ++r) {
         if (r < r_lo || r >= r_hi) continue;
         const int yy = gh * q.ty + 4 * trow - 1 + R0 + r;
         const bool rok = live && yy >= 0 && yy < p.H;
-        const unsigned soff = rok ? xbase + (unsigned)((long)(R0 + r) * p.W * p.x_pitch * 4) : nrec_x;
+        const unsigned soff = rok ? xbase + (unsigned)((long)((R0 + r + xh) >> xh) * Wx * p.x_pitch * 4) : nrec_x;
 #pragma unroll
         for (int cc = 0; cc < 6; ++cc) {
-          unsigned vo = xlane + (unsigned)((long)cc * p.x_pitch * 4);
+          unsigned vo = xlane + (unsigned)((long)((cc + xh) >> xh) * p.x_pitch * 4);
           if (cc == 0) vo = (q.gx == 0 && tcol == 0) ? nrec_x : vo;
           if (cc == 5) vo = (q.gx == p.grow - 1 && tcol == tlast) ? nrec_x : vo;
           d[r][cc] = __builtin_bit_cast(float, __builtin_amdgcn_raw_buffer_load_b32(rsrc_x, vo, soff, 0));
@@ -426,8 +432,9 @@
 }
 
 static void wino4_wgrad_prepare(const LgmConvGeom* g, const float* y, long y_pitch, const float* x, long x_pitch, float* out,
-                                int bias, long slab, int splits, int gps, int total, lgmwino4w::WArgs& p) {
+                                int bias, long slab, int splits, int gps, int total, lgmwino4w::WArgs& p, int x_half = 0) {
   p = lgmwino4w::WArgs{};
+  p.x_half = x_half;
   p.y = y; p.x = x; p.out = out; p.bias = bias; p.slab = slab; p.y_pitch = y_pitch; p.x_pitch = x_pitch;
   p.B = g->B; p.H = g->H; p.W = g->W; p.Nw = g->Nw; p.Cw = g->Cw;
   p.tiles_c = g->Cw / 32;
@@ -442,10 +449,10 @@
 static constexpr size_t kW4Smem = (size_t)(2 * lgmwino4w::MH + 256) * sizeof(float);
 
 int lgm_wino4_wgrad_launch(const LgmConvGeom* g, const float* y, long y_pitch, const float* x, long x_pitch, float* out,
-                           int bias, long slab, int splits, int gps, int total, hipStream_t s) {
+                           int bias, long slab, int splits, int gps, int total, hipStream_t s, int x_half) {
   using namespace lgmwino4w;
   WArgs p;
-  wino4_wgrad_prepare(g, y, y_pitch, x, x_pitch, out, bias, slab, splits, gps, total, p);
+  wino4_wgrad_prepare(g, y, y_pitch, x, x_pitch, out, bias, slab, splits, gps, total, p, x_half);
   const unsigned nblocks = (unsigned)((g->Nw / 64) * (g->Cw / 32) * splits);
   static bool attr = false;
   if (!attr) {
@@ -461,12 +468,13 @@
 
 int lgm_wino4_wgradn_launch(int n, const LgmConvGeom* const* gs, const float* const* ys, const long* yps,
                             const float* const* xs, const long* xps, float* const* outs, const int* biases, const long* slabs,
-                            const int* splits, const int* gpss, const int* totals, hipStream_t s) {
+                            const int* splits, const int* gpss, const int* totals, hipStream_t s, const int* x_half) {
   using namespace lgmwino4w;
   WArgs pp[8];
   unsigned nb[8] = {0, 0, 0, 0, 0, 0, 0, 0};
   for (int k = 0; k < n; ++k) {
-    wino4_wgrad_prepare(gs[k], ys[k], yps[k], xs[k], xps[k], outs[k], biases[k], slabs[k], splits[k], gpss[k], totals[k], pp[k]);
+    wino4_wgrad_prepare(gs[k], ys[k], yps[k], xs[k], xps[k], outs[k], biases[k], slabs[k], splits[k], gpss[k], totals[k], pp[k],
+                        x_half ? x_half[k] : 0);
     nb[k] = (unsigned)((gs[k]->Nw / 64) * (gs[k]->Cw / 32) * splits[k]);
   }
   for (int k = n; k < 8; ++k) pp[k] = pp[n - 1];
@@ -522,9 +530,23 @@
   return (int64_t)splits * ((int64_t)g->Nw * 9 * g->Cw + g->Nw) * (int64_t)sizeof(float);
 }
 
+static int wino4_wgrad_entry(const LgmConvGeom* g, const float* y, int64_t y_pitch, const float* x, int64_t x_pitch, float* gw,
+                             float* gbias, float beta, void* workspace, int64_t workspace_bytes, int64_t* desc, void* stream,
+                             int x_half);
 extern "C" int lgm_conv3x3_wino4_wgrad(const LgmConvGeom* g, const float* y, int64_t y_pitch, const float* x, int64_t x_pitch,
                                        float* gw, float* gbias, float beta, void* workspace, int64_t workspace_bytes,
                                        int64_t* desc, void* stream) {
+  return wino4_wgrad_entry(g, y, y_pitch, x, x_pitch, gw, gbias, beta, workspace, workspace_bytes, desc, stream, 0);
+}
+extern "C" int lgm_conv3x3_wino4_wgrad_up2(const LgmConvGeom* g, const float* y, int64_t y_pitch, const float* x,
+                                           int64_t x_pitch, float* gw, float* gbias, float beta, void* workspace,
+                                           int64_t workspace_bytes, int64_t* desc, void* stream) {
+  LGM_REQUIRE(g && g->H % 2 == 0 && g->W % 2 == 0, "conv3x3_wino4_wgrad_up2: even map sizes expected");
+  return wino4_wgrad_entry(g, y, y_pitch, x, x_pitch, gw, gbias, beta, workspace, workspace_bytes, desc, stream, 1);
+}
+static int wino4_wgrad_entry(const LgmConvGeom* g, const float* y, int64_t y_pitch, const float* x, int64_t x_pitch, float* gw,
+                             float* gbias, float beta, void* workspace, int64_t workspace_bytes, int64_t* desc, void* stream,
+                             int x_half) {
   LGM_REQUIRE(g && y && x && gw && workspace && desc, "conv3x3_wino4_wgrad: null pointer");
   LGM_REQUIRE(lgm_wino4_wgrad_supported(g), "conv3x3_wino4_wgrad: unsupported geometry");
   LGM_REQUIRE(y_pitch % 4 == 0 && x_pitch % 4 == 0 && y_pitch >= g->Nw && x_pitch >= g->Cw && lgm_aligned16(y) && lgm_aligned16(x) &&
@@ -536,7 +558,7 @@
   const long n_w = (long)g->Nw * 9 * g->Cw, slab = n_w + g->Nw;
   LGM_REQUIRE(workspace_bytes >= (int64_t)splits * slab * (int64_t)sizeof(float), "conv3x3_wino4_wgrad: workspace too small");
   if (int rc = lgm_wino4_wgrad_launch(g, y, y_pitch, x, x_pitch, (float*)workspace, gbias ? 1 : 0, slab, splits, gps, total,
-                                      (hipStream_t)stream))
+                                      (hipStream_t)stream, x_half))
     return rc;
   union { float f; int64_t i; } bb;
   bb.i = 0;
diff --git a/lightning-generative-models_amd/csrc/winograd4l.hip b/lightning-generative-models_amd/csrc/winograd4l.hip
--- a/lightning-generative-models_amd/csrc/winograd4l.hip
+++ b/lightning-generative-models_amd/csrc/winograd4l.hip
@@ -70,8 +70,7 @@
       const int py = rem / PW, px = rem - py * PW;
       const int gy = h0 - 1 + py, gx = w0 - 1 + px;
       l = (unsigned)(q * 4 * PLANE + img * IMG + py * RS + px);
-      if (gy >= 0 && gy < p.H && gx >= 0 && gx < p.W)
-        g = (unsigned)((((long)(b0 + img) * p.H + gy) * p.W + gx) * p.a_pitch + q * 4) * 4u;
+      g = patch_offset<false>(p, b0 + img, gy, gx, q, nrec_a);
     }
     goff[j] = g;
     plds[j] = l;
diff --git a/lightning-generative-models_amd/lgm_hip/nn.py b/lightning-generative-models_amd/lgm_hip/nn.py
--- a/lightning-generative-models_amd/lgm_hip/nn.py
+++ b/lightning-generative-models_amd/lgm_hip/nn.py
@@ -37,8 +37,8 @@
         if self.deferred:
             ops.wgrad_reduce_batch(self.deferred, self.flat.device)
 
-    def queue_wgrad(self, g, gy, x, gw_ptr: int, beta: float, gb_ptr):
-        new = (g, gy, x, gw_ptr, beta, gb_ptr)
+    def queue_wgrad(self, g, gy, x, gw_ptr: int, beta: float, gb_ptr, x_half: bool = False):
+        new = (g, gy, x, gw_ptr, beta, gb_ptr, True) if x_half else (g, gy, x, gw_ptr, beta, gb_ptr)
         if self._pending and not ops.wgrad_group_supported([e[0] for e in self._pending] + [g]):
             self._finish_pending3x3()
         self._pending.append(new)
@@ -48,7 +48,7 @@
     def _finish_pending3x3(self):
         pend, self._pending = self._pending, []
         if len(pend) == 1:
-            e = pend[0]
+            e = ops.wgrad_materialised(pend[0])
             ops.conv_wgrad(e[0], e[1], e[2], e[3], e[4], e[5], defer=self.deferred)
         elif pend:
             ops.conv_wgrad_group(pend, self.deferred)
@@ -207,6 +207,44 @@
         return gx
 
 
+def _conv_up2_ok(self, x_lo, y) -> bool:
+    if self.k != 3 or self.stride != 1 or self.padding != 1:
+        return False
+    B, H, W, _ = x_lo.shape
+    fp = _flat(self.weight)
+    return ops.conv_up2_ok(self.geom(B, 2 * H, 2 * W), fp.ptr(self.weight),
+                           fp.ptr(self.bias) if self.bias is not None else None, x_lo, y)
+
+
+def _conv_fwd_up2(self, x_lo, out):
+    B, H, W, _ = x_lo.shape
+    fp = _flat(self.weight)
+    ops.conv_xy_up2(self.geom(B, 2 * H, 2 * W), x_lo, fp.ptr(self.weight),
+                    fp.ptr(self.bias) if self.bias is not None else None, out)
+    return out
+
+
+def _conv_bwd_up2(self, gc: GradCtx, x_lo, gy, gx, accumulate) -> bool:
+    B, H, W, _ = gy.shape
+    g = self.geom(B, H, W)
+    if gc.deferred is None or gc.defer_for(self.weight) is None or not ops.conv_yx_up2_ok(gy, gx):
+        return False
+    if not ops.wgrad_queueable(g, gy, x_lo):
+        return False
+    fp = gc.flat
+    bw = gc.beta(self.weight)
+    gb = None
+    if self.bias is not None:
+        bb = gc.beta(self.bias)
+        if bb == bw:
+            gb = fp.gptr(self.bias)
+        else:
+            ops.colsum(gy, fp.gptr(self.bias), bb)
+    gc.queue_wgrad(g, gy, x_lo, fp.gptr(self.weight), bw, gb, x_half=True)
+    ops.conv_yx_up2(g, gy, fp.ptr(self.weight), gx if accumulate else None, gx)
+    return True
+
+
 def _conv_linear(self, x, out=None):
     B, H, W, _ = x.shape
     g = self.geom(B, H, W)
@@ -233,6 +271,9 @@
     ops.conv_wgrad(self.geom(B, H, W), y, x, gc.flat.gptr(self.weight), gc.beta(self.weight), None)
 
 
+Conv2d.up2_ok = _conv_up2_ok
+Conv2d.fwd_up2 = _conv_fwd_up2
+Conv2d.bwd_up2 = _conv_bwd_up2
 Conv2d.linear = _conv_linear
 Conv2d.dgrad = _conv_dgrad
 Conv2d.wgrad = _conv_wgrad
diff --git a/lightning-generative-models_amd/lgm_hip/ops.py b/lightning-generative-models_amd/lgm_hip/ops.py
--- a/lightning-generative-models_amd/lgm_hip/ops.py
+++ b/lightning-generative-models_amd/lgm_hip/ops.py
@@ -266,6 +266,60 @@
     getattr(L, launch)(yx, ctypes.byref(g), a.data_ptr(), pitch(a), u_ptr, bias_ptr, _p(res),
                        pitch(res) if res is not None else 0, out.data_ptr(), pitch(out), *wsa, stream())
     return True
+
+
+_UP2_OK = _plan_cache()
+
+
+def _up2_operand_ok(*ts) -> bool:
+    return all(t is None or (t.data_ptr() % 16 == 0 and pitch(t) % 4 == 0) for t in ts)
+
+
+def conv_up2_ok(g: ConvGeom, w_ptr: Optional[int], bias_ptr, x_lo, y) -> bool:
+    if not (WINO and WINO4 and WGRAD2 and _WINO_FLATS and not B3) or g.KH != 3 or g.KW != 3 or w_ptr is None:
+        return False
+    if WENG and _weng_take(g, w_ptr, None, False) is not None:
+        return False
+    if not (_wino4_preferred(g, 0) and _wino4_preferred(g, 1)):
+        return False
+    if not _memo(_UP2_OK, _gkey(g), lambda: bool(lib().lgm_conv3x3_wino4_up2_supported(ctypes.byref(g)))):
+        return False
+    if _wino_u(w_ptr, False, f4=True) is None or _wino_u(w_ptr, True, f4=True) is None:
+        return False
+    return _up2_operand_ok(x_lo, y) and (bias_ptr or 0) % 16 == 0 and wgrad_group_supported([g, g])
+
+
+def _conv_up2(yx: int, g: ConvGeom, a, w_ptr: int, bias_ptr, res, out):
+    L = lib()
+    n = _memo(_WINO_WS, (g.B, g.H, g.W, g.Cw, g.Nw, yx, "lgm_conv3x3_wino4", False),
+              lambda: L.lgm_conv3x3_wino4_workspace(ctypes.byref(g), yx))
+    ws = workspace(n, a.device) if n > 0 else None
+    wsa = (None, 0) if ws is None else (ws.data_ptr(), ws.numel() * 4)
+    with _timed("igemm_yx" if yx else "igemm_xy", g):
+        L.lgm_conv3x3_wino4_up2(yx, ctypes.byref(g), a.data_ptr(), pitch(a), _wino_u(w_ptr, bool(yx), f4=True), bias_ptr,
+                                _p(res), pitch(res) if res is not None else 0, out.data_ptr(), pitch(out), *wsa, stream())
+
+
+def conv_xy_up2(g: ConvGeom, x_lo, w_ptr: int, bias_ptr: Optional[int], y):
+    _conv_up2(0, g, x_lo, w_ptr, bias_ptr, None, y)
+
+
+def conv_yx_up2(g: ConvGeom, gy, w_ptr: int, res_lo, gx_lo):
+    _conv_up2(1, g, gy, w_ptr, None, res_lo, gx_lo)
+
+
+def conv_yx_up2_ok(gy, gx_lo) -> bool:
+    return _up2_operand_ok(gy, gx_lo)
+
+
+def wgrad_materialised(e):
+    if len(e) < 7 or not e[6]:
+        return tuple(e[:6])
+    x = e[2]
+    B, H, W, C = x.shape
+    hi = new((B, 2 * H, 2 * W, C), x)
+    upsample2x_fwd(x, hi)
+    return (e[0], e[1], hi) + tuple(e[3:6])
 
 
 _EPI_STATS = _plan_cache()
@@ -596,6 +650,14 @@
     launch, _, sizes = kind
     n = len(entries)
     geoms = [e[0] for e in entries]
+    half = [1 if (len(e) > 6 and e[6]) else 0 for e in entries]
+    if any(half):
+        arr = _geom_array(geoms)
+        if kind is not _WGRAD3X3 or not _memo(_UP2_OK, ("group",) + tuple(_gkey(g) for g in geoms),
+                                              lambda: bool(L.lgm_conv3x3_wino_wgradn_up2_supported(n, ctypes.addressof(arr)))):
+            entries = [wgrad_materialised(e) for e in entries]
+            half = [0] * n
+    entries = [tuple(e[:6]) for e in entries]
 
     def plan():
         out = (ctypes.c_int64 * n)()
@@ -612,7 +674,11 @@
         items[k] = WgradItem(ctypes.addressof(g), gy.data_ptr(), pitch(gy), x.data_ptr(), pitch(x), gw_ptr, gb_ptr, beta,
                              ws.data_ptr(), ws.numel() * 4, ctypes.addressof(desc))
     with _timed("wgrad", geoms):
-        getattr(L, launch)(n, ctypes.addressof(items), stream())
+        if any(half):
+            flags = (ctypes.c_int * n)(*half)
+            getattr(L, launch + "_up2")(n, ctypes.addressof(items), ctypes.addressof(flags), stream())
+        else:
+            getattr(L, launch)(n, ctypes.addressof(items), stream())
     for desc in descs:
         if desc[6] > 1:
             defer.append(tuple(desc))
diff --git a/lightning-generative-models_amd/models/generative/diffusion/ddpm.py b/lightning-generative-models_amd/models/generative/diffusion/ddpm.py
--- a/lightning-generative-models_amd/models/generative/diffusion/ddpm.py
+++ b/lightning-generative-models_amd/models/generative/diffusion/ddpm.py
@@ -222,14 +222,26 @@
 
     def fwd(self, x, out, save):
         B, H, W, C = x.shape
+        conv = self._modules["1"]
+        if conv.up2_ok(x, out):
+            conv.fwd_up2(x, out)
+            return (x, True) if save else None
         hi = ops.new((B, 2 * H, 2 * W, C), x)
         ops.upsample2x_fwd(x, hi)
-        self._modules["1"].fwd(hi, out=out)
-        return (hi,) if save else None
+        conv.fwd(hi, out=out)
+        return (hi, False) if save else None
 
     def bwd(self, gc, saved, gy, gx, accumulate):
-        (hi,) = saved
-        ghi = self._modules["1"].bwd(gc, hi, gy)
+        x, folded = saved
+        conv = self._modules["1"]
+        if folded:
+            if conv.bwd_up2(gc, x, gy, gx, accumulate):
+                return gx
+            B, H, W, C = x.shape
+            hi = ops.new((B, 2 * H, 2 * W, C), x)
+            ops.upsample2x_fwd(x, hi)
+            x = hi
+        ghi = conv.bwd(gc, x, gy)
         ops.upsample2x_bwd(ghi, gx, accumulate)
         return gx
 
```
